# Blaizzy/mlx-audio-swift

Hardware: NVIDIA H100
Metric: orpheus3b_tts_rtfx_batch8 (higher is better)
Workload: dtype bf16

## Files before the change

### include/b200audio_internal.h

```cpp
#ifndef B200AUDIO_INTERNAL_H
#define B200AUDIO_INTERNAL_H

#include "b200audio.h"

#ifdef __cplusplus
extern "C" {
#endif

int32_t b2a_tts_create_random(int32_t device, const b2a_llama_config* cfg, float std, uint64_t seed,
                              b2a_snac* snac, b2a_tts** out);
int32_t b2a_stt_create_random(int32_t device, const b2a_whisper_config* cfg, float std, uint64_t seed, b2a_stt** out);
int32_t b2a_tts_set_bench_flags(b2a_tts* h, int32_t mask_eos, int32_t wrap_codes);
int32_t b2a_stt_set_bench_flags(b2a_stt* h, int32_t mask_eot);
int32_t b2a_tts_time_steps(b2a_tts* h, int32_t batch, int32_t ctx, int32_t iters, float* ms_per_step);
int32_t b2a_qwen3_talker_create_random(int32_t device, const b2a_qwen3_talker_config* cfg, float std, uint64_t seed, b2a_qwen3_talker** out);
int32_t b2a_qwen3_talker_set_bench_flags(b2a_qwen3_talker* h, int32_t mask_eos);

int32_t b2a_tts_debug_trace(b2a_tts* h, int32_t enable, int32_t batch, float* out);
int32_t b2a_debug_step_smem(int32_t gqa, int32_t* out);

int32_t b2a_speech_tokenizer_debug_layout(const float* w, int32_t out, int32_t k, int32_t in, int32_t stride, float* layout_out,
                                          int64_t capacity, int32_t* rows, int32_t* taps, int32_t* kpad);
int32_t b2a_speech_tokenizer_debug_stage(b2a_speech_tokenizer* h, int32_t stage, float* out, int64_t capacity, int64_t* n);
int32_t b2a_qwen3_sample_test(const float* logits, int32_t batch, int32_t vocab, float temperature, float top_p, int32_t top_k,
                              float min_p, float repetition_penalty, int32_t eos, int32_t suppress_lo, int32_t suppress_hi,
                              uint32_t* seen, int32_t track, uint64_t seed, int32_t step, int32_t* tokens_out, float* filtered_out);
int32_t b2a_implicit_conv_test(const float* w, int32_t M, int32_t taps, int32_t Cin, const float* x, int32_t B, int32_t Ttot, int32_t T,
                               int32_t dil, int32_t shift0, int32_t up, const float* bias, const float* gamma, int32_t gelu, int32_t add,
                               int32_t bias_twice_t0, const float* sa, const float* sb, int32_t Hout, int32_t fp16, float* xo, float* hl_out);
int32_t b2a_tc_gemm_epilogue_test(const void* W, const void* X, void* out, int32_t M, int32_t N, int32_t K, int32_t bn, int32_t epi,
                                  int32_t split, int32_t hilo, int32_t ctas, const float* bias, int32_t act, int32_t tile_rows,
                                  int32_t lo_rows, const float* rstd_ss, int32_t rstd_parts, float rstd_eps, int32_t stages, void* stream);
int32_t b2a_tc_gemm_test(const void* W, const void* X, void* out, int32_t M, int32_t N, int32_t K, int32_t bn, int32_t epi,
                         int32_t split, int32_t hilo, int32_t ctas, void* stream);
int32_t b2a_tc_gemm_splitk_test(const void* W, const void* X, float* h, const float* gain, void* xn, float* ss, int32_t M, int32_t N,
                                int32_t K, int32_t cluster, int32_t stages, void* stream);
int32_t b2a_mha_tc_test(const float* qkv, void* out, int32_t B, int32_t T, int32_t nh, void* stream);
int32_t b2a_wh_decode_attn_test(int32_t self_attn, const float* q, const float* kv, const int32_t* pos, void* kcache, void* vcache,
                                void* out, float* part_o, float* part_ml, int32_t* counters, int32_t B, int32_t nh, int32_t max_t,
                                void* stream);
int32_t b2a_conv_gemm_test(const float* w, int32_t M, int32_t K, const void* X, int32_t N, int32_t epi, const float* bias,
                           const float* alpha, const float* gamma, int32_t gelu, float* x, int32_t ldx, void* hl, int32_t ldh,
                           int32_t dual, int32_t T, int32_t Cout, int32_t stride, int32_t pad, int32_t Tin, const float* noise,
                           uint64_t seed, int32_t ctas, void* stream);
int32_t b2a_snac_unit_test(int32_t mode, int32_t C, int32_t dil, const float* x, float* y, int32_t B, int32_t T, const float* dw_w,
                           const float* dw_b, const float* a_in, const float* a_mid, const float* pw_w, const float* pw_bias,
                           const float* noise, uint64_t seed, void* hl, const float* a_next, int32_t ctas, void* stream);
int32_t b2a_snac_convt_test(const float* x, float* y, const float* alpha, const float* bias, const float* w, int32_t B, int32_t Tin,
                            int32_t stride, int32_t cout, int32_t ctas, void* stream);
int32_t b2a_snac_encode_latent_test(b2a_snac* h, const float* wave, int32_t batch, int64_t n_samples, float* z);

#ifdef __cplusplus
}
#endif
#endif
```

### mlx-audio-swift_b200/_ffi.py

```python
from __future__ import annotations

import ctypes as C
from pathlib import Path

import numpy as np

LIB_PATH = Path(__file__).resolve().parent / "lib" / "libb200audio.so"

(OK, ERR_MODEL_NOT_INITIALIZED, ERR_GENERATION_FAILED, ERR_INVALID_INPUT, ERR_AUDIO_DECODING_FAILED,
 ERR_AUDIO_ENCODING_FAILED, ERR_CANCELLED, ERR_CUDA) = range(8)
DTYPE_F32, DTYPE_BF16, DTYPE_I32 = 0, 1, 2


class AudioGenerationError(RuntimeError):
    CASES = {1: "modelNotInitialized", 2: "generationFailed", 3: "invalidInput", 4: "audioDecodingFailed",
             5: "audioEncodingFailed", 6: "cancelled", 7: "cudaError"}

    def __init__(self, code: int, message: str):
        super().__init__(f"{self.CASES.get(code, code)}: {message}")
        self.code, self.case, self.message = code, self.CASES.get(code, str(code)), message


class Tensor(C.Structure):
    _fields_ = [("name", C.c_char_p), ("dtype", C.c_int32), ("ndim", C.c_int32), ("shape", C.c_int64 * 4),
                ("data", C.c_void_p)]


class SnacConfig(C.Structure):
    _fields_ = [("sampling_rate", C.c_int32), ("encoder_dim", C.c_int32), ("n_encoder_rates", C.c_int32),
                ("encoder_rates", C.c_int32 * 8), ("latent_dim", C.c_int32), ("decoder_dim", C.c_int32),
                ("n_decoder_rates", C.c_int32), ("decoder_rates", C.c_int32 * 8), ("attn_window_size", C.c_int32),
                ("codebook_size", C.c_int32), ("codebook_dim", C.c_int32), ("n_vq_strides", C.c_int32),
                ("vq_strides", C.c_int32 * 8), ("noise", C.c_int32), ("depthwise", C.c_int32)]


class LlamaConfig(C.Structure):
    _fields_ = [("hidden_size", C.c_int32), ("num_hidden_layers", C.c_int32), ("intermediate_size", C.c_int32),
                ("num_attention_heads", C.c_int32), ("num_key_value_heads", C.c_int32), ("head_dim", C.c_int32),
                ("vocab_size", C.c_int32), ("rms_norm_eps", C.c_float), ("rope_theta", C.c_float),
                ("rope_factor", C.c_float), ("rope_low_freq_factor", C.c_float), ("rope_high_freq_factor", C.c_float),
                ("rope_old_context_len", C.c_float), ("tie_word_embeddings", C.c_int32), ("max_batch", C.c_int32),
                ("max_context", C.c_int32)]


class GenParams(C.Structure):
    _fields_ = [("max_tokens", C.c_int32), ("temperature", C.c_float), ("top_p", C.c_float),
                ("repetition_penalty", C.c_float), ("repetition_context_size", C.c_int32), ("seed", C.c_uint64)]


class GenInfo(C.Structure):
    _fields_ = [("prompt_token_count", C.c_int32), ("generation_token_count", C.c_int32), ("prefill_time", C.c_double),
                ("generate_time", C.c_double), ("tokens_per_second", C.c_double), ("codec_time", C.c_double),
                ("peak_memory_gb", C.c_double)]


class VocosConfig(C.Structure):
    _fields_ = [(n, C.c_int32) for n in ("input_channels", "dim", "intermediate_dim", "num_layers", "n_fft", "hop_length",
                                          "input_kernel_size", "dw_kernel_size", "adanorm_num_embeddings")]


class EncodecConfig(C.Structure):
    _fields_ = ([(n, C.c_int32) for n in ("audio_channels", "num_filters", "kernel_size", "num_residual_layers",
                                           "dilation_growth_rate", "codebook_size", "codebook_dim", "hidden_size",
                                           "num_lstm_layers", "residual_kernel_size", "use_causal_conv", "pad_mode_reflect",
                                           "norm_type", "last_kernel_size", "compress", "n_upsampling_ratios")]
                + [("upsampling_ratios", C.c_int32 * 8), ("sampling_rate", C.c_int32), ("use_conv_shortcut", C.c_int32),
                   ("trim_right_ratio", C.c_float), ("chunk_length_s", C.c_float), ("overlap", C.c_float)])


class SpeechTokenizerConfig(C.Structure):
    _fields_ = ([(n, C.c_int32) for n in ("codebook_size", "codebook_dim", "latent_dim", "decoder_dim", "hidden_size",
                                           "intermediate_size", "head_dim", "num_attention_heads", "num_key_value_heads",
                                           "num_hidden_layers", "num_quantizers", "num_semantic_quantizers")]
                + [("rms_norm_eps", C.c_float), ("rope_theta", C.c_float), ("attention_bias", C.c_int32),
                   ("num_upsample_rates", C.c_int32), ("upsample_rates", C.c_int32 * 8),
                   ("num_upsampling_ratios", C.c_int32), ("upsampling_ratios", C.c_int32 * 8),
                   ("max_batch", C.c_int32), ("max_cache_frames", C.c_int32)])


class Qwen3TalkerConfig(C.Structure):
    _fields_ = ([(n, C.c_int32) for n in ("vocab_size", "hidden_size", "intermediate_size", "num_hidden_layers", "num_attention_heads",
                                           "num_key_value_heads", "head_dim")]
                + [("rms_norm_eps", C.c_float), ("rope_theta", C.c_float)]
                + [(n, C.c_int32) for n in ("num_code_groups", "text_hidden_size", "text_vocab_size", "codec_eos_token_id", "cp_vocab_size",
                                             "cp_hidden_size", "cp_intermediate_size", "cp_num_hidden_layers", "cp_num_attention_heads",
                                             "cp_num_key_value_heads", "cp_head_dim")]
                + [("cp_rms_norm_eps", C.c_float), ("cp_rope_theta", C.c_float), ("max_batch", C.c_int32), ("max_context", C.c_int32)])


class Qwen3GenParams(C.Structure):
    _fields_ = [("max_tokens", C.c_int32), ("temperature", C.c_float), ("top_p", C.c_float), ("top_k", C.c_int32), ("min_p", C.c_float),
                ("repetition_penalty", C.c_float), ("seed", C.c_uint64)]


class WhisperConfig(C.Structure):
    _fields_ = [(n, C.c_int32) for n in ("vocab_size", "num_mel_bins", "d_model", "encoder_layers", "encoder_attention_heads",
                                          "encoder_ffn_dim", "max_source_positions", "decoder_layers", "decoder_attention_heads",
                                          "decoder_ffn_dim", "max_target_positions", "max_batch")]


class SttParams(C.Structure):
    _fields_ = [("max_tokens", C.c_int32), ("temperature", C.c_float), ("prompt_ids", C.c_void_p), ("n_prompt", C.c_int32),
                ("begin_suppress", C.c_void_p), ("n_begin_suppress", C.c_int32), ("suppress", C.c_void_p),
                ("n_suppress", C.c_int32), ("timestamp_begin", C.c_int32), ("eot", C.c_int32), ("seed", C.c_uint64)]


class SttInfo(C.Structure):
    _fields_ = [("prompt_tokens", C.c_int32), ("generation_tokens", C.c_int32), ("decode_steps", C.c_int32),
                ("encode_time", C.c_double), ("decode_time", C.c_double), ("total_time", C.c_double)]


TOKEN_CB = C.CFUNCTYPE(None, C.c_void_p, C.c_int32, C.c_int32, C.c_int32)
AUDIO_CB = C.CFUNCTYPE(None, C.c_void_p, C.c_int32, C.POINTER(C.c_float), C.c_int64, C.c_int32)
STT_DECODE_CB = C.CFUNCTYPE(C.c_int32, C.c_void_p, C.POINTER(C.c_float), C.c_int64, C.POINTER(C.c_int32), C.c_int32, C.POINTER(C.c_int32),
                            C.c_int32, C.POINTER(C.c_int32))


class SttStreamConfig(C.Structure):
    _fields_ = [("decode_interval_s", C.c_double), ("window_s", C.c_double), ("window_overlap_s", C.c_double), ("delay_ms", C.c_int32),
                ("min_agreement_passes", C.c_int32), ("max_tokens_per_pass", C.c_int32), ("sample_rate", C.c_int32)]


class SttStreamUpdate(C.Structure):
    _fields_ = [("kind", C.c_int32), ("promoted", C.c_int32), ("completed_windows", C.c_int32), ("n_confirmed", C.c_int32),
                ("n_provisional", C.c_int32), ("total_audio_s", C.c_double), ("pass_encode_time", C.c_double), ("pass_decode_time", C.c_double)]


_P = C.c_void_p
SIGNATURES = {
    "b2a_last_error": (C.c_char_p, []),
    "b2a_version": (C.c_char_p, []),
    "b2a_device_count": (C.c_int32, []),
    "b2a_launch_count": (C.c_int64, []),
    "b2a_hanning_window": (C.c_int32, [C.c_int32, C.c_int32, _P]),
    "b2a_hamming_window": (C.c_int32, [C.c_int32, C.c_int32, _P]),
    "b2a_power_to_db": (C.c_int32, [_P, C.c_int64, C.c_float, C.c_float, _P]),
    "b2a_mel_filters": (C.c_int32, [C.c_int32, C.c_int32, C.c_int32, C.c_float, C.c_float, C.c_int32, C.c_int32, _P]),
    "b2a_mel_create": (C.c_int32, [C.c_int32, C.c_int32, C.c_int32, C.c_int32, C.c_int32, C.POINTER(_P)]),
    "b2a_mel_max_frames": (C.c_int64, [_P, C.c_int64]),
    "b2a_mel_process": (C.c_int32, [_P, _P, C.c_int64, _P, C.c_int64, C.POINTER(C.c_int64)]),
    "b2a_mel_flush": (C.c_int32, [_P, _P, C.c_int64, C.POINTER(C.c_int64)]),
    "b2a_mel_reset": (C.c_int32, [_P]),
    "b2a_mel_total_frames": (C.c_int64, [_P]),
    "b2a_mel_destroy": (None, [_P]),
    "b2a_logmel_create": (C.c_int32, [C.c_int32, C.c_int32, C.c_int32, C.c_int32, C.c_int32, C.c_int32, C.POINTER(_P)]),
    "b2a_logmel_frames": (C.c_int64, [_P, C.c_int64]),
    "b2a_logmel_compute": (C.c_int32, [_P, _P, C.c_int32, C.c_int64, _P]),
    "b2a_logmel_compute_dev": (C.c_int32, [_P, _P, C.c_int32, C.c_int64, _P, _P]),
    "b2a_logmel_destroy": (None, [_P]),
    "b2a_snac_create": (C.c_int32, [C.c_int32, C.POINTER(SnacConfig), C.POINTER(Tensor), C.c_int32, C.POINTER(_P)]),
    "b2a_snac_hop_length": (C.c_int64, [_P]),
    "b2a_snac_decode": (C.c_int32, [_P, C.POINTER(_P), C.c_int32, C.c_int64, C.POINTER(_P), C.c_int32, C.c_uint64, _P]),
    "b2a_snac_decode_dev": (C.c_int32, [_P, C.POINTER(_P), C.c_int32, C.c_int64, C.POINTER(_P), C.c_int32, C.c_uint64, _P, _P]),
    "b2a_snac_quantize": (C.c_int32, [_P, _P, C.c_int32, C.c_int64, C.POINTER(_P), _P]),
    "b2a_snac_encoded_length": (C.c_int64, [_P, C.c_int64]),
    "b2a_snac_encode": (C.c_int32, [_P, _P, C.c_int32, C.c_int64, C.POINTER(_P)]),
    "b2a_snac_encode_dev": (C.c_int32, [_P, _P, C.c_int32, C.c_int64, C.POINTER(_P), _P]),
    "b2a_snac_encode_latent_test": (C.c_int32, [_P, _P, C.c_int32, C.c_int64, _P]),
    "b2a_snac_destroy": (None, [_P]),
    "b2a_tts_create": (C.c_int32, [C.c_int32, C.POINTER(LlamaConfig), C.POINTER(Tensor), C.c_int32, _P, C.POINTER(_P)]),
    "b2a_tts_debug_trace": (C.c_int32, [_P, C.c_int32, C.c_int32, _P]),
    "b2a_debug_step_smem": (C.c_int32, [C.c_int32, C.POINTER(C.c_int32)]),
    "b2a_tts_create_random": (C.c_int32, [C.c_int32, C.POINTER(LlamaConfig), C.c_float, C.c_uint64, _P, C.POINTER(_P)]),
    "b2a_tts_stream": (C.c_void_p, [_P]),
    "b2a_tts_set_bench_flags": (C.c_int32, [_P, C.c_int32, C.c_int32]),
    "b2a_stt_set_bench_flags": (C.c_int32, [_P, C.c_int32]),
    "b2a_tts_time_steps": (C.c_int32, [_P, C.c_int32, C.c_int32, C.c_int32, C.POINTER(C.c_float)]),
    "b2a_snac_stream": (C.c_void_p, [_P]),
    "b2a_tts_prepare_input_ids": (C.c_int32, [C.POINTER(_P), _P, C.c_int32, _P, C.POINTER(C.c_int32)]),
    "b2a_tts_prepare_input_ids_ref": (C.c_int32, [C.POINTER(_P), _P, C.c_int32, _P, C.c_int32, _P, C.c_int32, _P, C.POINTER(C.c_int32)]),
    "b2a_tts_forward_logits": (C.c_int32, [_P, _P, C.c_int32, C.c_int32, C.c_int32, _P]),
    "b2a_tts_generate": (C.c_int32, [_P, _P, C.c_int32, C.c_int32, C.POINTER(GenParams), _P, _P, _P, C.c_int64, _P,
                                     C.POINTER(GenInfo), TOKEN_CB, _P]),
    "b2a_tts_generate_stream": (C.c_int32, [_P, _P, C.c_int32, C.c_int32, C.POINTER(GenParams), C.c_int32, C.c_int32, _P, _P,
                                            C.POINTER(GenInfo), TOKEN_CB, AUDIO_CB, _P]),
    "b2a_tts_generate_dev": (C.c_int32, [_P, _P, C.c_int32, C.c_int32, C.POINTER(GenParams), _P, C.c_int64, _P,
                                         C.POINTER(GenInfo)]),
    "b2a_tts_cancel": (C.c_int32, [_P]),
    "b2a_tts_parse_output": (C.c_int32, [_P, C.c_int32, C.c_int32, _P, _P]),
    "b2a_tts_deinterleave": (C.c_int32, [_P, C.c_int32, _P, _P, _P, C.POINTER(C.c_int32)]),
    "b2a_tts_interleave": (C.c_int32, [_P, _P, _P, C.c_int32, _P]),
    "b2a_tts_destroy": (None, [_P]),
    "b2a_vocos_create": (C.c_int32, [C.c_int32, C.POINTER(VocosConfig), C.POINTER(Tensor), C.c_int32, C.POINTER(_P)]),
    "b2a_vocos_output_length": (C.c_int64, [_P, C.c_int32]),
    "b2a_vocos_stream": (C.c_void_p, [_P]),
    "b2a_vocos_decode": (C.c_int32, [_P, _P, C.c_int32, C.c_int32, _P]),
    "b2a_vocos_decode_dev": (C.c_int32, [_P, _P, C.c_int32, C.c_int32, _P, _P]),
    "b2a_vocos_decode_cond": (C.c_int32, [_P, _P, _P, C.c_int32, C.c_int32, _P]),
    "b2a_vocos_destroy": (None, [_P]),
    "b2a_speech_tokenizer_create": (C.c_int32, [C.c_int32, C.POINTER(SpeechTokenizerConfig), C.POINTER(Tensor), C.c_int32, C.POINTER(_P)]),
    "b2a_speech_tokenizer_total_upsample": (C.c_int32, [_P]),
    "b2a_speech_tokenizer_stream": (C.c_void_p, [_P]),
    "b2a_speech_tokenizer_reset": (C.c_int32, [_P]),
    "b2a_speech_tokenizer_streaming_step": (C.c_int32, [_P, _P, C.c_int32, C.c_int32, C.c_int32, _P]),
    "b2a_speech_tokenizer_streaming_step_dev": (C.c_int32, [_P, _P, C.c_int32, C.c_int32, C.c_int32, _P, _P]),
    "b2a_speech_tokenizer_streaming_decode": (C.c_int32, [_P, _P, C.c_int32, C.c_int32, C.c_int32, C.c_int32, _P]),
    "b2a_speech_tokenizer_chunked_decode": (C.c_int32, [_P, _P, C.c_int32, C.c_int32, C.c_int32, C.c_int32, C.c_int32, _P]),
    "b2a_speech_tokenizer_destroy": (None, [_P]),
    "b2a_weights_sanitize_speech_tokenizer": (C.c_int32, [_P]),
    "b2a_speech_tokenizer_config_from_json": (C.c_int32, [C.c_char_p, C.c_int32, C.c_int32, C.POINTER(SpeechTokenizerConfig), C.POINTER(C.c_int32)]),
    "b2a_speech_tokenizer_create_from_directory": (C.c_int32, [C.c_char_p, C.c_int32, C.c_int32, C.c_int32, C.POINTER(_P), C.POINTER(C.c_int32)]),
    "b2a_qwen3_sample_test": (C.c_int32, [_P, C.c_int32, C.c_int32, C.c_float, C.c_float, C.c_int32, C.c_float, C.c_float, C.c_int32, C.c_int32,
                                         C.c_int32, _P, C.c_int32, C.c_uint64, C.c_int32, _P, _P]),
    "b2a_implicit_conv_test": (C.c_int32, [_P, C.c_int32, C.c_int32, C.c_int32, _P, C.c_int32, C.c_int32, C.c_int32, C.c_int32, C.c_int32, C.c_int32,
                                          _P, _P, C.c_int32, C.c_int32, C.c_int32, _P, _P, C.c_int32, C.c_int32, _P, _P]),
    "b2a_tc_gemm_test": (C.c_int32, [_P, _P, _P] + [C.c_int32] * 8 + [_P]),
    "b2a_tc_gemm_epilogue_test": (C.c_int32, [_P, _P, _P] + [C.c_int32] * 8 + [_P, C.c_int32, C.c_int32, C.c_int32, _P, C.c_int32,
                                                                             C.c_float, C.c_int32, _P]),
    "b2a_tc_gemm_splitk_test": (C.c_int32, [_P, _P, _P, _P, _P, _P] + [C.c_int32] * 5 + [_P]),
    "b2a_mha_tc_test": (C.c_int32, [_P, _P, C.c_int32, C.c_int32, C.c_int32, _P]),
    "b2a_wh_decode_attn_test": (C.c_int32, [C.c_int32, _P, _P, _P, _P, _P, _P, _P, _P, _P, C.c_int32, C.c_int32, C.c_int32, _P]),
    "b2a_conv_gemm_test": (C.c_int32, [_P, C.c_int32, C.c_int32, _P, C.c_int32, C.c_int32, _P, _P, _P, C.c_int32, _P, C.c_int32, _P,
                                       C.c_int32] + [C.c_int32] * 6 + [_P, C.c_uint64, C.c_int32, _P]),
    "b2a_snac_unit_test": (C.c_int32, [C.c_int32] * 3 + [_P, _P, C.c_int32, C.c_int32] + [_P] * 6 + [_P, C.c_uint64, _P, _P, C.c_int32, _P]),
    "b2a_snac_convt_test": (C.c_int32, [_P] * 5 + [C.c_int32] * 5 + [_P]),
    "b2a_speech_tokenizer_debug_stage": (C.c_int32, [_P, C.c_int32, _P, C.c_int64, _P]),
    "b2a_speech_tokenizer_debug_layout": (C.c_int32, [_P, C.c_int32, C.c_int32, C.c_int32, C.c_int32, _P, C.c_int64, _P, _P, _P]),
    "b2a_encodec_create": (C.c_int32, [C.c_int32, C.POINTER(EncodecConfig), C.POINTER(Tensor), C.c_int32, C.POINTER(_P)]),
    "b2a_encodec_output_length": (C.c_int64, [_P, C.c_int32, C.c_int32]),
    "b2a_encodec_num_codebooks": (C.c_int32, [_P]),
    "b2a_encodec_stream": (C.c_void_p, [_P]),
    "b2a_encodec_decode": (C.c_int32, [_P, _P, C.c_int32, C.c_int32, C.c_int32, C.c_int32, _P, _P]),
    "b2a_encodec_decode_dev": (C.c_int32, [_P, _P, C.c_int32, C.c_int32, C.c_int32, C.c_int32, _P, _P, _P]),
    "b2a_encodec_destroy": (None, [_P]),
    "b2a_weights_load": (C.c_int32, [C.c_char_p, C.POINTER(_P)]),
    "b2a_weights_count": (C.c_int32, [_P]),
    "b2a_weights_get": (C.c_int32, [_P, C.c_int32, C.POINTER(Tensor)]),
    "b2a_weights_sanitize_whisper": (C.c_int32, [_P, C.POINTER(C.c_int32)]),
    "b2a_weights_sanitize_llama": (C.c_int32, [_P, C.c_int32, C.c_int32, C.c_int32]),
    "b2a_weights_sanitize_llama_config": (C.c_int32, [_P, C.c_char_p]),
    "b2a_weights_dequantize": (C.c_int32, [_P, C.c_int32, C.c_int32]),
    "b2a_weights_free": (None, [_P]),
    "b2a_tts_config_from_json": (C.c_int32, [C.c_char_p, C.c_int32, C.c_int32, C.POINTER(LlamaConfig), C.POINTER(C.c_int32), C.POINTER(C.c_int32)]),
    "b2a_tts_create_from_directory": (C.c_int32, [C.c_char_p, C.c_int32, C.c_int32, C.c_int32, _P, C.POINTER(_P)]),
    "b2a_stt_create": (C.c_int32, [C.c_int32, C.POINTER(WhisperConfig), C.POINTER(Tensor), C.c_int32, C.POINTER(_P)]),
    "b2a_stt_create_random": (C.c_int32, [C.c_int32, C.POINTER(WhisperConfig), C.c_float, C.c_uint64, C.POINTER(_P)]),
    "b2a_stt_stream": (C.c_void_p, [_P]),
    "b2a_stt_encode": (C.c_int32, [_P, _P, C.c_int32, C.c_int64, _P]),
    "b2a_stt_decoder_logits": (C.c_int32, [_P, _P, C.c_int32, C.c_int32, _P]),
    "b2a_stt_transcribe": (C.c_int32, [_P, _P, C.c_int32, C.c_int64, C.POINTER(SttParams), _P, _P, C.POINTER(SttInfo)]),
    "b2a_stt_transcribe_dev": (C.c_int32, [_P, _P, C.c_int32, C.c_int64, C.POINTER(SttParams), _P, _P, C.POINTER(SttInfo)]),
    "b2a_stt_transcribe_long": (C.c_int32, [_P, _P, C.c_int64, C.POINTER(SttParams), C.c_int32, _P, _P, _P, C.POINTER(C.c_int32), C.POINTER(SttInfo)]),
    "b2a_qwen3_talker_create": (C.c_int32, [C.c_int32, C.POINTER(Qwen3TalkerConfig), C.POINTER(Tensor), C.c_int32, C.POINTER(_P)]),
    "b2a_qwen3_talker_create_random": (C.c_int32, [C.c_int32, C.POINTER(Qwen3TalkerConfig), C.c_float, C.c_uint64, C.POINTER(_P)]),
    "b2a_qwen3_talker_set_bench_flags": (C.c_int32, [_P, C.c_int32]),
    "b2a_qwen3_talker_stream": (C.c_void_p, [_P]),
    "b2a_qwen3_talker_embed_text": (C.c_int32, [_P, _P, C.c_int32, _P]),
    "b2a_qwen3_talker_embed_codec": (C.c_int32, [_P, _P, C.c_int32, _P]),
    "b2a_qwen3_talker_forward": (C.c_int32, [_P, _P, C.c_int32, C.c_int32, _P, _P]),
    "b2a_qwen3_talker_generate": (C.c_int32, [_P, _P, C.c_int32, C.c_int32, _P, _P, C.c_int32, _P, C.POINTER(Qwen3GenParams), _P, _P,
                                              C.POINTER(GenInfo), _P, _P]),
    "b2a_qwen3_talker_config_from_json": (C.c_int32, [C.c_char_p, C.c_int32, C.c_int32, C.POINTER(Qwen3TalkerConfig)]),
    "b2a_weights_sanitize_qwen3_talker": (C.c_int32, [_P, C.c_char_p]),
    "b2a_qwen3_talker_create_from_directory": (C.c_int32, [C.c_char_p, C.c_int32, C.c_int32, C.c_int32, C.POINTER(_P)]),
    "b2a_qwen3_talker_cancel": (C.c_int32, [_P]),
    "b2a_qwen3_talker_destroy": (None, [_P]),
    "b2a_stt_session_create": (C.c_int32, [_P, C.POINTER(SttParams), C.POINTER(SttStreamConfig), C.POINTER(_P)]),
    "b2a_stt_session_create_with_decoder": (C.c_int32, [STT_DECODE_CB, _P, C.POINTER(SttStreamConfig), C.POINTER(_P)]),
    "b2a_stt_session_feed": (C.c_int32, [_P, _P, C.c_int64, C.c_double, C.POINTER(SttStreamUpdate)]),
    "b2a_stt_session_stop": (C.c_int32, [_P, C.c_double, C.POINTER(SttStreamUpdate)]),
    "b2a_stt_session_tokens": (C.c_int32, [_P, C.c_int32, C.c_int32, _P, C.c_int32, C.POINTER(C.c_int32)]),
    "b2a_stt_session_destroy": (None, [_P]),
    "b2a_stt_cancel": (C.c_int32, [_P]),
    "b2a_stt_destroy": (None, [_P]),
}

_lib = None


def lib() -> C.CDLL:
    global _lib
    if _lib is None:
        if not LIB_PATH.exists():
            raise ImportError(f"{LIB_PATH} is missing: build it with `python -c 'import __graft_entry__ as g; g.build()'`"
                              " -- there is no CPU fallback")
        _lib = C.CDLL(str(LIB_PATH))
        for name, (res, args) in SIGNATURES.items():
            fn = getattr(_lib, name)
            fn.restype, fn.argtypes = res, args
    return _lib


def check(status: int) -> None:
    if status != OK:
        raise AudioGenerationError(status, lib().b2a_last_error().decode("utf-8", "replace"))


def ptr(a) -> C.c_void_p:
    if a is None:
        return C.c_void_p(None)
    if isinstance(a, np.ndarray):
        assert a.flags["C_CONTIGUOUS"]
        return C.c_void_p(a.ctypes.data)
    return C.c_void_p(a.data_ptr())


def make_tensor_table(weights: dict):
    import torch
    arr = (Tensor * len(weights))()
    keep = []
    for i, (name, w) in enumerate(weights.items()):
        if isinstance(w, torch.Tensor):
            w = w.detach().contiguous().cpu()
            if w.dtype == torch.bfloat16:
                dt = DTYPE_BF16
            elif w.dtype == torch.float32:
                dt = DTYPE_F32
            else:
                w = w.to(torch.float32); dt = DTYPE_F32
            data, shape = w.data_ptr(), tuple(w.shape)
        else:
            w = np.ascontiguousarray(w)
            if w.dtype == np.int32:
                dt = DTYPE_I32
            else:
                if w.dtype != np.float32:
                    w = w.astype(np.float32)
                dt = DTYPE_F32
            data, shape = w.ctypes.data, w.shape
        assert len(shape) <= 4, name
        nm = name.encode()
        keep += [w, nm]
        arr[i].name, arr[i].dtype, arr[i].ndim, arr[i].data = nm, dt, len(shape), data
        for j, s in enumerate(shape):
            arr[i].shape[j] = s
    return arr, keep
```

### mlx-audio-swift_b200/csrc/llama.cu

```cuda
#include "common.cuh"
#include <cooperative_groups.h>
#include "tc_gemm.cuh"
#include "qwen3_sampler.cuh"

#include <algorithm>
#include <cstdlib>
#include <cstring>
#include <chrono>
#include <cmath>

namespace b2a {

typedef __nv_bfloat16 bf16;

constexpr int TOK_START_OF_HUMAN = 128259, TOK_END_OF_HUMAN = 128260, TOK_END_OF_TEXT = 128009;
constexpr int TOK_START_OF_SPEECH = 128257, TOK_END_OF_SPEECH = 128258, TOK_PAD = 128263;
constexpr int TOK_AUDIO_OFFSET = 128266;
constexpr int TOK_AUDIO_START = 128261, TOK_AUDIO_END = 128262;

__device__ __forceinline__ float bf16_round(float x) { return __bfloat162float(__float2bfloat16_rn(x)); }
__device__ __forceinline__ float bf_lo(unsigned u) { return __uint_as_float(u << 16); }
__device__ __forceinline__ float bf_hi(unsigned u) { return __uint_as_float(u & 0xffff0000u); }

__device__ __forceinline__ uint4 ldg_stream(const uint4* p) {
    uint4 r;
    asm volatile("ld.global.nc.L1::no_allocate.v4.u32 {%0,%1,%2,%3}, [%4];"
                 : "=r"(r.x), "=r"(r.y), "=r"(r.z), "=r"(r.w) : "l"(p));
    return r;
}

__global__ void embed_kernel(const int* __restrict__ tokens, const bf16* __restrict__ embed, float* __restrict__ x,
                             float* __restrict__ y, int H, int V) {
    const int b = blockIdx.x;
    pdl_trigger();
    pdl_wait();
    int tok = tokens[b];
    tok = min(max(tok, 0), V - 1);
    for (int i = threadIdx.x; i < H; i += blockDim.x) {
        x[(long long)b * H + i] = __bfloat162float(embed[(long long)tok * H + i]);
        y[(long long)b * H + i] = 0.f;
    }
}

__global__ void ext_embed_kernel(const float* __restrict__ src, float* __restrict__ x, float* __restrict__ y, int H) {
    const int b = blockIdx.x;
    pdl_trigger();
    pdl_wait();
    for (int i = threadIdx.x; i < H; i += blockDim.x) {
        x[(long long)b * H + i] = src[(long long)b * H + i];
        y[(long long)b * H + i] = 0.f;
    }
}

__global__ void finalize_norm_kernel(const float* __restrict__ x, const float* __restrict__ w, const float* __restrict__ ss, int parts,
                                     float* __restrict__ out, int H, float eps) {
    const int b = blockIdx.x;
    pdl_trigger();
    pdl_wait();
    float t = 0.f;
    for (int p = 0; p < parts; ++p) t += ss[p * 8 + b];
    const float r = rsqrtf(t / (float)H + eps);
    for (int i = threadIdx.x; i < H; i += blockDim.x) out[(long long)b * H + i] = x[(long long)b * H + i] * r * w[i];
}

constexpr int LO_ROW = 8;

constexpr int RN_THREADS = 1024, RN_MAXV = 8;
__global__ void __launch_bounds__(RN_THREADS)
add_rmsnorm_kernel(float* __restrict__ x, float* __restrict__ delta, const float* __restrict__ w,
                   bf16* __restrict__ xn, int H, float eps, float* __restrict__ trace, float* __restrict__ zero_ptr,
                   int zero_n, int half, float* __restrict__ normed = nullptr, float* __restrict__ ss_out = nullptr,
                   int ss_parts = 0) {
    __shared__ float red[RN_THREADS / 32];
    const int b = blockIdx.x, tid = threadIdx.x;
    pdl_trigger();
    pdl_wait();
    float* xr = x + (long long)b * H;
    float v[RN_MAXV];
    float ss = 0.f;
#pragma unroll
    for (int j = 0; j < RN_MAXV; ++j) {
        const int i = tid + j * RN_THREADS;
        float val = 0.f;
        if (i < H) {
            val = xr[i];
            if (delta) { val += delta[(long long)b * H + i]; xr[i] = val; delta[(long long)b * H + i] = 0.f; }
            if (trace) trace[(long long)b * H + i] = val;
        }
        v[j] = val;
        ss += val * val;
    }
    ss = warp_sum(ss);
    if ((tid & 31) == 0) red[tid >> 5] = ss;
    __syncthreads();
    float tot = 0.f;
#pragma unroll
    for (int i = 0; i < RN_THREADS / 32; ++i) tot += red[i];
    const float r = ss_out ? 1.0f : rsqrtf(tot / (float)H + eps);
    if (ss_out && tid < ss_parts) ss_out[tid * 8 + b] = tid == 0 ? tot : 0.f;
#pragma unroll
    for (int j = 0; j < RN_MAXV; ++j) {
        const int i = tid + j * RN_THREADS;
        if (i < H) {
            const float o = v[j] * r * w[i];
            tc::store_hilo(xn, H, b, i, o, half);
            if (normed) normed[(long long)b * H + i] = o;
        }
    }
    if (zero_ptr)
        for (int i = tid; i < zero_n; i += RN_THREADS) zero_ptr[(long long)b * zero_n + i] = 0.f;
}

constexpr int GV_MAX_THREADS = 256;
enum : int { GV_F32 = 0, GV_SWIGLU = 1, GV_F32_ATOMIC = 2 };

template <int NB, int ROWS, int EPI>
__global__ void __launch_bounds__(GV_MAX_THREADS)
gemv_bf16_kernel(const bf16* __restrict__ W, const bf16* __restrict__ xin, float* __restrict__ y,
                 bf16* __restrict__ act, int N, int K) {
    extern __shared__ uint4 sx[];
    pdl_trigger();
    pdl_wait();
    const int K8 = K >> 3;
    const int Kc8 = K8 / gridDim.y, kbase = blockIdx.y * Kc8;
    for (int i = threadIdx.x; i < 2 * NB * Kc8; i += blockDim.x) {
        const int r = i / Kc8, k = i - r * Kc8;
        const int grow = r < NB ? r : LO_ROW + (r - NB);
        sx[i] = reinterpret_cast<const uint4*>(xin)[(long long)grow * K8 + kbase + k];
    }
    __syncthreads();
    const int warp = threadIdx.x >> 5, lane = threadIdx.x & 31;
    const int row0 = (blockIdx.x * (blockDim.x >> 5) + warp) * ROWS;
    if (row0 >= N) return;
    const uint4* Wr[ROWS];
#pragma unroll
    for (int r = 0; r < ROWS; ++r)
        Wr[r] = reinterpret_cast<const uint4*>(W) + (long long)min(row0 + r, N - 1) * K8 + kbase;

    float acc[ROWS][2 * NB];
#pragma unroll
    for (int r = 0; r < ROWS; ++r)
#pragma unroll
        for (int b = 0; b < 2 * NB; ++b) acc[r][b] = 0.f;

    for (int k8 = lane; k8 < Kc8; k8 += 32) {
        float wf[ROWS][8];
#pragma unroll
        for (int r = 0; r < ROWS; ++r) {
            const uint4 wv = ldg_stream(Wr[r] + k8);
            wf[r][0] = bf_lo(wv.x); wf[r][1] = bf_hi(wv.x); wf[r][2] = bf_lo(wv.y); wf[r][3] = bf_hi(wv.y);
            wf[r][4] = bf_lo(wv.z); wf[r][5] = bf_hi(wv.z); wf[r][6] = bf_lo(wv.w); wf[r][7] = bf_hi(wv.w);
        }
#pragma unroll
        for (int b = 0; b < 2 * NB; ++b) {
            const uint4 xv = sx[b * Kc8 + k8];
            const float xf[8] = {bf_lo(xv.x), bf_hi(xv.x), bf_lo(xv.y), bf_hi(xv.y),
                                 bf_lo(xv.z), bf_hi(xv.z), bf_lo(xv.w), bf_hi(xv.w)};
#pragma unroll
            for (int r = 0; r < ROWS; ++r)
#pragma unroll
                for (int j = 0; j < 8; ++j) acc[r][b] = fmaf(wf[r][j], xf[j], acc[r][b]);
        }
    }
#pragma unroll
    for (int r = 0; r < ROWS; ++r)
#pragma unroll
        for (int b = 0; b < NB; ++b) acc[r][b] = warp_sum(acc[r][b] + acc[r][NB + b]);
    if (lane == 0) {
        if (EPI == GV_F32 || EPI == GV_F32_ATOMIC) {
#pragma unroll
            for (int r = 0; r < ROWS; ++r)
                if (row0 + r < N)
#pragma unroll
                    for (int b = 0; b < NB; ++b) {
                        if (EPI == GV_F32) y[(long long)b * N + row0 + r] = acc[r][b];
                        else atomicAdd(&y[(long long)b * N + row0 + r], acc[r][b]);
                    }
        } else {
#pragma unroll
            for (int r = 0; r < ROWS; r += 2)
                if (row0 + r + 1 < N)
#pragma unroll
                    for (int b = 0; b < NB; ++b) {
                        const float g = acc[r][b], u = acc[r + 1][b];
                        tc::store_hilo(act, N / 2, b, (row0 + r) / 2, g / (1.0f + __expf(-g)) * u, LO_ROW);
                    }
        }
    }
}

constexpr int HD = 128, AT_THREADS = 256, MAXG = 8, AT_CAP = 64;
constexpr int AT_SLOTS = 3;
constexpr size_t attn_smem_bytes(int G) {
    return ((size_t)AT_SLOTS * AT_CAP * HD + (size_t)G * HD + 2 * HD + (size_t)G * HD + 2 * MAXG) * sizeof(float) + 64;
}
static_assert((AT_THREADS / 32) * MAXG * HD <= AT_CAP * HD, "the warp-partial outputs must fit in one ring slot");

struct AttnArgs {
    const float* qkv;
    const int* pos;
    const float* freqs;
    float* kcache;
    float* vcache;
    bf16* out;
    int nq, nkv, max_ctx;
    float scale;
    const float* qnorm;
    const float* knorm;
    float qk_eps;
    int zero_qkv;
};

template <int G>
__global__ void __cluster_dims__(1, 1, 2) __launch_bounds__(AT_THREADS)
attn_decode_cluster_kernel(const __grid_constant__ AttnArgs a) {
    namespace cgr = cooperative_groups;
    cgr::cluster_group cluster = cgr::this_cluster();
    const int rank = (int)cluster.block_rank();
    extern __shared__ __align__(16) uint8_t at_smem[];
    float* sKV = reinterpret_cast<float*>(at_smem);
    float* wpo = sKV;
    float* sq = sKV + (size_t)AT_SLOTS * AT_CAP * HD;
    float* snew = sq + G * HD;
    float* xo = snew + 2 * HD;
    float* xml = xo + G * HD;
    uint64_t* bars = reinterpret_cast<uint64_t*>(xml + 2 * MAXG);
    __shared__ float red_m[AT_THREADS / 32][MAXG], red_l[AT_THREADS / 32][MAXG];

    const int h = blockIdx.x, b = blockIdx.y, tid = threadIdx.x;
    pdl_trigger();
    const int p = a.pos[b];
    if (!(p >= 0 && p < a.max_ctx)) { pdl_wait(); return; }
    const int nch = p / AT_CAP + 1;
    const int n_my = nch > rank ? (nch - rank + 1) / 2 : 0;
    const bool owner = ((nch - 1) & 1) == rank;
    const int qkv_ld = (a.nq + 2 * a.nkv) * HD;
    const float* row = a.qkv + (long long)b * qkv_ld;
    float* kc = a.kcache + (((long long)b * a.nkv + h) * a.max_ctx) * HD;
    float* vc = a.vcache + (((long long)b * a.nkv + h) * a.max_ctx) * HD;
    const int n_mat = 2 * n_my;
    auto issue = [&](int j) {
        const int slot = j % AT_SLOTS, c = rank + 2 * (j >> 1);
        const int n_load = (c < nch - 1) ? AT_CAP : p - c * AT_CAP;
        if (n_load > 0) {
            const uint32_t bytes = (uint32_t)n_load * HD * 4;
            tc::mbar_arrive_expect_tx(&bars[slot], bytes);
            asm volatile("cp.async.bulk.shared::cluster.global.mbarrier::complete_tx::bytes [%0], [%1], %2, [%3];"
                         ::"r"(tc::smem_u32(sKV + (size_t)slot * AT_CAP * HD)), "l"(((j & 1) ? vc : kc) + (long long)c * AT_CAP * HD), "r"(bytes),
                           "r"(tc::smem_u32(&bars[slot])) : "memory");
        } else {
            tc::mbar_arrive(&bars[slot]);
        }
    };
    if (tid == 0) {
        for (int i = 0; i < AT_SLOTS; ++i) tc::mbar_init(&bars[i], 1);
        tc::fence_barrier_init();
        asm volatile("fence.proxy.async.shared::cta;" ::: "memory");
        for (int j = 0; j < min(n_mat, AT_SLOTS); ++j) issue(j);
    }
    float sn = 0.f, cs = 1.f;
    if (tid < HD / 2) sincosf((float)p / a.freqs[tid], &sn, &cs);
    pdl_wait();
    const float* qsrc = row + (long long)h * G * HD;
    const float* ksrc = row + (a.nq + h) * HD;
    if (a.qnorm) {
        for (int vec = tid >> 5; vec < G + 1; vec += AT_THREADS / 32) {
            const float* src = vec < G ? qsrc + vec * HD : ksrc;
            const float* w = vec < G ? a.qnorm : a.knorm;
            const float4 x = reinterpret_cast<const float4*>(src)[tid & 31];
            const float ss = warp_sum(x.x * x.x + x.y * x.y + x.z * x.z + x.w * x.w);
            const float r = rsqrtf(ss * (1.0f / HD) + a.qk_eps);
            const float4 g4 = reinterpret_cast<const float4*>(w)[tid & 31];
            reinterpret_cast<float4*>(vec < G ? sq + vec * HD : snew)[tid & 31] =
                make_float4(x.x * r * g4.x, x.y * r * g4.y, x.z * r * g4.z, x.w * r * g4.w);
        }
        __syncthreads();
        qsrc = sq;
        ksrc = snew;
    }
    if (tid < HD / 2) {
        const int d = tid;
        _Pragma("unroll") for (int g = 0; g < G; ++g) {
            const float* q = qsrc + g * HD;
            const float x1 = q[d], x2 = q[d + HD / 2];
            sq[g * HD + d] = x1 * cs - x2 * sn;
            sq[g * HD + d + HD / 2] = x2 * cs + x1 * sn;
        }
        const float* k = ksrc;
        const float x1 = k[d], x2 = k[d + HD / 2];
        const float k1 = x1 * cs - x2 * sn, k2 = x2 * cs + x1 * sn;
        if (owner) { kc[(long long)p * HD + d] = k1; kc[(long long)p * HD + d + HD / 2] = k2; }
        snew[d] = k1;
        snew[d + HD / 2] = k2;
    } else if (tid >= 128) {
        const int d = tid - 128;
        const float v = row[(a.nq + a.nkv + h) * HD + d];
        if (owner) vc[(long long)p * HD + d] = v;
        snew[HD + d] = v;
    }
    __syncthreads();

    const int lane = tid & 31, warp = tid >> 5;
    const int kslot = warp * 8 + (lane >> 2), part = lane & 3;
    float m_run[G], l_run[G];
    float4 o4[G];
    _Pragma("unroll") for (int g = 0; g < G; ++g) { m_run[g] = -INFINITY; l_run[g] = 0.f; o4[g] = make_float4(0.f, 0.f, 0.f, 0.f); }

    for (int i = 0; i < n_my; ++i) {
        const int jk = 2 * i, jv = 2 * i + 1, c = rank + 2 * i;
        float* sK = sKV + (size_t)(jk % AT_SLOTS) * AT_CAP * HD;
        float* sV = sKV + (size_t)(jv % AT_SLOTS) * AT_CAP * HD;
        const int t0 = c * AT_CAP, nk = min(AT_CAP, p + 1 - t0);
        tc::mbar_wait(&bars[jk % AT_SLOTS], (uint32_t)((jk / AT_SLOTS) & 1));
        if (c == nch - 1) {
            if (tid < HD) sK[(p - t0) * HD + tid] = snew[tid];
            __syncthreads();
        }
        float sacc[G];
        _Pragma("unroll") for (int g = 0; g < G; ++g) sacc[g] = 0.f;
        if (kslot < nk) {
            const float4* kr = reinterpret_cast<const float4*>(sK + kslot * HD);
#pragma unroll
            for (int j = 0; j < 8; ++j) {
                const int d4 = part + 4 * ((j + kslot) & 7);
                const float4 kf = kr[d4];
                _Pragma("unroll") for (int g = 0; g < G; ++g) {
                    const float4 qf = reinterpret_cast<const float4*>(sq + g * HD)[d4];
                    sacc[g] = fmaf(qf.x, kf.x, sacc[g]); sacc[g] = fmaf(qf.y, kf.y, sacc[g]);
                    sacc[g] = fmaf(qf.z, kf.z, sacc[g]); sacc[g] = fmaf(qf.w, kf.w, sacc[g]);
                }
            }
        }
        if (jk + AT_SLOTS < n_mat) {
            __syncthreads();
            if (tid == 0) issue(jk + AT_SLOTS);
        }
        float pw[G];
        _Pragma("unroll") for (int g = 0; g < G; ++g) {
            float v = sacc[g];
            v += __shfl_xor_sync(0xffffffffu, v, 1);
            v += __shfl_xor_sync(0xffffffffu, v, 2);
            const float sv = kslot < nk ? v * a.scale : -INFINITY;
            float m = sv;
            m = fmaxf(m, __shfl_xor_sync(0xffffffffu, m, 4));
            m = fmaxf(m, __shfl_xor_sync(0xffffffffu, m, 8));
            m = fmaxf(m, __shfl_xor_sync(0xffffffffu, m, 16));
            const float m_new = fmaxf(m_run[g], m);
            const float rescale = (m_run[g] == -INFINITY) ? 0.f : __expf(m_run[g] - m_new);
            const float e = (sv == -INFINITY) ? 0.f : __expf(sv - m_new);
            float l = part == 0 ? e : 0.f;
            l = warp_sum(l);
            l_run[g] = l_run[g] * rescale + l;
            m_run[g] = m_new;
            o4[g].x *= rescale; o4[g].y *= rescale; o4[g].z *= rescale; o4[g].w *= rescale;
            pw[g] = e;
        }
        tc::mbar_wait(&bars[jv % AT_SLOTS], (uint32_t)((jv / AT_SLOTS) & 1));
        if (c == nch - 1) {
            if (tid >= HD) sV[(p - t0) * HD + tid - HD] = snew[tid];
            __syncthreads();
        }
#pragma unroll
        for (int kk = 0; kk < 8; ++kk) {
            const int t = warp * 8 + kk;
            if (t < nk) {
                const float4 v = reinterpret_cast<const float4*>(sV + t * HD)[lane];
                _Pragma("unroll") for (int g = 0; g < G; ++g) {
                    const float pk = __shfl_sync(0xffffffffu, pw[g], kk * 4);
                    o4[g].x = fmaf(pk, v.x, o4[g].x); o4[g].y = fmaf(pk, v.y, o4[g].y);
                    o4[g].z = fmaf(pk, v.z, o4[g].z); o4[g].w = fmaf(pk, v.w, o4[g].w);
                }
            }
        }
        if (jv + AT_SLOTS < n_mat) {
            __syncthreads();
            if (tid == 0) issue(jv + AT_SLOTS);
        }
    }
    __syncthreads();
    _Pragma("unroll") for (int g = 0; g < G; ++g) {
        reinterpret_cast<float4*>(wpo + (warp * G + g) * HD)[lane] = o4[g];
        if (lane == 0) { red_m[warp][g] = m_run[g]; red_l[warp][g] = l_run[g]; }
    }
    __syncthreads();
    float Ms[G], Ls[G], Os[G];
    if (tid < HD) {
        _Pragma("unroll") for (int g = 0; g < G; ++g) {
            float M = red_m[0][g];
#pragma unroll
            for (int w = 1; w < AT_THREADS / 32; ++w) M = fmaxf(M, red_m[w][g]);
            float L = 0.f, O = 0.f;
#pragma unroll
            for (int w = 0; w < AT_THREADS / 32; ++w) {
                const float sc_w = red_m[w][g] == -INFINITY ? 0.f : __expf(red_m[w][g] - M);
                L = fmaf(red_l[w][g], sc_w, L);
                O = fmaf(wpo[(w * G + g) * HD + tid], sc_w, O);
            }
            Ms[g] = M; Ls[g] = L; Os[g] = O;
        }
        if (rank == 1) {
            float* rxo = cluster.map_shared_rank(xo, 0);
            float* rxml = cluster.map_shared_rank(xml, 0);
            _Pragma("unroll") for (int g = 0; g < G; ++g) {
                rxo[g * HD + tid] = Os[g];
                if (tid == 0) { rxml[g] = Ms[g]; rxml[MAXG + g] = Ls[g]; }
            }
        }
    }
    cluster.sync();
    if (a.zero_qkv && rank == 0) {
        float* wrow = const_cast<float*>(row);
        for (int i = tid; i < G * HD; i += AT_THREADS) wrow[(long long)h * G * HD + i] = 0.f;
        if (tid < HD) { wrow[(a.nq + h) * HD + tid] = 0.f; wrow[(a.nq + a.nkv + h) * HD + tid] = 0.f; }
    }
    if (rank == 0 && tid < HD) {
        _Pragma("unroll") for (int g = 0; g < G; ++g) {
            const float M1 = xml[g], L1 = xml[MAXG + g], O1 = xo[g * HD + tid];
            const float M = fmaxf(Ms[g], M1);
            const float w0 = Ms[g] == -INFINITY ? 0.f : __expf(Ms[g] - M), w1 = M1 == -INFINITY ? 0.f : __expf(M1 - M);
            const float L = Ls[g] * w0 + L1 * w1, O = Os[g] * w0 + O1 * w1;
            tc::store_hilo(a.out, (long long)a.nq * HD, b, (h * G + g) * HD + tid, O / L, LO_ROW);
        }
    }
}

constexpr int PF_HALF = 64;
constexpr int PA_QT = 32, PA_THREADS = 256, PA_MAXL = 128;

__global__ void embed_rows_kernel(const int* __restrict__ ids, const bf16* __restrict__ embed, float* __restrict__ x,
                                  int H, int V) {
    const int t = blockIdx.x;
    int tok = ids[t];
    tok = min(max(tok, 0), V - 1);
    for (int i = threadIdx.x; i < H; i += blockDim.x) x[(long long)t * H + i] = __bfloat162float(embed[(long long)tok * H + i]);
}

__global__ void rope_table_kernel(const float* __restrict__ freqs, float2* __restrict__ tab, int L) {
    const int i = blockIdx.x * blockDim.x + threadIdx.x;
    if (i >= L * (HD / 2)) return;
    const int p = i / (HD / 2), d = i - p * (HD / 2);
    float s, c;
    sincosf((float)p / freqs[d], &s, &c);
    tab[i] = make_float2(c, s);
}

struct PrefillAttnArgs {
    const float* qkv;
    const float2* rope;
    float* kcache;
    float* vcache;
    bf16* out;
    int nq, nkv, max_ctx, L;
    float scale;
};

template <int G>
__global__ void __launch_bounds__(PA_THREADS)
prefill_attn_kernel(PrefillAttnArgs a) {
    extern __shared__ __align__(16) uint8_t pa_smem[];
    const int h = blockIdx.x, b = blockIdx.y, q0 = blockIdx.z * PA_QT;
    const int nqt = min(PA_QT, a.L - q0), kmax = q0 + nqt;
    float* sK = reinterpret_cast<float*>(pa_smem);
    float* sV = sK + (size_t)a.L * HD;
    float* sQ = sV + (size_t)a.L * HD;
    const int tid = threadIdx.x, lane = tid & 31, warp = tid >> 5;
    const int ld = (a.nq + 2 * a.nkv) * HD;
    const float* base = a.qkv + (long long)b * a.L * ld;
    float* kc = a.kcache + (((long long)b * a.nkv + h) * a.max_ctx) * HD;
    float* vc = a.vcache + (((long long)b * a.nkv + h) * a.max_ctx) * HD;

    for (int i = tid; i < kmax * (HD / 2); i += PA_THREADS) {
        const int t = i / (HD / 2), d = i - t * (HD / 2);
        const float2 cs = a.rope[t * (HD / 2) + d];
        const float* k = base + (long long)t * ld + (a.nq + h) * HD;
        const float x1 = k[d], x2 = k[d + HD / 2];
        const float k1 = x1 * cs.x - x2 * cs.y, k2 = x2 * cs.x + x1 * cs.y;
        sK[t * HD + d] = k1; sK[t * HD + d + HD / 2] = k2;
        if (t >= q0) { kc[(long long)t * HD + d] = k1; kc[(long long)t * HD + d + HD / 2] = k2; }
    }
    for (int i = tid; i < kmax * HD; i += PA_THREADS) {
        const int t = i / HD, d = i - t * HD;
        const float v = base[(long long)t * ld + (a.nq + a.nkv + h) * HD + d];
        sV[i] = v;
        if (t >= q0) vc[(long long)t * HD + d] = v;
    }
    for (int i = tid; i < G * nqt * (HD / 2); i += PA_THREADS) {
        const int g = i / (nqt * (HD / 2)), r = i - g * nqt * (HD / 2), qi = r / (HD / 2), d = r - qi * (HD / 2);
        const float2 cs = a.rope[(q0 + qi) * (HD / 2) + d];
        const float* q = base + (long long)(q0 + qi) * ld + (h * G + g) * HD;
        const float x1 = q[d], x2 = q[d + HD / 2];
        sQ[(g * PA_QT + qi) * HD + d] = x1 * cs.x - x2 * cs.y;
        sQ[(g * PA_QT + qi) * HD + d + HD / 2] = x2 * cs.x + x1 * cs.y;
    }
    __syncthreads();

    constexpr int KJ = PA_MAXL / 32;
    for (int r = warp; r < G * nqt; r += PA_THREADS / 32) {
        const int g = r / nqt, qi = r - g * nqt, qpos = q0 + qi;
        const float4* q4 = reinterpret_cast<const float4*>(sQ + (g * PA_QT + qi) * HD);
        float sc[KJ];
        float mx = -INFINITY;
#pragma unroll
        for (int j = 0; j < KJ; ++j) {
            const int t = j * 32 + lane;
            float acc = -INFINITY;
            if (t <= qpos) {
                const float4* k4 = reinterpret_cast<const float4*>(sK + t * HD);
                acc = 0.f;
#pragma unroll 8
                for (int i = 0; i < HD / 4; ++i) {
                    const int d4 = (i + lane) & (HD / 4 - 1);
                    const float4 kf = k4[d4], qf = q4[d4];
                    acc = fmaf(qf.x, kf.x, acc); acc = fmaf(qf.y, kf.y, acc);
                    acc = fmaf(qf.z, kf.z, acc); acc = fmaf(qf.w, kf.w, acc);
                }
                acc *= a.scale;
            }
            sc[j] = acc;
            mx = fmaxf(mx, acc);
        }
        for (int o = 16; o; o >>= 1) mx = fmaxf(mx, __shfl_xor_sync(0xffffffffu, mx, o));
        float sum = 0.f;
#pragma unroll
        for (int j = 0; j < KJ; ++j) { sc[j] = sc[j] == -INFINITY ? 0.f : __expf(sc[j] - mx); sum += sc[j]; }
        sum = warp_sum(sum);
        float4 o = make_float4(0.f, 0.f, 0.f, 0.f);
#pragma unroll
        for (int j = 0; j < KJ; ++j) {
            if (j * 32 > qpos) break;
            for (int l = 0; l < 32; ++l) {
                const int t = j * 32 + l;
                if (t > qpos) break;
                const float p = __shfl_sync(0xffffffffu, sc[j], l);
                const float4 v = reinterpret_cast<const float4*>(sV + t * HD)[lane];
                o.x = fmaf(p, v.x, o.x); o.y = fmaf(p, v.y, o.y); o.z = fmaf(p, v.z, o.z); o.w = fmaf(p, v.w, o.w);
            }
        }
        const float inv = 1.0f / sum;
        const int tok = b * a.L + qpos;
        const long long col = (long long)(h * G + g) * HD + lane * 4;
        const long long ldo = (long long)a.nq * HD;
        tc::store_hilo(a.out, ldo, tok, col + 0, o.x * inv, PF_HALF);
        tc::store_hilo(a.out, ldo, tok, col + 1, o.y * inv, PF_HALF);
        tc::store_hilo(a.out, ldo, tok, col + 2, o.z * inv, PF_HALF);
        tc::store_hilo(a.out, ldo, tok, col + 3, o.w * inv, PF_HALF);
    }
}

__global__ void gather_last_kernel(const float* __restrict__ xp, const float* __restrict__ yp, float* __restrict__ x,
                                   float* __restrict__ y, int* __restrict__ pos, int L, int H) {
    const int b = blockIdx.x;
    const long long src = ((long long)b * L + L - 1) * H;
    for (int i = threadIdx.x; i < H; i += blockDim.x) {
        x[(long long)b * H + i] = xp[src + i];
        y[(long long)b * H + i] = yp[src + i];
    }
    if (threadIdx.x == 0) pos[b] = L - 1;
}

constexpr int SM_THREADS = 1024, SM_WARPS = SM_THREADS / 32, SM_MAX_ATTEMPTS = 12;

struct SampleArgs {
    float* logits;
    float* probs;
    int* tokens;
    int* pos;
    int* recent;
    int* recent_n;
    int* out_tokens;
    int* n_gen;
    int* done;
    int* n_active;
    const int* forced;
    int V, R, max_tokens;
    float temperature, top_p, rep_penalty;
    unsigned long long seed;
    int mask_eos;
};

constexpr int SM_CLUSTER = 8;
struct SampleExchange { float v[2][SM_CLUSTER]; int i[2][SM_CLUSTER]; float s[2][SM_CLUSTER]; };

__global__ void __cluster_dims__(SM_CLUSTER, 1, 1) __launch_bounds__(SM_THREADS)
sample_kernel(SampleArgs a) {
    namespace cgr = cooperative_groups;
    cgr::cluster_group cluster = cgr::this_cluster();
    const int rank = (int)cluster.block_rank();
    __shared__ float sred[SM_WARPS];
    __shared__ float s_val[SM_WARPS];
    __shared__ int s_idx[SM_WARPS];
    __shared__ SampleExchange ex;
    const int b = blockIdx.x / SM_CLUSTER, t = threadIdx.x, lane = t & 31, warp = t >> 5;
    pdl_wait();
    float* lg = a.logits + (long long)b * a.V;
    const int chunk = (a.V + SM_CLUSTER - 1) / SM_CLUSTER, i0 = rank * chunk, i1 = min(a.V, i0 + chunk);
    const int nrec = min(a.recent_n[b], a.R);
    int parity = 0;
    int tok_final = 0;

    auto exchange = [&](float& v, int& i, float& sum) {
        for (int o = 16; o; o >>= 1) {
            const float ov = __shfl_xor_sync(0xffffffffu, v, o);
            const int oi = __shfl_xor_sync(0xffffffffu, i, o);
            if (ov > v || (ov == v && oi < i)) { v = ov; i = oi; }
        }
        sum = warp_sum(sum);
        __syncthreads();
        if (lane == 0) { s_val[warp] = v; s_idx[warp] = i; sred[warp] = sum; }
        __syncthreads();
        if (warp == 0) {
            float bv = s_val[lane], bs = sred[lane];
            int bi = s_idx[lane];
            for (int o = 16; o; o >>= 1) {
                const float ov = __shfl_xor_sync(0xffffffffu, bv, o);
                const int oi = __shfl_xor_sync(0xffffffffu, bi, o);
                if (ov > bv || (ov == bv && oi < bi)) { bv = ov; bi = oi; }
            }
            bs = warp_sum(bs);
            if (lane < SM_CLUSTER) {
                SampleExchange* peer = cluster.map_shared_rank(&ex, lane);
                peer->v[parity][rank] = bv; peer->i[parity][rank] = bi; peer->s[parity][rank] = bs;
            }
        }
        cluster.sync();
        v = ex.v[parity][0]; i = ex.i[parity][0]; sum = ex.s[parity][0];
#pragma unroll
        for (int r = 1; r < SM_CLUSTER; ++r) {
            const float ov = ex.v[parity][r];
            const int oi = ex.i[parity][r];
            if (ov > v || (ov == v && oi < i)) { v = ov; i = oi; }
            sum += ex.s[parity][r];
        }
        parity ^= 1;
    };

    if (a.forced == nullptr) {
        if (a.rep_penalty != 1.0f && t < nrec) {
            const int tok = a.recent[b * a.R + t];
            bool dup = false;
            for (int j = 0; j < t; ++j) dup |= (a.recent[b * a.R + j] == tok);
            if (!dup && tok >= i0 && tok < i1) {
                const float l = lg[tok];
                lg[tok] = l < 0.f ? l * a.rep_penalty : l / a.rep_penalty;
            }
        }
        if (a.mask_eos && t == 0 && TOK_END_OF_SPEECH >= i0 && TOK_END_OF_SPEECH < i1) lg[TOK_END_OF_SPEECH] = -INFINITY;
        __syncthreads();

        float best = -INFINITY, dummy = 0.f;
        int bi = 0x7fffffff;
        for (int i = i0 + t; i < i1; i += SM_THREADS) {
            const float v = lg[i];
            if (v > best) { best = v; bi = i; }
        }
        exchange(best, bi, dummy);
        const float mx = best;
        tok_final = bi;

        if (a.temperature > 0.f) {
            const float inv_t = 1.0f / a.temperature;
            const int step = a.n_gen[b];
            auto gumbel_key = [&](int i, float l, int att) {
                unsigned long long z = a.seed + 0x9E3779B97F4A7C15ull * ((unsigned long long)b * 1000003ull + (unsigned long long)step * 131ull + (unsigned long long)att + 1ull);
                z ^= (unsigned long long)(unsigned)i * 0xD6E8FEB86659FD93ull;
                z = (z ^ (z >> 30)) * 0xBF58476D1CE4E5B9ull;
                z = (z ^ (z >> 27)) * 0x94D049BB133111EBull;
                z ^= z >> 31;
                const float u = ((float)(z >> 40) + 0.5f) * (1.0f / 16777216.0f);
                return l * inv_t - __logf(-__logf(u));
            };
            float z = 0.f, gv = -INFINITY;
            int gi = 0x7fffffff;
            for (int i = i0 + t; i < i1; i += SM_THREADS) {
                const float l = lg[i];
                z += __expf((l - mx) * inv_t);
                const float k = l == -INFINITY ? -INFINITY : gumbel_key(i, l, 0);
                if (k > gv) { gv = k; gi = i; }
            }
            exchange(gv, gi, z);
            const float Z = z;
            int cand = gi;
            bool accepted = a.top_p >= 1.0f;
            for (int att = 0; !accepted; ++att) {
                const float lc = lg[cand];
                float gm = 0.f, dv = -INFINITY;
                int di = 0x7fffffff;
                for (int i = i0 + t; i < i1; i += SM_THREADS) { const float l = lg[i]; if (l > lc) gm += __expf((l - mx) * inv_t); }
                exchange(dv, di, gm);
                if (gm < a.top_p * Z) { accepted = true; break; }
                if (att + 1 >= SM_MAX_ATTEMPTS) { cand = tok_final; break; }
                gv = -INFINITY; gi = 0x7fffffff;
                float ds = 0.f;
                for (int i = i0 + t; i < i1; i += SM_THREADS) {
                    const float l = lg[i];
                    const float k = l == -INFINITY ? -INFINITY : gumbel_key(i, l, att + 1);
                    if (k > gv) { gv = k; gi = i; }
                }
                exchange(gv, gi, ds);
                cand = gi;
            }
            if (cand >= 0 && cand < a.V) tok_final = cand;
        }
    } else {
        tok_final = a.forced[b];
    }

    if (rank == 0 && t == 0) {
        const int tok = tok_final;
        a.tokens[b] = tok;
        a.pos[b] += 1;
        const int rn = a.recent_n[b];
        if (a.R > 0) {
            if (rn < a.R) a.recent[b * a.R + rn] = tok;
            else {
                for (int j = 1; j < a.R; ++j) a.recent[b * a.R + j - 1] = a.recent[b * a.R + j];
                a.recent[b * a.R + a.R - 1] = tok;
            }
            a.recent_n[b] = rn + 1;
        }
        if (a.forced == nullptr && !a.done[b]) {
            if (tok == TOK_END_OF_SPEECH) {
                a.done[b] = 1;
                atomicSub(a.n_active, 1);
            } else {
                const int n = a.n_gen[b];
                if (n < a.max_tokens) a.out_tokens[b * a.max_tokens + n] = tok;
                a.n_gen[b] = n + 1;
                if (n + 1 >= a.max_tokens) { a.done[b] = 1; atomicSub(a.n_active, 1); }
            }
        }
    }
}

__global__ void prefill_advance_kernel(const int* __restrict__ ids, int L, int* tokens, int* pos, int B) {
    const int b = threadIdx.x;
    pdl_wait();
    if (b >= B) return;
    const int p = pos[b] + 1;
    pos[b] = p;
    if (p < L) tokens[b] = ids[b * L + p];
}

__global__ void init_rows_kernel(const int* __restrict__ ids, int L, int B, int R, int* tokens, int* pos, int* recent,
                                 int* recent_n, int* n_gen, int* done, int* n_active, int start_pos) {
    const int b = threadIdx.x;
    if (b == 0) *n_active = B;
    if (b >= B) return;
    tokens[b] = ids[b * L];
    pos[b] = start_pos;
    n_gen[b] = 0;
    done[b] = 0;
    const int n = min(R, L);
    for (int j = 0; j < n; ++j) recent[b * R + j] = ids[b * L + L - n + j];
    recent_n[b] = n;
}

__global__ void random_bf16_kernel(bf16* __restrict__ w, long long n, float std, unsigned long long seed) {
    for (long long i = (long long)blockIdx.x * blockDim.x + threadIdx.x; i < n; i += (long long)gridDim.x * blockDim.x) {
        unsigned long long z = seed + 0x9E3779B97F4A7C15ull * (unsigned long long)(i + 1);
        z = (z ^ (z >> 30)) * 0xBF58476D1CE4E5B9ull;
        z = (z ^ (z >> 27)) * 0x94D049BB133111EBull;
        z ^= z >> 31;
        const float u1 = ((unsigned)(z >> 40) + 1.0f) * (1.0f / 16777217.0f);
        const float u2 = (unsigned)((z >> 8) & 0xFFFFFF) * (1.0f / 16777216.0f);
        w[i] = __float2bfloat16_rn(std * sqrtf(-2.0f * __logf(u1)) * cospif(2.0f * u2));
    }
}
__global__ void fill_f32_kernel(float* p, int n, float v) {
    const int i = blockIdx.x * blockDim.x + threadIdx.x;
    if (i < n) p[i] = v;
}

static std::vector<float> llama3_freqs(const b2a_llama_config& c) {
    const int d = c.head_dim;
    std::vector<float> f(d / 2);
    const float low_wl = c.rope_old_context_len / c.rope_low_freq_factor;
    const float high_wl = c.rope_old_context_len / c.rope_high_freq_factor;
    for (int i = 0; i < d / 2; ++i) {
        float fr = powf(c.rope_theta, (float)(2 * i) / (float)d);
        const float wl = 2.0f * (float)M_PI * fr;
        const float base = fr;
        if (wl > low_wl) fr = fr * c.rope_factor;
        const bool med = wl > high_wl && wl < low_wl;
        if (med) {
            const float smooth = (c.rope_old_context_len / wl - c.rope_low_freq_factor) /
                                 (c.rope_high_freq_factor - c.rope_low_freq_factor);
            fr = base / ((1.0f - smooth) / c.rope_factor + smooth);
        }
        f[i] = fr;
    }
    return f;
}

struct LayerW {
    DBuf<bf16> wqkv, wo, wgu, wdown;
    DBuf<float> ln1, ln2;
    DBuf<float> qnorm, knorm;
};

struct StackSpec {
    std::string prefix = "model.";
    bool qk_norm = false;
    bool has_embed = true;
    std::string head;
    bool has_head = true;
};

}

using namespace b2a;

struct b2a_tts {
    int device;
    b2a_llama_config cfg;
    b2a_snac* snac;
    cudaStream_t stream = nullptr;
    std::vector<LayerW> layers;
    DBuf<bf16> embed, lm_head_w;
    const bf16* lm_head = nullptr;
    DBuf<float> final_ln, freqs;
    DBuf<float> kcache, vcache;
    DBuf<float> x, y, qkv, logits, probs;
    DBuf<bf16> xn, attn, act;
    DBuf<float> sk_ws;
    DBuf<unsigned> sk_cnt;
    int sk_slots = 0;
    bool use_tc = true;
    int num_sms = 132;
    std::vector<CUtensorMap> tm_qkv, tm_o, tm_gu, tm_down;
    static int pick_tile_rows(int M, int sms) {
        if (cdiv(M, tc::BM) * 4 >= sms * 3) return tc::BM;
        return std::max(8, std::min(tc::BM, cdiv(cdiv(M, sms), 8) * 8));
    }
    int lm_tile_rows = 128, head_rows_now = 0;
    std::vector<CUtensorMap> tm_gu_dec;
    int gu_tile_rows = 0;
    CUtensorMap tm_lm{}, tmx_xn{}, tmx_attn{}, tmx_act{};
    DBuf<float> xp, yp, qkvp;
    DBuf<bf16> xnp, attnp, actp;
    DBuf<float2> rope_tab;
    CUtensorMap tmp_xn{}, tmp_attn{}, tmp_act{};
    int pf_tokens_cap = 0;
    bool use_batched_prefill = true;
    DBuf<int> tokens, pos, recent, recent_n, out_tokens, n_gen, done, n_active, ids, forced;
    HBuf<int> h_flag;
    cudaEvent_t ev_poll[2] = {nullptr, nullptr};
    bool fused = false;
    static constexpr int fused_cluster = 5;
    static constexpr int gemm_stages = 6, splitk_stages = 5;
    int fused_parts = 0;
    DBuf<float> ss_a, ss_b;
    StackSpec spec;
    const float* x_ext = nullptr;
    float* normed_out = nullptr;
    std::atomic<int> cancel{0};
    int bench_mask_eos = 0, bench_wrap_codes = 0;
    int nb_pad = 0;
    bool trace_on = false;
    DBuf<float> trace;
    cudaGraphExec_t g_step = nullptr, g_prefill = nullptr;
    SampleArgs g_args{};
    int g_nb = 0;
    DBuf<int> d_codes[3];
    DBuf<float> d_wave;

    ~b2a_tts() {
        if (g_step) cudaGraphExecDestroy(g_step);
        if (g_prefill) cudaGraphExecDestroy(g_prefill);
        for (auto& e : ev_poll) if (e) cudaEventDestroy(e);
        if (stream) cudaStreamDestroy(stream);
    }

    static void upload_bf16(const TensorTable& tt, const std::string& name, int64_t expect, DBuf<bf16>& dst, size_t offset_elems,
                            size_t total_elems) {
        const b2a_tensor& t = tt.get(name);
        B2A_CHECK(t.dtype == B2A_DTYPE_BF16 || t.dtype == B2A_DTYPE_F32, B2A_ERR_MODEL_NOT_INITIALIZED, "tensor must be bf16 or f32: " + name);
        B2A_CHECK(TensorTable::numel(t) == expect, B2A_ERR_MODEL_NOT_INITIALIZED, "bad shape for tensor: " + name);
        dst.alloc(total_elems);
        if (t.dtype == B2A_DTYPE_BF16) {
            B2A_CUDA(cudaMemcpy(dst.p + offset_elems, t.data, expect * sizeof(bf16), cudaMemcpyHostToDevice));
        } else {
            std::vector<bf16> tmp((size_t)expect);
            const float* src = (const float*)t.data;
            for (int64_t i = 0; i < expect; ++i) tmp[i] = __float2bfloat16_rn(src[i]);
            B2A_CUDA(cudaMemcpy(dst.p + offset_elems, tmp.data(), expect * sizeof(bf16), cudaMemcpyHostToDevice));
        }
    }

    template <int G>
    static void attn_cluster_attr() {
        B2A_CUDA(cudaFuncSetAttribute(attn_decode_cluster_kernel<G>, cudaFuncAttributeMaxDynamicSharedMemorySize, (int)attn_smem_bytes(G)));
        B2A_CUDA(cudaFuncSetAttribute(attn_decode_cluster_kernel<G>, cudaFuncAttributePreferredSharedMemoryCarveout, cudaSharedmemCarveoutMaxShared));
    }
    void attn_launch(const AttnArgs& aa, int B, cudaStream_t s) {
        const int G = aa.nq / aa.nkv;
        const size_t sm = attn_smem_bytes(G);
        const dim3 g3(aa.nkv, B, 2);
        switch (G) {
            case 1: launch_pdl(attn_decode_cluster_kernel<1>, g3, dim3(AT_THREADS), sm, s, aa); break;
            case 2: launch_pdl(attn_decode_cluster_kernel<2>, g3, dim3(AT_THREADS), sm, s, aa); break;
            case 3: launch_pdl(attn_decode_cluster_kernel<3>, g3, dim3(AT_THREADS), sm, s, aa); break;
            case 4: launch_pdl(attn_decode_cluster_kernel<4>, g3, dim3(AT_THREADS), sm, s, aa); break;
            case 6: launch_pdl(attn_decode_cluster_kernel<6>, g3, dim3(AT_THREADS), sm, s, aa); break;
            default: launch_pdl(attn_decode_cluster_kernel<8>, g3, dim3(AT_THREADS), sm, s, aa); break;
        }
    }

    void check_config() {
        const b2a_llama_config& c = cfg;
        B2A_CHECK(c.head_dim == HD, B2A_ERR_INVALID_INPUT, "llama: head_dim must be 128");
        B2A_CHECK(c.hidden_size % 8 == 0 && c.intermediate_size % 8 == 0, B2A_ERR_INVALID_INPUT, "llama: sizes must be multiples of 8");
        {
            const int g = c.num_key_value_heads > 0 && c.num_attention_heads % c.num_key_value_heads == 0
                              ? c.num_attention_heads / c.num_key_value_heads : 0;
            B2A_CHECK(g == 1 || g == 2 || g == 3 || g == 4 || g == 6 || g == 8, B2A_ERR_INVALID_INPUT,
                      "llama: unsupported GQA ratio (q heads per kv head must be 1, 2, 3, 4, 6 or 8)");
        }
        B2A_CHECK(c.max_batch >= 1 && c.max_batch <= 8, B2A_ERR_INVALID_INPUT, "llama: max_batch must be in 1..8");
        B2A_CHECK(c.max_context >= 8, B2A_ERR_INVALID_INPUT, "llama: max_context too small");
        require_device(device);
        B2A_CUDA(cudaStreamCreateWithFlags(&stream, cudaStreamNonBlocking));
    }

    void alloc_state() {
        const b2a_llama_config& c = cfg;
        const int H = c.hidden_size, I = c.intermediate_size, nq = c.num_attention_heads, nkv = c.num_key_value_heads;
        const int NQ = nq * HD, NKV = nkv * HD;
        B2A_CHECK(H <= RN_THREADS * RN_MAXV, B2A_ERR_INVALID_INPUT, "llama: hidden_size above 8192 is not supported");
        std::vector<float> fr = llama3_freqs(c);
        freqs.upload(fr.data(), fr.size());
        const size_t kv = (size_t)c.num_hidden_layers * c.max_batch * nkv * c.max_context * HD;
        kcache.alloc(kv);
        vcache.alloc(kv);
        B2A_CUDA(cudaMemset(kcache.p, 0, kv * sizeof(float)));
        B2A_CUDA(cudaMemset(vcache.p, 0, kv * sizeof(float)));
        const int B = 8, R16 = 16;
        x.alloc((size_t)B * H); y.alloc((size_t)B * H); qkv.alloc((size_t)B * (NQ + 2 * NKV));
        logits.alloc((size_t)B * c.vocab_size); probs.alloc((size_t)B * c.vocab_size);
        xn.alloc((size_t)R16 * H); attn.alloc((size_t)R16 * NQ); act.alloc((size_t)R16 * I);
        B2A_CUDA(cudaMemset(xn.p, 0, (size_t)R16 * H * sizeof(bf16)));
        B2A_CUDA(cudaMemset(attn.p, 0, (size_t)R16 * NQ * sizeof(bf16)));
        B2A_CUDA(cudaMemset(act.p, 0, (size_t)R16 * I * sizeof(bf16)));
        B2A_CUDA(cudaMemset(x.p, 0, (size_t)B * H * sizeof(float)));
        B2A_CUDA(cudaMemset(y.p, 0, (size_t)B * H * sizeof(float)));
        B2A_CUDA(cudaMemset(qkv.p, 0, (size_t)B * (NQ + 2 * NKV) * sizeof(float)));
        tokens.alloc(B); pos.alloc(B); recent.alloc(B * 64); recent_n.alloc(B); n_gen.alloc(B); done.alloc(B);
        n_active.alloc(1); forced.alloc(B);
        B2A_CUDA(cudaMemset(tokens.p, 0, B * sizeof(int)));
        B2A_CUDA(cudaMemset(pos.p, 0, B * sizeof(int)));
        h_flag.alloc(16);
        gemv_attrs<1>(); gemv_attrs<2>(); gemv_attrs<4>(); gemv_attrs<8>();
        attn_cluster_attr<1>(); attn_cluster_attr<2>(); attn_cluster_attr<3>(); attn_cluster_attr<4>(); attn_cluster_attr<6>(); attn_cluster_attr<8>();
        const char* env = getenv("B2A_GEMM");
        use_tc = !(env && std::string(env) == "simt") && H % tc::BK == 0 && NQ % tc::BK == 0 && I % tc::BK == 0;
        fused_parts = H / tc::BM;
        fused = use_tc && H % tc::BM == 0 && fused_parts <= 64;
        ss_a.alloc((size_t)64 * 8); ss_b.alloc((size_t)64 * 8);
        B2A_CUDA(cudaMemset(ss_a.p, 0, 64 * 8 * sizeof(float)));
        B2A_CUDA(cudaMemset(ss_b.p, 0, 64 * 8 * sizeof(float)));
        B2A_CUDA(cudaDeviceGetAttribute(&num_sms, cudaDevAttrMultiProcessorCount, device));
        {
            const int ops[3][2] = {{NQ + 2 * NKV, H}, {H, NQ}, {H, I}};
            int mt_max = 0;
            for (const auto& op : ops) {
                const int mt = cdiv(op[0], tc::BM), kb = op[1] / tc::BK;
                if (kb == 0) continue;
                const int ctas = (int)std::min<long long>(num_sms, (long long)mt * kb);
                sk_slots = std::max(sk_slots, tc::stream_k_slots(mt, kb, ctas));
                mt_max = std::max(mt_max, mt);
            }
            sk_ws.alloc((size_t)std::max(1, mt_max) * std::max(1, sk_slots) * 16 * tc::BM);
            sk_cnt.alloc((size_t)std::max(1, mt_max));
            B2A_CUDA(cudaMemset(sk_cnt.p, 0, (size_t)std::max(1, mt_max) * sizeof(unsigned)));
        }
        const char* envp = getenv("B2A_PREFILL");
        use_batched_prefill = !(envp && std::string(envp) == "step");
        if (use_tc) {
            tc::set_attributes();
            for (auto& L : layers) {
                tm_qkv.push_back(tc::make_tmap_bf16(L.wqkv.p, NQ + 2 * NKV, H, tc::BM));
                tm_o.push_back(tc::make_tmap_bf16(L.wo.p, H, NQ, tc::BM));
                tm_gu.push_back(tc::make_tmap_bf16(L.wgu.p, 2 * I, H, tc::BM));
                {
                    gu_tile_rows = pick_tile_rows(2 * I, num_sms);
                    tm_gu_dec.push_back(tc::make_tmap_bf16(L.wgu.p, 2 * I, H, gu_tile_rows));
                }
                tm_down.push_back(tc::make_tmap_bf16(L.wdown.p, H, I, tc::BM));
            }
            lm_tile_rows = pick_tile_rows(c.vocab_size, num_sms);
            if (lm_head) tm_lm = tc::make_tmap_bf16(lm_head, c.vocab_size, H, lm_tile_rows);
            tmx_xn = tc::make_tmap_bf16(xn.p, R16, H, 16);
            tmx_attn = tc::make_tmap_bf16(attn.p, R16, NQ, 16);
            tmx_act = tc::make_tmap_bf16(act.p, R16, I, 16);
        }
        B2A_CUDA(cudaDeviceSynchronize());
    }

    b2a_tts(int dev, const b2a_llama_config& c, const TensorTable& tt, b2a_snac* sn, const StackSpec& sp = StackSpec())
        : device(dev), cfg(c), snac(sn), spec(sp) {
        check_config();
        const int H = c.hidden_size, I = c.intermediate_size, nq = c.num_attention_heads, nkv = c.num_key_value_heads;
        const int NQ = nq * HD, NKV = nkv * HD;
        if (sp.has_embed) upload_bf16(tt, sp.prefix + "embed_tokens.weight", (int64_t)c.vocab_size * H, embed, 0, (size_t)c.vocab_size * H);
        if (sp.has_head) {
            if (sp.head.empty() && c.tie_word_embeddings) {
                B2A_CHECK(sp.has_embed, B2A_ERR_MODEL_NOT_INITIALIZED, "a tied head needs the embedding");
                lm_head = embed.p;
            } else {
                upload_bf16(tt, sp.head.empty() ? std::string("lm_head.weight") : sp.head, (int64_t)c.vocab_size * H, lm_head_w, 0, (size_t)c.vocab_size * H);
                lm_head = lm_head_w.p;
            }
        }
        layers.resize(c.num_hidden_layers);
        std::vector<bf16> tmp;
        for (int l = 0; l < c.num_hidden_layers; ++l) {
            const std::string p = sp.prefix + "layers." + std::to_string(l) + ".";
            if (sp.qk_norm) {
                std::vector<float> qn = tt.f32(p + "self_attn.q_norm.weight", HD), kn = tt.f32(p + "self_attn.k_norm.weight", HD);
                layers[l].qnorm.upload(qn.data(), HD);
                layers[l].knorm.upload(kn.data(), HD);
            }
            LayerW& L = layers[l];
            const size_t qkv_n = (size_t)(NQ + 2 * NKV) * H;
            upload_bf16(tt, p + "self_attn.q_proj.weight", (int64_t)NQ * H, L.wqkv, 0, qkv_n);
            upload_bf16(tt, p + "self_attn.k_proj.weight", (int64_t)NKV * H, L.wqkv, (size_t)NQ * H, qkv_n);
            upload_bf16(tt, p + "self_attn.v_proj.weight", (int64_t)NKV * H, L.wqkv, (size_t)(NQ + NKV) * H, qkv_n);
            upload_bf16(tt, p + "self_attn.o_proj.weight", (int64_t)H * NQ, L.wo, 0, (size_t)H * NQ);
            upload_bf16(tt, p + "mlp.down_proj.weight", (int64_t)H * I, L.wdown, 0, (size_t)H * I);
            const b2a_tensor& tg = tt.get(p + "mlp.gate_proj.weight");
            const b2a_tensor& tu = tt.get(p + "mlp.up_proj.weight");
            B2A_CHECK(tg.dtype == tu.dtype && (tg.dtype == B2A_DTYPE_BF16 || tg.dtype == B2A_DTYPE_F32) &&
                          TensorTable::numel(tg) == (int64_t)I * H && TensorTable::numel(tu) == (int64_t)I * H,
                      B2A_ERR_MODEL_NOT_INITIALIZED, "bad gate/up projection: " + p);
            tmp.resize((size_t)2 * I * H);
            for (int n = 0; n < I; ++n) {
                if (tg.dtype == B2A_DTYPE_BF16) {
                    memcpy(&tmp[(size_t)(2 * n) * H], (const bf16*)tg.data + (size_t)n * H, H * sizeof(bf16));
                    memcpy(&tmp[(size_t)(2 * n + 1) * H], (const bf16*)tu.data + (size_t)n * H, H * sizeof(bf16));
                } else {
                    for (int k = 0; k < H; ++k) {
                        tmp[(size_t)(2 * n) * H + k] = __float2bfloat16_rn(((const float*)tg.data)[(size_t)n * H + k]);
                        tmp[(size_t)(2 * n + 1) * H + k] = __float2bfloat16_rn(((const float*)tu.data)[(size_t)n * H + k]);
                    }
                }
            }
            L.wgu.alloc(tmp.size());
            B2A_CUDA(cudaMemcpy(L.wgu.p, tmp.data(), tmp.size() * sizeof(bf16), cudaMemcpyHostToDevice));
            std::vector<float> g1 = tt.f32(p + "input_layernorm.weight", H), g2 = tt.f32(p + "post_attention_layernorm.weight", H);
            L.ln1.upload(g1.data(), H);
            L.ln2.upload(g2.data(), H);
        }
        std::vector<float> gf = tt.f32(sp.prefix + "norm.weight", H);
        final_ln.upload(gf.data(), H);
        alloc_state();
    }

    b2a_tts(int dev, const b2a_llama_config& c, float std, unsigned long long seed, b2a_snac* sn, const StackSpec& sp = StackSpec())
        : device(dev), cfg(c), snac(sn), spec(sp) {
        check_config();
        const int H = c.hidden_size, I = c.intermediate_size, nq = c.num_attention_heads, nkv = c.num_key_value_heads;
        const int NQ = nq * HD, NKV = nkv * HD;
        unsigned long long sd = seed * 1000003ull + 17;
        auto rnd = [&](DBuf<bf16>& d, size_t n) {
            d.alloc(n);
            random_bf16_kernel<<<132 * 8, 256, 0, stream>>>(d.p, (long long)n, std, sd++);
            count_launch();
        };
        auto ones = [&](DBuf<float>& d, int n) {
            d.alloc(n);
            fill_f32_kernel<<<cdiv(n, 256), 256, 0, stream>>>(d.p, n, 1.0f);
            count_launch();
        };
        if (sp.has_embed) rnd(embed, (size_t)c.vocab_size * H);
        if (sp.has_head) {
            if (sp.head.empty() && c.tie_word_embeddings && sp.has_embed) lm_head = embed.p;
            else { rnd(lm_head_w, (size_t)c.vocab_size * H); lm_head = lm_head_w.p; }
        }
        layers.resize(c.num_hidden_layers);
        for (auto& L : layers) {
            if (sp.qk_norm) { ones(L.qnorm, HD); ones(L.knorm, HD); }
            rnd(L.wqkv, (size_t)(NQ + 2 * NKV) * H);
            rnd(L.wo, (size_t)H * NQ);
            rnd(L.wgu, (size_t)2 * I * H);
            rnd(L.wdown, (size_t)H * I);
            ones(L.ln1, H);
            ones(L.ln2, H);
        }
        ones(final_ln, H);
        B2A_CUDA(cudaStreamSynchronize(stream));
        B2A_CUDA(cudaGetLastError());
        alloc_state();
    }

    template <int NB, int ROWS, int EPI>
    void gemv_launch(const bf16* W, const bf16* xin, float* yout, bf16* actout, int N, int K, int warps, int ksplit,
                     cudaStream_t s) {
        const size_t sm = (size_t)2 * NB * (K / ksplit) * sizeof(bf16);
        dim3 grid(cdiv(N, warps * ROWS), ksplit);
        launch_pdl(gemv_bf16_kernel<NB, ROWS, EPI>, grid, dim3(warps * 32), sm, s, W, xin, yout, actout, N, K);
    }
    template <int NB, int ROWS, int EPI>
    static void gemv_attr() {
        B2A_CUDA(cudaFuncSetAttribute(gemv_bf16_kernel<NB, ROWS, EPI>, cudaFuncAttributeMaxDynamicSharedMemorySize, 200 * 1024));
    }
    template <int NB>
    static void gemv_attrs() {
        gemv_attr<NB, 2, GV_F32>(); gemv_attr<NB, 2, GV_SWIGLU>(); gemv_attr<NB, 2, GV_F32_ATOMIC>();
    }
    enum { OP_QKV, OP_O, OP_GU, OP_DOWN, OP_LM };
    template <int NB>
    void gemv_op(int op, const bf16* W, const bf16* xin, float* yout, bf16* actout, int N, int K, cudaStream_t s) {
        const bool split = (K / 8) % 2 == 0 && (size_t)2 * NB * K * sizeof(bf16) > 96 * 1024;
        switch (op) {
            case OP_GU: gemv_launch<NB, 2, GV_SWIGLU>(W, xin, yout, actout, N, K, 8, 1, s); break;
            case OP_DOWN:
            case OP_O:
                if (split) gemv_launch<NB, 2, GV_F32_ATOMIC>(W, xin, yout, actout, N, K, 4, 2, s);
                else gemv_launch<NB, 2, GV_F32>(W, xin, yout, actout, N, K, 4, 1, s);
                break;
            default: gemv_launch<NB, 2, GV_F32>(W, xin, yout, actout, N, K, 8, 1, s); break;
        }
    }
    void gemv_nb(int op, const bf16* W, const bf16* xin, float* yout, bf16* actout, int N, int K, cudaStream_t s) {
        B2A_CHECK((size_t)2 * nb_pad * K * sizeof(bf16) <= 200 * 1024 * ((op == OP_DOWN || op == OP_O) ? 2 : 1),
                  B2A_ERR_INVALID_INPUT, "llama: layer too wide for the shared-memory activation tile");
        switch (nb_pad) {
            case 1: gemv_op<1>(op, W, xin, yout, actout, N, K, s); break;
            case 2: gemv_op<2>(op, W, xin, yout, actout, N, K, s); break;
            case 4: gemv_op<4>(op, W, xin, yout, actout, N, K, s); break;
            default: gemv_op<8>(op, W, xin, yout, actout, N, K, s); break;
        }
    }

    void tc_gemm(const CUtensorMap& tmW, const CUtensorMap& tmX, int op, float* yout, bf16* actout, int B, int M, int K,
                 cudaStream_t s, const float* rstd_ss = nullptr) {
        tc::Args a{};
        a.rstd_ss = rstd_ss; a.rstd_parts = fused_parts; a.rstd_inv_h = 1.0f / (float)cfg.hidden_size; a.rstd_eps = cfg.rms_norm_eps;
        a.out_f32 = yout; a.out_bf16 = actout; a.M = M; a.N = B; a.K = K;
        a.m_tiles = cdiv(M, tc::BM); a.k_blocks = K / tc::BK;
        a.stages = gemm_stages;
        a.hilo = 1;
        int ctas = num_sms;
        if (op == OP_GU) {
            a.ldo = M / 2; a.epi_full = tc::EPI_SWIGLU; a.epi_partial = -1; a.lo_rows = LO_ROW;
            a.tile_rows = gu_tile_rows; a.m_tiles = cdiv(M, gu_tile_rows);
            ctas = std::min(num_sms, a.m_tiles);
        } else if (op == OP_LM) {
            a.ldo = M; a.epi_full = tc::EPI_STORE; a.epi_partial = -1; a.lo_rows = 0;
            a.tile_rows = head_rows_now > 0 ? head_rows_now : lm_tile_rows; a.m_tiles = cdiv(M, a.tile_rows);
            ctas = std::min(num_sms, a.m_tiles);
        } else {
            a.ldo = M; a.epi_full = tc::EPI_STORE; a.epi_partial = tc::EPI_PARTIAL; a.lo_rows = 0;
            ctas = (int)std::min<long long>(num_sms, (long long)a.m_tiles * a.k_blocks);
            a.part_ws = sk_ws.p; a.part_cnt = sk_cnt.p; a.part_slots = sk_slots;
        }
        tc::launch<16>(tmW, tmX, a, ctas, 1, s);
    }

    void gemm(int op, int layer, int B, cudaStream_t s) {
        const int H = cfg.hidden_size, I = cfg.intermediate_size, NQ = cfg.num_attention_heads * HD,
                  NKV = cfg.num_key_value_heads * HD;
        LayerW* L = layer >= 0 ? &layers[layer] : nullptr;
        switch (op) {
            case OP_QKV:
                if (use_tc) tc_gemm(tm_qkv[layer], tmx_xn, op, qkv.p, nullptr, B, NQ + 2 * NKV, H, s);
                else gemv_nb(op, L->wqkv.p, xn.p, qkv.p, nullptr, NQ + 2 * NKV, H, s);
                break;
            case OP_O:
                if (use_tc) tc_gemm(tm_o[layer], tmx_attn, op, y.p, nullptr, B, H, NQ, s);
                else gemv_nb(op, L->wo.p, attn.p, y.p, nullptr, H, NQ, s);
                break;
            case OP_GU:
                if (use_tc) tc_gemm(tm_gu_dec[layer], tmx_xn, op, nullptr, act.p, B, 2 * I, H, s);
                else gemv_nb(op, L->wgu.p, xn.p, nullptr, act.p, 2 * I, H, s);
                break;
            case OP_DOWN:
                if (use_tc) tc_gemm(tm_down[layer], tmx_act, op, y.p, nullptr, B, H, I, s);
                else gemv_nb(op, L->wdown.p, act.p, y.p, nullptr, H, I, s);
                break;
            default:
                if (use_tc) tc_gemm(tm_lm, tmx_xn, op, logits.p, nullptr, B, cfg.vocab_size, H, s);
                else gemv_nb(op, lm_head, xn.p, logits.p, nullptr, cfg.vocab_size, H, s);
                break;
        }
    }

    void splitk_gemm(const CUtensorMap& tmW, const CUtensorMap& tmX, int M, int K, const float* gain, float* ss, int B, cudaStream_t s) {
        tc::SplitArgs a{};
        a.M = M; a.N = B; a.K = K; a.k_blocks = K / tc::BK; a.stages = splitk_stages;
        a.h = x.p; a.gain = gain; a.xn = xn.p; a.ss = ss;
        a.rstd_ss = nullptr; a.rstd_parts = 0; a.rstd_inv_h = 0.f; a.rstd_eps = 0.f;
        tc::launch_splitk(tmW, tmX, a, cdiv(M, tc::BM), std::max(1, std::min(fused_cluster, a.k_blocks)), s);
    }
    void run_layers_fused(int B, cudaStream_t s) {
        const int H = cfg.hidden_size, I = cfg.intermediate_size, nq = cfg.num_attention_heads, nkv = cfg.num_key_value_heads;
        const int NQ = nq * HD, NKV = nkv * HD, L = cfg.num_hidden_layers;
        if (x_ext) launch_pdl(ext_embed_kernel, dim3(B), dim3(256), 0, s, x_ext, x.p, y.p, H);
        else launch_pdl(embed_kernel, dim3(B), dim3(256), 0, s, tokens.p, embed.p, x.p, y.p, H, cfg.vocab_size);
        launch_pdl(add_rmsnorm_kernel, dim3(B), dim3(RN_THREADS), 0, s, x.p, (float*)nullptr, layers[0].ln1.p, xn.p, H, cfg.rms_norm_eps,
                   (float*)nullptr, (float*)nullptr, 0, LO_ROW, (float*)nullptr, ss_b.p, fused_parts);
        const size_t kv_layer = (size_t)cfg.max_batch * nkv * cfg.max_context * HD;
        for (int l = 0; l < L; ++l) {
            LayerW& Lw = layers[l];
            tc_gemm(tm_qkv[l], tmx_xn, OP_QKV, qkv.p, nullptr, B, NQ + 2 * NKV, H, s, ss_b.p);
            AttnArgs aa{qkv.p, pos.p, freqs.p, kcache.p + l * kv_layer, vcache.p + l * kv_layer, attn.p, nq, nkv, cfg.max_context,
                        1.0f / sqrtf((float)HD), spec.qk_norm ? Lw.qnorm.p : nullptr, spec.qk_norm ? Lw.knorm.p : nullptr, cfg.rms_norm_eps, 1};
            attn_launch(aa, B, s);
            splitk_gemm(tm_o[l], tmx_attn, H, NQ, Lw.ln2.p, ss_a.p, B, s);
            tc_gemm(tm_gu_dec[l], tmx_xn, OP_GU, nullptr, act.p, B, 2 * I, H, s, ss_a.p);
            splitk_gemm(tm_down[l], tmx_act, H, I, l + 1 < L ? layers[l + 1].ln1.p : final_ln.p, ss_b.p, B, s);
        }
    }
    int launches_layers_fused() const { return 2 + cfg.num_hidden_layers * 5; }

    void run_layers(int B, cudaStream_t s) {
        if (fused && !trace_on) { run_layers_fused(B, s); return; }
        const int H = cfg.hidden_size, nq = cfg.num_attention_heads, nkv = cfg.num_key_value_heads;
        const int QKV_N = (nq + 2 * nkv) * HD, G = nq / nkv;
        if (x_ext) launch_pdl(ext_embed_kernel, dim3(B), dim3(256), 0, s, x_ext, x.p, y.p, H);
        else launch_pdl(embed_kernel, dim3(B), dim3(256), 0, s, tokens.p, embed.p, x.p, y.p, H, cfg.vocab_size);
        const size_t kv_layer = (size_t)cfg.max_batch * nkv * cfg.max_context * HD;
        for (int l = 0; l < cfg.num_hidden_layers; ++l) {
            LayerW& L = layers[l];
            launch_pdl(add_rmsnorm_kernel, dim3(B), dim3(RN_THREADS), 0, s, x.p, l == 0 ? (float*)nullptr : y.p, L.ln1.p, xn.p, H,
                       cfg.rms_norm_eps, trace_on ? trace.p + (size_t)(2 * l) * 8 * H : (float*)nullptr, (float*)nullptr, 0, LO_ROW,
                       (float*)nullptr, (float*)nullptr, 0);
            gemm(OP_QKV, l, B, s);
            AttnArgs aa{qkv.p, pos.p, freqs.p, kcache.p + l * kv_layer, vcache.p + l * kv_layer, attn.p, nq, nkv, cfg.max_context,
                        1.0f / sqrtf((float)HD), spec.qk_norm ? L.qnorm.p : nullptr, spec.qk_norm ? L.knorm.p : nullptr, cfg.rms_norm_eps, 0};
            attn_launch(aa, B, s);
            gemm(OP_O, l, B, s);
            launch_pdl(add_rmsnorm_kernel, dim3(B), dim3(RN_THREADS), 0, s, x.p, y.p, L.ln2.p, xn.p, H, cfg.rms_norm_eps,
                       trace_on ? trace.p + (size_t)(2 * l + 1) * 8 * H : (float*)nullptr, qkv.p, QKV_N, LO_ROW, (float*)nullptr, (float*)nullptr, 0);
            gemm(OP_GU, l, B, s);
            gemm(OP_DOWN, l, B, s);
        }
        (void)G;
    }

    void run_final_norm(int B, cudaStream_t s) {
        if (fused && !trace_on) {
            if (normed_out)
                launch_pdl(finalize_norm_kernel, dim3(B), dim3(256), 0, s, (const float*)x.p, (const float*)final_ln.p, (const float*)ss_b.p, fused_parts,
                           normed_out, cfg.hidden_size, cfg.rms_norm_eps);
            return;
        }
        launch_pdl(add_rmsnorm_kernel, dim3(B), dim3(RN_THREADS), 0, s, x.p, y.p, final_ln.p, xn.p, cfg.hidden_size, cfg.rms_norm_eps,
                   trace_on ? trace.p + (size_t)(2 * cfg.num_hidden_layers) * 8 * cfg.hidden_size : (float*)nullptr, (float*)nullptr, 0, LO_ROW,
                   normed_out, (float*)nullptr, 0);
    }
    void run_lm_head(int B, cudaStream_t s) {
        run_final_norm(B, s);
        if (fused && !trace_on) tc_gemm(tm_lm, tmx_xn, OP_LM, logits.p, nullptr, B, cfg.vocab_size, cfg.hidden_size, s, ss_b.p);
        else gemm(OP_LM, -1, B, s);
    }
    void run_lm_head_after_prefill(int B, cudaStream_t s) {
        launch_pdl(add_rmsnorm_kernel, dim3(B), dim3(RN_THREADS), 0, s, x.p, y.p, final_ln.p, xn.p, cfg.hidden_size, cfg.rms_norm_eps,
                   (float*)nullptr, (float*)nullptr, 0, LO_ROW, (float*)nullptr, (float*)nullptr, 0);
        gemm(OP_LM, -1, B, s);
    }
    void run_head(const CUtensorMap& tmW, const bf16* W, int M, float* logits_out, int B, cudaStream_t s, int tile_rows = 0) {
        head_rows_now = tile_rows;
        if (use_tc) tc_gemm(tmW, tmx_xn, OP_LM, logits_out, nullptr, B, M, cfg.hidden_size, s, (fused && !trace_on) ? ss_b.p : nullptr);
        else gemv_nb(OP_LM, W, xn.p, logits_out, nullptr, M, cfg.hidden_size, s);
        head_rows_now = 0;
    }

    template <int G>
    static void pattn_attr() {
        B2A_CUDA(cudaFuncSetAttribute(prefill_attn_kernel<G>, cudaFuncAttributeMaxDynamicSharedMemorySize, 220 * 1024));
    }
    size_t pattn_smem(int L) const {
        const int G = cfg.num_attention_heads / cfg.num_key_value_heads;
        return ((size_t)2 * L * HD + (size_t)G * PA_QT * HD) * sizeof(float);
    }
    bool can_batch_prefill(int L) const {
        return use_tc && use_batched_prefill && spec.has_embed && !spec.qk_norm && L >= 2 && L <= PA_MAXL && pattn_smem(L) <= 220 * 1024;
    }

    void pf_gemm(const CUtensorMap& tmW, const CUtensorMap& tmX, int epi, float* yout, bf16* actout, int T, int M, int K,
                 cudaStream_t s) {
        tc::Args a{};
        a.out_f32 = yout; a.out_bf16 = actout; a.M = M; a.N = T; a.K = K;
        a.m_tiles = cdiv(M, tc::BM); a.k_blocks = K / tc::BK;
        a.stages = tc::Smem<128>::max_stages(); a.hilo = 1; a.epi_full = epi; a.epi_partial = -1;
        a.ldo = epi == tc::EPI_SWIGLU ? M / 2 : M;
        a.lo_rows = epi == tc::EPI_SWIGLU ? PF_HALF : 0;
        const int n_tiles = cdiv(T, PF_HALF);
        const int ctas = std::max(1, std::min(a.m_tiles, num_sms / n_tiles));
        tc::launch<128>(tmW, tmX, a, ctas, n_tiles, s);
    }

    void prefill_batched(int B, int L, cudaStream_t s) {
        const int H = cfg.hidden_size, I = cfg.intermediate_size, nq = cfg.num_attention_heads, nkv = cfg.num_key_value_heads;
        const int NQ = nq * HD, QKV_N = (nq + 2 * nkv) * HD, T = B * L, G = nq / nkv;
        const int n_tiles = cdiv(T, PF_HALF), Tp = n_tiles * PF_HALF;
        if (Tp > pf_tokens_cap) {
            xp.alloc((size_t)Tp * H); yp.alloc((size_t)Tp * H); qkvp.alloc((size_t)Tp * QKV_N);
            xnp.alloc((size_t)2 * Tp * H); attnp.alloc((size_t)2 * Tp * NQ); actp.alloc((size_t)2 * Tp * I);
            pf_tokens_cap = Tp;
            tmp_xn = tc::make_tmap_bf16(xnp.p, 2 * Tp, H, 128);
            tmp_attn = tc::make_tmap_bf16(attnp.p, 2 * Tp, NQ, 128);
            tmp_act = tc::make_tmap_bf16(actp.p, 2 * Tp, I, 128);
            pattn_attr<1>(); pattn_attr<2>(); pattn_attr<3>(); pattn_attr<4>(); pattn_attr<6>(); pattn_attr<8>();
        }
        rope_tab.alloc((size_t)PA_MAXL * (HD / 2));
        B2A_CUDA(cudaMemsetAsync(xnp.p, 0, (size_t)2 * pf_tokens_cap * H * sizeof(bf16), s));
        B2A_CUDA(cudaMemsetAsync(attnp.p, 0, (size_t)2 * pf_tokens_cap * NQ * sizeof(bf16), s));
        B2A_CUDA(cudaMemsetAsync(actp.p, 0, (size_t)2 * pf_tokens_cap * I * sizeof(bf16), s));
        embed_rows_kernel<<<T, 256, 0, s>>>(ids.p, embed.p, xp.p, H, cfg.vocab_size);
        rope_table_kernel<<<cdiv(L * (HD / 2), 256), 256, 0, s>>>(freqs.p, rope_tab.p, L);
        count_launch(2);
        const size_t kv_layer = (size_t)cfg.max_batch * nkv * cfg.max_context * HD;
        for (int l = 0; l < cfg.num_hidden_layers; ++l) {
            LayerW& Lw = layers[l];
            launch_pdl(add_rmsnorm_kernel, dim3(T), dim3(RN_THREADS), 0, s, xp.p, l == 0 ? (float*)nullptr : yp.p, Lw.ln1.p, xnp.p, H,
                       cfg.rms_norm_eps, (float*)nullptr, (float*)nullptr, 0, PF_HALF, (float*)nullptr, (float*)nullptr, 0);
            pf_gemm(tm_qkv[l], tmp_xn, tc::EPI_STORE, qkvp.p, nullptr, T, QKV_N, H, s);
            PrefillAttnArgs pa{qkvp.p, rope_tab.p, kcache.p + l * kv_layer, vcache.p + l * kv_layer, attnp.p, nq, nkv,
                               cfg.max_context, L, 1.0f / sqrtf((float)HD)};
            const dim3 grid(nkv, B, cdiv(L, PA_QT));
            const size_t sm = pattn_smem(L);
            switch (G) {
                case 1: prefill_attn_kernel<1><<<grid, PA_THREADS, sm, s>>>(pa); break;
                case 2: prefill_attn_kernel<2><<<grid, PA_THREADS, sm, s>>>(pa); break;
                case 3: prefill_attn_kernel<3><<<grid, PA_THREADS, sm, s>>>(pa); break;
                case 4: prefill_attn_kernel<4><<<grid, PA_THREADS, sm, s>>>(pa); break;
                case 6: prefill_attn_kernel<6><<<grid, PA_THREADS, sm, s>>>(pa); break;
                default: prefill_attn_kernel<8><<<grid, PA_THREADS, sm, s>>>(pa); break;
            }
            count_launch();
            pf_gemm(tm_o[l], tmp_attn, tc::EPI_STORE, yp.p, nullptr, T, H, NQ, s);
            launch_pdl(add_rmsnorm_kernel, dim3(T), dim3(RN_THREADS), 0, s, xp.p, yp.p, Lw.ln2.p, xnp.p, H, cfg.rms_norm_eps,
                       (float*)nullptr, (float*)nullptr, 0, PF_HALF, (float*)nullptr, (float*)nullptr, 0);
            pf_gemm(tm_gu[l], tmp_xn, tc::EPI_SWIGLU, nullptr, actp.p, T, 2 * I, H, s);
            pf_gemm(tm_down[l], tmp_act, tc::EPI_STORE, yp.p, nullptr, T, H, I, s);
        }
        gather_last_kernel<<<B, 256, 0, s>>>(xp.p, yp.p, x.p, y.p, pos.p, L, H);
        count_launch();
        B2A_CUDA(cudaGetLastError());
    }

    void set_batch(int B) {
        nb_pad = B <= 1 ? 1 : B <= 2 ? 2 : B <= 4 ? 4 : 8;
    }

    void drop_graphs() {
        if (g_step) { cudaGraphExecDestroy(g_step); g_step = nullptr; }
        if (g_prefill) { cudaGraphExecDestroy(g_prefill); g_prefill = nullptr; }
    }

    static bool same_args(const SampleArgs& a, const SampleArgs& b) {
        return a.V == b.V && a.R == b.R && a.max_tokens == b.max_tokens && a.temperature == b.temperature &&
               a.top_p == b.top_p && a.rep_penalty == b.rep_penalty && a.seed == b.seed && a.mask_eos == b.mask_eos &&
               a.out_tokens == b.out_tokens;
    }

    void capture(int B, const SampleArgs& sa, int L) {
        if (g_step && g_nb == B && same_args(sa, g_args) && g_L == L) return;
        drop_graphs();
        cudaGraph_t g;
        B2A_CUDA(cudaStreamBeginCapture(stream, cudaStreamCaptureModeThreadLocal));
        run_layers(B, stream);
        run_lm_head(B, stream);
        launch_pdl(sample_kernel, dim3(B * SM_CLUSTER), dim3(SM_THREADS), 0, stream, sa);
        B2A_CUDA(cudaStreamEndCapture(stream, &g));
        B2A_CUDA(cudaGraphInstantiate(&g_step, g, 0));
        cudaGraphDestroy(g);
        B2A_CUDA(cudaStreamBeginCapture(stream, cudaStreamCaptureModeThreadLocal));
        run_layers(B, stream);
        launch_pdl(prefill_advance_kernel, dim3(1), dim3(32), 0, stream, ids.p, L, tokens.p, pos.p, B);
        B2A_CUDA(cudaStreamEndCapture(stream, &g));
        B2A_CUDA(cudaGraphInstantiate(&g_prefill, g, 0));
        cudaGraphDestroy(g);
        g_nb = B; g_args = sa; g_L = L;
        launches_step = fused ? launches_layers_fused() + 1 + 1 : 1 + cfg.num_hidden_layers * 7 + 2 + 1;
        launches_prefill = fused ? launches_layers_fused() + 1 : 1 + cfg.num_hidden_layers * 7 + 1;
    }
    int g_L = 0, launches_step = 0, launches_prefill = 0;
};

static std::vector<int> parse_row(const int* row, int n, int crop_after) {
    std::vector<int> r;
    for (int j = crop_after + 1; j < n; ++j)
        if (row[j] != TOK_END_OF_SPEECH) r.push_back(row[j]);
    r.resize((r.size() / 7) * 7);
    for (auto& t : r) t -= TOK_AUDIO_OFFSET;
    return r;
}

static void deinterleave(const int* cl, int n, std::vector<int>& l1, std::vector<int>& l2, std::vector<int>& l3) {
    const int groups = (n + 1) / 7;
    for (int i = 0; i < groups; ++i) {
        const int b = 7 * i;
        l1.push_back(cl[b]);
        l2.push_back(cl[b + 1] - 4096);
        l3.push_back(cl[b + 2] - 2 * 4096);
        l3.push_back(cl[b + 3] - 3 * 4096);
        l2.push_back(cl[b + 4] - 4 * 4096);
        l3.push_back(cl[b + 5] - 5 * 4096);
        l3.push_back(cl[b + 6] - 6 * 4096);
    }
}

static double now_s() {
    return std::chrono::duration<double>(std::chrono::steady_clock::now().time_since_epoch()).count();
}

struct StreamSpec {
    int frames_per_chunk = 0;
    int left_context = 0;
    b2a_audio_cb on_audio = nullptr;
};

static void tts_generate_impl(b2a_tts* h, const int32_t* input_ids, bool ids_on_device, int32_t B, int32_t L,
                              const b2a_gen_params* gp, int32_t* tokens_out, int32_t* n_tokens_out, float* wave_out,
                              bool wave_on_device, int64_t wave_cap, int64_t* wave_len, b2a_gen_info* info,
                              b2a_token_cb on_token, void* user, const StreamSpec& ss = StreamSpec()) {
    B2A_CHECK(h && input_ids && gp, B2A_ERR_INVALID_INPUT, "tts generate: null argument");
    B2A_CHECK(B >= 1 && B <= h->cfg.max_batch, B2A_ERR_INVALID_INPUT, "tts generate: batch exceeds max_batch");
    B2A_CHECK(L >= 1, B2A_ERR_INVALID_INPUT, "tts generate: empty prompt");
    B2A_CHECK(gp->max_tokens >= 1, B2A_ERR_INVALID_INPUT, "tts generate: max_tokens must be positive");
    B2A_CHECK(L + gp->max_tokens <= h->cfg.max_context, B2A_ERR_INVALID_INPUT, "tts generate: prompt + max_tokens exceeds max_context");
    B2A_CHECK(gp->repetition_context_size >= 0 && gp->repetition_context_size <= 64, B2A_ERR_INVALID_INPUT,
              "tts generate: repetition_context_size must be in 0..64");
    B2A_CHECK(gp->temperature >= 0.f && gp->top_p > 0.f, B2A_ERR_INVALID_INPUT, "tts generate: bad sampling parameters");
    if (wave_out) B2A_CHECK(h->snac, B2A_ERR_MODEL_NOT_INITIALIZED, "SNAC model not loaded");
    B2A_CUDA(cudaSetDevice(h->device));
    cudaStream_t s = h->stream;
    h->cancel.store(0);
    h->set_batch(B);
    if (h->trace_on) { h->trace_on = false; h->drop_graphs(); }
    const int MT = gp->max_tokens, R = std::max(1, gp->repetition_context_size);
    h->ids.alloc((size_t)B * L);
    h->out_tokens.alloc((size_t)B * MT);
    h->recent.alloc((size_t)8 * R);
    B2A_CUDA(cudaMemcpyAsync(h->ids.p, input_ids, (size_t)B * L * sizeof(int),
                             ids_on_device ? cudaMemcpyDeviceToDevice : cudaMemcpyHostToDevice, s));
    SampleArgs sa{};
    sa.logits = h->logits.p; sa.probs = h->probs.p; sa.tokens = h->tokens.p; sa.pos = h->pos.p; sa.recent = h->recent.p;
    sa.recent_n = h->recent_n.p; sa.out_tokens = h->out_tokens.p; sa.n_gen = h->n_gen.p; sa.done = h->done.p;
    sa.n_active = h->n_active.p; sa.forced = nullptr; sa.V = h->cfg.vocab_size; sa.R = gp->repetition_context_size > 0 ? R : 0;
    sa.max_tokens = MT; sa.temperature = gp->temperature; sa.top_p = gp->top_p;
    sa.rep_penalty = gp->repetition_context_size > 0 ? gp->repetition_penalty : 1.0f;
    sa.seed = gp->seed; sa.mask_eos = h->bench_mask_eos;
    if (sa.R == 0) { sa.R = 1; }
    h->capture(B, sa, L);

    const double t0 = now_s();
    init_rows_kernel<<<1, 32, 0, s>>>(h->ids.p, L, B, gp->repetition_context_size > 0 ? R : 0, h->tokens.p, h->pos.p, h->recent.p,
                                      h->recent_n.p, h->n_gen.p, h->done.p, h->n_active.p, 0);
    count_launch();
    int steps = 0;
    if (h->can_batch_prefill(L)) {
        h->prefill_batched(B, L, s);
        h->run_lm_head_after_prefill(B, s);
        launch_pdl(sample_kernel, dim3(B * SM_CLUSTER), dim3(SM_THREADS), 0, s, sa);
        steps = 1;
    } else {
        for (int p = 0; p < L - 1; ++p) {
            B2A_CUDA(cudaGraphLaunch(h->g_prefill, s));
            count_launch(h->launches_prefill);
        }
    }
    B2A_CUDA(cudaStreamSynchronize(s));
    const double t1 = now_s();
    bool cancelled = false;
    int streamed = 0;
    std::vector<int> h_tok;
    const bool streaming = ss.frames_per_chunk > 0 && ss.on_audio;
    if (streaming) B2A_CHECK(h->snac && !ids_on_device, B2A_ERR_MODEL_NOT_INITIALIZED, "SNAC model not loaded");
    std::vector<int> emitted(B, 0), s_prompt, s_tok, s_ng(B);
    std::vector<float> s_wave;
    double codec_stream_t = 0;
    if (streaming) { s_prompt.assign(input_ids, input_ids + (size_t)B * L); s_tok.resize((size_t)B * MT); }
    auto emit_audio = [&](bool final_call) {
        const double c0 = now_s();
        B2A_CUDA(cudaMemcpy(s_ng.data(), h->n_gen.p, B * sizeof(int), cudaMemcpyDeviceToHost));
        B2A_CUDA(cudaMemcpy(s_tok.data(), h->out_tokens.p, (size_t)B * MT * sizeof(int), cudaMemcpyDeviceToHost));
        const int64_t hop = b2a_snac_hop_length(h->snac);
        for (int b = 0; b < B; ++b) {
            const int ng = std::min(s_ng[b], MT);
            std::vector<int> all(s_prompt.begin() + (size_t)b * L, s_prompt.begin() + (size_t)(b + 1) * L);
            all.insert(all.end(), s_tok.begin() + (size_t)b * MT, s_tok.begin() + (size_t)b * MT + ng);
            int last = -1;
            for (int j = 0; j < (int)all.size(); ++j) if (all[j] == TOK_START_OF_SPEECH) last = j;
            std::vector<int> cl = parse_row(all.data(), (int)all.size(), last);
            if (h->bench_wrap_codes)
                for (size_t i = 0; i < cl.size(); ++i) cl[i] = ((cl[i] % 4096) + 4096) % 4096 + 4096 * (int)(i % 7);
            const int total = (int)cl.size() / 7;
            while (total - emitted[b] >= ss.frames_per_chunk || (final_call && total > emitted[b])) {
                const int f1 = final_call ? total : emitted[b] + ss.frames_per_chunk;
                const int f0 = std::max(0, emitted[b] - ss.left_context);
                std::vector<int> l1, l2, l3;
                deinterleave(cl.data() + (size_t)f0 * 7, (f1 - f0) * 7, l1, l2, l3);
                const int F = f1 - f0;
                h->d_codes[0].upload(l1.data(), l1.size(), s);
                h->d_codes[1].upload(l2.data(), l2.size(), s);
                h->d_codes[2].upload(l3.data(), l3.size(), s);
                const int64_t T = 4ll * F, wl = T * hop;
                h->d_wave.alloc((size_t)wl);
                const int* dc[3] = {h->d_codes[0].p, h->d_codes[1].p, h->d_codes[2].p};
                B2A_CUDA(cudaStreamSynchronize(s));
                const int32_t st = b2a_snac_decode_dev(h->snac, dc, 1, T, nullptr, 0, gp->seed + (uint64_t)b, h->d_wave.p, s);
                B2A_CHECK(st == B2A_OK, B2A_ERR_AUDIO_DECODING_FAILED, std::string("SNAC decode failed: ") + b2a_last_error());
                const int64_t skip = (int64_t)(emitted[b] - f0) * 4 * hop, n_new = wl - skip;
                s_wave.resize((size_t)n_new);
                B2A_CUDA(cudaMemcpyAsync(s_wave.data(), h->d_wave.p + skip, (size_t)n_new * sizeof(float), cudaMemcpyDeviceToHost, s));
                B2A_CUDA(cudaStreamSynchronize(s));
                emitted[b] = f1;
                ss.on_audio(user, b, s_wave.data(), n_new, (final_call && f1 == total) ? 1 : 0);
            }
        }
        codec_stream_t += now_s() - c0;
    };
    auto stream_tokens = [&]() {
        h_tok.resize((size_t)B * MT);
        std::vector<int> ng(B);
        B2A_CUDA(cudaMemcpy(ng.data(), h->n_gen.p, B * sizeof(int), cudaMemcpyDeviceToHost));
        B2A_CUDA(cudaMemcpy(h_tok.data(), h->out_tokens.p, (size_t)B * MT * sizeof(int), cudaMemcpyDeviceToHost));
        for (int b = 0; b < B; ++b)
            if (ng[b] > streamed) on_token(user, b, streamed, h_tok[(size_t)b * MT + streamed]);
        ++streamed;
    };
    if (steps == 1) {
        if (on_token) stream_tokens();
        B2A_CUDA(cudaMemcpyAsync(h->h_flag.p, h->n_active.p, sizeof(int), cudaMemcpyDeviceToHost, s));
        B2A_CUDA(cudaStreamSynchronize(s));
    }
    const bool pipelined = !on_token && !streaming;
    if (pipelined && !h->ev_poll[0]) { B2A_CUDA(cudaEventCreateWithFlags(&h->ev_poll[0], cudaEventDisableTiming)); B2A_CUDA(cudaEventCreateWithFlags(&h->ev_poll[1], cudaEventDisableTiming)); }
    int slot = 0, pending = -1;
    while (steps < MT && !(steps == 1 && h->h_flag.p[0] <= 0)) {
        const int burst = on_token ? 1 : std::min(streaming ? 7 : 16, MT - steps);
        for (int i = 0; i < burst; ++i) {
            B2A_CUDA(cudaGraphLaunch(h->g_step, s));
            count_launch(h->launches_step);
        }
        steps += burst;
        if (pipelined) {
            B2A_CUDA(cudaMemcpyAsync(h->h_flag.p + 1 + slot, h->n_active.p, sizeof(int), cudaMemcpyDeviceToHost, s));
            B2A_CUDA(cudaEventRecord(h->ev_poll[slot], s));
            if (pending >= 0) {
                B2A_CUDA(cudaEventSynchronize(h->ev_poll[pending]));
                if (h->cancel.load()) { cancelled = true; break; }
                if (h->h_flag.p[1 + pending] <= 0) break;
            }
            pending = slot; slot ^= 1;
            continue;
        }
        B2A_CUDA(cudaMemcpyAsync(h->h_flag.p, h->n_active.p, sizeof(int), cudaMemcpyDeviceToHost, s));
        B2A_CUDA(cudaStreamSynchronize(s));
        if (on_token) stream_tokens();
        if (streaming) emit_audio(false);
        if (h->cancel.load()) { cancelled = true; break; }
        if (h->h_flag.p[0] <= 0) break;
    }
    if (pipelined) { B2A_CUDA(cudaStreamSynchronize(s)); if (h->cancel.load()) cancelled = true; }
    if (streaming && !cancelled) emit_audio(true);
    const double t2 = now_s();
    B2A_CHECK(!cancelled, B2A_ERR_CANCELLED, "generation cancelled");

    std::vector<int> ng(B), toks((size_t)B * MT), prompt((size_t)B * L);
    B2A_CUDA(cudaMemcpyAsync(ng.data(), h->n_gen.p, B * sizeof(int), cudaMemcpyDeviceToHost, s));
    B2A_CUDA(cudaMemcpyAsync(toks.data(), h->out_tokens.p, (size_t)B * MT * sizeof(int), cudaMemcpyDeviceToHost, s));
    B2A_CUDA(cudaMemcpyAsync(prompt.data(), h->ids.p, (size_t)B * L * sizeof(int), cudaMemcpyDeviceToHost, s));
    B2A_CUDA(cudaStreamSynchronize(s));
    int total_gen = 0;
    for (int b = 0; b < B; ++b) {
        ng[b] = std::min(ng[b], MT);
        total_gen += ng[b];
        if (n_tokens_out) n_tokens_out[b] = ng[b];
        if (tokens_out) memcpy(tokens_out + (size_t)b * MT, toks.data() + (size_t)b * MT, ng[b] * sizeof(int));
    }

    double codec_t = 0;
    if (wave_out) {
        const double c0 = now_s();
        std::vector<std::vector<int>> l1(B), l2(B), l3(B);
        std::vector<int> frames(B, 0);
        bool any = false;
        for (int b = 0; b < B; ++b) {
            std::vector<int> all(prompt.begin() + (size_t)b * L, prompt.begin() + (size_t)(b + 1) * L);
            all.insert(all.end(), toks.begin() + (size_t)b * MT, toks.begin() + (size_t)b * MT + ng[b]);
            int last = -1;
            for (int j = 0; j < (int)all.size(); ++j) if (all[j] == TOK_START_OF_SPEECH) last = j;
            std::vector<int> cl = parse_row(all.data(), (int)all.size(), last);
            if (h->bench_wrap_codes)
                for (size_t i = 0; i < cl.size(); ++i) cl[i] = ((cl[i] % 4096) + 4096) % 4096 + 4096 * (int)(i % 7);
            deinterleave(cl.data(), (int)cl.size(), l1[b], l2[b], l3[b]);
            frames[b] = (int)l1[b].size();
            any |= frames[b] > 0;
            if (wave_len) wave_len[b] = 0;
        }
        B2A_CHECK(any, B2A_ERR_GENERATION_FAILED, "No audio codes generated");
        const int64_t hop = b2a_snac_hop_length(h->snac);
        std::vector<bool> used(B, false);
        for (int b = 0; b < B; ++b) {
            if (used[b] || frames[b] == 0) continue;
            std::vector<int> grp;
            for (int c = b; c < B; ++c) if (!used[c] && frames[c] == frames[b]) { grp.push_back(c); used[c] = true; }
            const int F = frames[b], nb = (int)grp.size();
            const int64_t T = 4ll * F, wl = T * hop;
            B2A_CHECK(wl <= wave_cap, B2A_ERR_INVALID_INPUT, "tts generate: wave buffer too small");
            std::vector<int> c0v, c1v, c2v;
            for (int r : grp) { c0v.insert(c0v.end(), l1[r].begin(), l1[r].end()); c1v.insert(c1v.end(), l2[r].begin(), l2[r].end());
                                c2v.insert(c2v.end(), l3[r].begin(), l3[r].end()); }
            h->d_codes[0].upload(c0v.data(), c0v.size(), s);
            h->d_codes[1].upload(c1v.data(), c1v.size(), s);
            h->d_codes[2].upload(c2v.data(), c2v.size(), s);
            h->d_wave.alloc((size_t)nb * wl);
            const int* dc[3] = {h->d_codes[0].p, h->d_codes[1].p, h->d_codes[2].p};
            B2A_CUDA(cudaStreamSynchronize(s));
            const int32_t st = b2a_snac_decode_dev(h->snac, dc, nb, T, nullptr, 0, gp->seed, h->d_wave.p, s);
            B2A_CHECK(st == B2A_OK, B2A_ERR_AUDIO_DECODING_FAILED, std::string("SNAC decode failed: ") + b2a_last_error());
            for (int i = 0; i < nb; ++i) {
                const int r = grp[i];
                B2A_CUDA(cudaMemcpyAsync(wave_out + (size_t)r * wave_cap, h->d_wave.p + (size_t)i * wl, wl * sizeof(float),
                                         wave_on_device ? cudaMemcpyDeviceToDevice : cudaMemcpyDeviceToHost, s));
                if (wave_len) wave_len[r] = wl;
            }
            B2A_CUDA(cudaStreamSynchronize(s));
        }
        codec_t = now_s() - c0;
    }
    if (info) {
        info->prompt_token_count = L;
        info->generation_token_count = total_gen;
        info->prefill_time = t1 - t0;
        info->generate_time = t2 - t1;
        info->tokens_per_second = total_gen / std::max(1e-9, t2 - t1);
        info->codec_time = codec_t + codec_stream_t;
        size_t fr = 0, tot = 0;
        cudaMemGetInfo(&fr, &tot);
        info->peak_memory_gb = (double)(tot - fr) / 1e9;
    }
}

extern "C" {

int32_t b2a_tts_generate_stream(b2a_tts* h, const int32_t* input_ids, int32_t B, int32_t L, const b2a_gen_params* gp,
                                int32_t frames_per_chunk, int32_t left_context_frames, int32_t* tokens_out, int32_t* n_tokens_out,
                                b2a_gen_info* info, b2a_token_cb on_token, b2a_audio_cb on_audio, void* user) {
    return guarded([&] {
        B2A_CHECK(on_audio && frames_per_chunk >= 1 && left_context_frames >= 0, B2A_ERR_INVALID_INPUT,
                  "b2a_tts_generate_stream: needs on_audio, frames_per_chunk >= 1, left_context_frames >= 0");
        StreamSpec ss;
        ss.frames_per_chunk = frames_per_chunk; ss.left_context = left_context_frames; ss.on_audio = on_audio;
        tts_generate_impl(h, input_ids, false, B, L, gp, tokens_out, n_tokens_out, nullptr, false, 0, nullptr, info, on_token, user, ss);
    });
}

int32_t b2a_tts_create(int32_t device, const b2a_llama_config* cfg, const b2a_tensor* tensors, int32_t n, b2a_snac* snac,
                       b2a_tts** out) {
    return guarded([&] {
        B2A_CHECK(out, B2A_ERR_INVALID_INPUT, "b2a_tts_create: null out");
        *out = nullptr;
        B2A_CHECK(cfg && tensors && n > 0, B2A_ERR_MODEL_NOT_INITIALIZED, "b2a_tts_create: missing config or weights");
        TensorTable tt(tensors, n);
        *out = new b2a_tts(device, *cfg, tt, snac);
    });
}

int32_t b2a_tts_create_random(int32_t device, const b2a_llama_config* cfg, float std, uint64_t seed, b2a_snac* snac,
                              b2a_tts** out) {
    return guarded([&] {
        B2A_CHECK(out, B2A_ERR_INVALID_INPUT, "b2a_tts_create_random: null out");
        *out = nullptr;
        B2A_CHECK(cfg && std > 0.f, B2A_ERR_MODEL_NOT_INITIALIZED, "b2a_tts_create_random: missing config");
        *out = new b2a_tts(device, *cfg, std, seed, snac);
    });
}

void* b2a_tts_stream(b2a_tts* h) { return h ? (void*)h->stream : nullptr; }

int32_t b2a_tts_time_steps(b2a_tts* h, int32_t B, int32_t ctx, int32_t iters, float* ms_per_step) {
    return guarded([&] {
        B2A_CHECK(h && ms_per_step && iters > 0, B2A_ERR_INVALID_INPUT, "b2a_tts_time_steps: bad argument");
        B2A_CHECK(B >= 1 && B <= h->cfg.max_batch && ctx >= 0 && ctx + iters < h->cfg.max_context, B2A_ERR_INVALID_INPUT,
                  "b2a_tts_time_steps: batch / context out of range");
        B2A_CUDA(cudaSetDevice(h->device));
        cudaStream_t s = h->stream;
        h->set_batch(B);
        const int MT = iters + 8;
        h->ids.alloc((size_t)B * 1);
        h->out_tokens.alloc((size_t)B * MT);
        h->recent.alloc(8);
        SampleArgs sa{};
        sa.logits = h->logits.p; sa.probs = h->probs.p; sa.tokens = h->tokens.p; sa.pos = h->pos.p; sa.recent = h->recent.p;
        sa.recent_n = h->recent_n.p; sa.out_tokens = h->out_tokens.p; sa.n_gen = h->n_gen.p; sa.done = h->done.p;
        sa.n_active = h->n_active.p; sa.forced = nullptr; sa.V = h->cfg.vocab_size; sa.R = 1; sa.max_tokens = MT;
        sa.temperature = 0.f; sa.top_p = 1.f; sa.rep_penalty = 1.f; sa.seed = 0; sa.mask_eos = 1;
        h->capture(B, sa, 1);
        B2A_CUDA(cudaMemsetAsync(h->ids.p, 0, (size_t)B * sizeof(int), s));
        init_rows_kernel<<<1, 32, 0, s>>>(h->ids.p, 1, B, 0, h->tokens.p, h->pos.p, h->recent.p, h->recent_n.p, h->n_gen.p,
                                          h->done.p, h->n_active.p, ctx);
        count_launch();
        cudaEvent_t e0, e1;
        B2A_CUDA(cudaEventCreate(&e0));
        B2A_CUDA(cudaEventCreate(&e1));
        B2A_CUDA(cudaGraphLaunch(h->g_step, s));
        B2A_CUDA(cudaEventRecord(e0, s));
        for (int i = 0; i < iters - 1; ++i) B2A_CUDA(cudaGraphLaunch(h->g_step, s));
        B2A_CUDA(cudaEventRecord(e1, s));
        B2A_CUDA(cudaStreamSynchronize(s));
        count_launch(h->launches_step * iters);
        float ms = 0.f;
        B2A_CUDA(cudaEventElapsedTime(&ms, e0, e1));
        cudaEventDestroy(e0);
        cudaEventDestroy(e1);
        *ms_per_step = ms / (float)std::max(1, iters - 1);
    });
}

int32_t b2a_tts_prepare_input_ids(const int32_t* const* prompt_ids, const int32_t* lens, int32_t batch, int32_t* out,
                                  int32_t* out_len) {
    return guarded([&] {
        B2A_CHECK(prompt_ids && lens && out_len && batch > 0, B2A_ERR_INVALID_INPUT, "b2a_tts_prepare_input_ids: null argument");
        int mx = 0;
        for (int b = 0; b < batch; ++b) mx = std::max(mx, lens[b]);
        *out_len = mx + 3;
        if (!out) return;
        for (int b = 0; b < batch; ++b) {
            int32_t* r = out + (size_t)b * (mx + 3);
            int j = 0;
            for (; j < mx - lens[b]; ++j) r[j] = TOK_PAD;
            r[j++] = TOK_START_OF_HUMAN;
            for (int i = 0; i < lens[b]; ++i) r[j++] = prompt_ids[b][i];
            r[j++] = TOK_END_OF_TEXT;
            r[j++] = TOK_END_OF_HUMAN;
        }
    });
}

int32_t b2a_tts_prepare_input_ids_ref(const int32_t* const* prompt_ids, const int32_t* lens, int32_t batch, const int32_t* ref_text_ids,
                                      int32_t ref_text_len, const int32_t* ref_code_list, int32_t ref_code_len, int32_t* out,
                                      int32_t* out_len) {
    return guarded([&] {
        B2A_CHECK(prompt_ids && lens && out_len && batch > 0 && ref_text_len >= 0 && ref_code_len >= 0 && (ref_text_ids || ref_text_len == 0) &&
                      (ref_code_list || ref_code_len == 0),
                  B2A_ERR_INVALID_INPUT, "b2a_tts_prepare_input_ids_ref: null argument");
        B2A_CHECK(ref_code_len % 7 == 0, B2A_ERR_INVALID_INPUT, "b2a_tts_prepare_input_ids_ref: ref_code_len must be a multiple of 7");
        for (int i = 0; i < ref_code_len; ++i)
            B2A_CHECK(ref_code_list[i] >= 0 && ref_code_list[i] < 7 * 4096, B2A_ERR_INVALID_INPUT,
                      "b2a_tts_prepare_input_ids_ref: reference code out of range [0, 7 * 4096)");
        int mx = 0;
        for (int b = 0; b < batch; ++b) {
            B2A_CHECK(lens[b] >= 0 && (prompt_ids[b] || lens[b] == 0), B2A_ERR_INVALID_INPUT, "b2a_tts_prepare_input_ids_ref: bad prompt");
            mx = std::max(mx, lens[b]);
        }
        const int ref = 1 + ref_text_len + 2 + 2 + ref_code_len + 2;
        *out_len = mx + ref + 3;
        if (!out) return;
        for (int b = 0; b < batch; ++b) {
            int32_t* r = out + (size_t)b * (mx + ref + 3);
            int j = 0;
            for (; j < mx - lens[b]; ++j) r[j] = TOK_PAD;
            r[j++] = TOK_START_OF_HUMAN;
            for (int i = 0; i < ref_text_len; ++i) r[j++] = ref_text_ids[i];
            r[j++] = TOK_END_OF_TEXT;
            r[j++] = TOK_END_OF_HUMAN;
            r[j++] = TOK_AUDIO_START;
            r[j++] = TOK_START_OF_SPEECH;
            for (int i = 0; i < ref_code_len; ++i) r[j++] = ref_code_list[i] + TOK_AUDIO_OFFSET;
            r[j++] = TOK_END_OF_SPEECH;
            r[j++] = TOK_AUDIO_END;
            r[j++] = TOK_START_OF_HUMAN;
            for (int i = 0; i < lens[b]; ++i) r[j++] = prompt_ids[b][i];
            r[j++] = TOK_END_OF_TEXT;
            r[j++] = TOK_END_OF_HUMAN;
        }
    });
}

int32_t b2a_debug_step_smem(int32_t gqa, int32_t* out) {
    return guarded([&] {
        B2A_CHECK(out && (gqa == 1 || gqa == 2 || gqa == 3 || gqa == 4 || gqa == 6 || gqa == 8), B2A_ERR_INVALID_INPUT,
                  "b2a_debug_step_smem: q heads per kv head must be 1, 2, 3, 4, 6 or 8");
        out[0] = (int32_t)tc::Smem<16>::bytes(b2a_tts::gemm_stages);
        out[1] = (int32_t)tc::SmemSplit::bytes(b2a_tts::splitk_stages, b2a_tts::fused_cluster);
        out[2] = (int32_t)attn_smem_bytes(gqa);
    });
}

int32_t b2a_tts_debug_trace(b2a_tts* h, int32_t enable, int32_t batch, float* out) {
    return guarded([&] {
        B2A_CHECK(h, B2A_ERR_INVALID_INPUT, "b2a_tts_debug_trace: null handle");
        B2A_CUDA(cudaSetDevice(h->device));
        const int H = h->cfg.hidden_size, n = 2 * h->cfg.num_hidden_layers + 1;
        if (out) {
            B2A_CHECK(h->trace.p && batch >= 1 && batch <= 8, B2A_ERR_INVALID_INPUT, "b2a_tts_debug_trace: nothing traced");
            B2A_CUDA(cudaStreamSynchronize(h->stream));
            for (int i = 0; i < n; ++i)
                B2A_CUDA(cudaMemcpy(out + (size_t)i * batch * H, h->trace.p + (size_t)i * 8 * H, (size_t)batch * H * sizeof(float),
                                    cudaMemcpyDeviceToHost));
        }
        h->trace_on = enable != 0;
        if (h->trace_on) { h->trace.alloc((size_t)n * 8 * H); h->drop_graphs(); }
    });
}

int32_t b2a_tts_forward_logits(b2a_tts* h, const int32_t* ids, int32_t B, int32_t L, int32_t reset_cache, float* logits_out) {
    return guarded([&] {
        B2A_CHECK(h && ids && logits_out, B2A_ERR_INVALID_INPUT, "b2a_tts_forward_logits: null argument");
        B2A_CHECK(B >= 1 && B <= h->cfg.max_batch && L >= 1, B2A_ERR_INVALID_INPUT, "b2a_tts_forward_logits: bad batch / length");
        B2A_CUDA(cudaSetDevice(h->device));
        cudaStream_t s = h->stream;
        h->set_batch(B);
        h->drop_graphs();
        std::vector<int> hp(8, 0);
        if (!reset_cache) B2A_CUDA(cudaMemcpy(hp.data(), h->pos.p, 8 * sizeof(int), cudaMemcpyDeviceToHost));
        const int start = reset_cache ? 0 : hp[0];
        B2A_CHECK(start + L <= h->cfg.max_context, B2A_ERR_INVALID_INPUT, "b2a_tts_forward_logits: context overflow");
        h->ids.alloc((size_t)B * L);
        B2A_CUDA(cudaMemcpyAsync(h->ids.p, ids, (size_t)B * L * sizeof(int), cudaMemcpyHostToDevice, s));
        const int V = h->cfg.vocab_size;
        std::vector<int> tk(8, 0), ps(8, -1);
        for (int p = 0; p < L; ++p) {
            for (int b = 0; b < B; ++b) { tk[b] = ids[(size_t)b * L + p]; ps[b] = start + p; }
            B2A_CUDA(cudaMemcpyAsync(h->tokens.p, tk.data(), 8 * sizeof(int), cudaMemcpyHostToDevice, s));
            B2A_CUDA(cudaMemcpyAsync(h->pos.p, ps.data(), 8 * sizeof(int), cudaMemcpyHostToDevice, s));
            h->run_layers(B, s);
            h->run_lm_head(B, s);
            for (int b = 0; b < B; ++b)
                B2A_CUDA(cudaMemcpyAsync(logits_out + ((size_t)b * L + p) * V, h->logits.p + (size_t)b * V, V * sizeof(float),
                                         cudaMemcpyDeviceToHost, s));
            B2A_CUDA(cudaStreamSynchronize(s));
        }
        for (int b = 0; b < B; ++b) ps[b] = start + L;
        B2A_CUDA(cudaMemcpy(h->pos.p, ps.data(), 8 * sizeof(int), cudaMemcpyHostToDevice));
        B2A_CUDA(cudaGetLastError());
    });
}

int32_t b2a_tts_generate(b2a_tts* h, const int32_t* input_ids, int32_t B, int32_t L, const b2a_gen_params* gp,
                         int32_t* tokens_out, int32_t* n_tokens_out, float* wave_out, int64_t wave_cap, int64_t* wave_len,
                         b2a_gen_info* info, b2a_token_cb on_token, void* user) {
    return guarded([&] {
        tts_generate_impl(h, input_ids, false, B, L, gp, tokens_out, n_tokens_out, wave_out, false, wave_cap, wave_len, info,
                          on_token, user);
    });
}

int32_t b2a_tts_generate_dev(b2a_tts* h, const int32_t* d_input_ids, int32_t B, int32_t L, const b2a_gen_params* gp,
                             float* d_wave_out, int64_t wave_cap, int64_t* wave_len, b2a_gen_info* info) {
    return guarded([&] {
        tts_generate_impl(h, d_input_ids, true, B, L, gp, nullptr, nullptr, d_wave_out, true, wave_cap, wave_len, info, nullptr,
                          nullptr);
    });
}

int32_t b2a_tts_set_bench_flags(b2a_tts* h, int32_t mask_eos, int32_t wrap_codes) {
    if (!h) return B2A_ERR_INVALID_INPUT;
    h->bench_mask_eos = mask_eos != 0;
    h->bench_wrap_codes = wrap_codes != 0;
    return B2A_OK;
}

int32_t b2a_tts_cancel(b2a_tts* h) {
    if (!h) return B2A_ERR_INVALID_INPUT;
    h->cancel.store(1);
    return B2A_OK;
}

int32_t b2a_tts_parse_output(const int32_t* tokens, int32_t batch, int32_t n, int32_t* code_lists_out, int32_t* code_lens) {
    return guarded([&] {
        B2A_CHECK(tokens && code_lists_out && code_lens && batch > 0 && n >= 0, B2A_ERR_INVALID_INPUT, "b2a_tts_parse_output: bad argument");
        int last = -1;
        for (int i = 0; i < batch; ++i)
            for (int j = 0; j < n; ++j)
                if (tokens[(size_t)i * n + j] == TOK_START_OF_SPEECH) last = j;
        for (int i = 0; i < batch; ++i) {
            std::vector<int> r = parse_row(tokens + (size_t)i * n, n, last);
            code_lens[i] = (int)r.size();
            memcpy(code_lists_out + (size_t)i * n, r.data(), r.size() * sizeof(int));
        }
    });
}

int32_t b2a_tts_deinterleave(const int32_t* code_list, int32_t n, int32_t* c0, int32_t* c1, int32_t* c2, int32_t* n_frames) {
    return guarded([&] {
        B2A_CHECK(code_list && c0 && c1 && c2 && n_frames && n >= 0, B2A_ERR_INVALID_INPUT, "b2a_tts_deinterleave: bad argument");
        const int groups = (n + 1) / 7;
        B2A_CHECK(groups * 7 <= n, B2A_ERR_INVALID_INPUT, "b2a_tts_deinterleave: code list must hold whole 7-token frames");
        std::vector<int> l1, l2, l3;
        deinterleave(code_list, n, l1, l2, l3);
        memcpy(c0, l1.data(), l1.size() * sizeof(int));
        memcpy(c1, l2.data(), l2.size() * sizeof(int));
        memcpy(c2, l3.data(), l3.size() * sizeof(int));
        *n_frames = groups;
    });
}

int32_t b2a_tts_interleave(const int32_t* c0, const int32_t* c1, const int32_t* c2, int32_t n_frames, int32_t* cl) {
    return guarded([&] {
        B2A_CHECK(c0 && c1 && c2 && cl && n_frames >= 0, B2A_ERR_INVALID_INPUT, "b2a_tts_interleave: bad argument");
        for (int i = 0; i < n_frames; ++i) {
            int32_t* o = cl + 7 * i;
            o[0] = c0[i];
            o[1] = c1[2 * i] + 4096;
            o[2] = c2[4 * i] + 2 * 4096;
            o[3] = c2[4 * i + 1] + 3 * 4096;
            o[4] = c1[2 * i + 1] + 4 * 4096;
            o[5] = c2[4 * i + 2] + 5 * 4096;
            o[6] = c2[4 * i + 3] + 6 * 4096;
        }
    });
}

void b2a_tts_destroy(b2a_tts* h) { delete h; }

}

namespace b2a {

__global__ void q3_gather_kernel(const bf16* __restrict__ table, int rows, const int* __restrict__ ids, int id_stride, int id_col,
                                 float* __restrict__ dst, int H, int* pos, int pos_value) {
    const int b = blockIdx.x;
    if (!pos) pdl_trigger();
    pdl_wait();
    int t = ids[b * id_stride + id_col];
    t = min(max(t, 0), rows - 1);
    for (int i = threadIdx.x; i < H; i += blockDim.x) dst[(long long)b * H + i] = __bfloat162float(table[(long long)t * H + i]);
    if (pos && threadIdx.x == 0) pos[b] = pos_value;
}
__global__ void q3_copy_rows_kernel(const float* __restrict__ src, long long src_stride, float* __restrict__ dst, int H, int* pos, int pos_value) {
    const int b = blockIdx.x;
    if (!(pos && pos_value >= 0)) pdl_trigger();
    pdl_wait();
    for (int i = threadIdx.x; i < H; i += blockDim.x) dst[(long long)b * H + i] = src[(long long)b * src_stride + i];
    if (pos && pos_value >= 0 && threadIdx.x == 0) pos[b] = pos_value;
}
__global__ void q3_linear_kernel(const bf16* __restrict__ W, const float* __restrict__ bias, const float* __restrict__ x, float* __restrict__ y,
                                 int O, int K, int silu) {
    const int o = blockIdx.x * (blockDim.x >> 5) + (threadIdx.x >> 5), t = blockIdx.y, lane = threadIdx.x & 31;
    if (o >= O) return;
    float acc = 0.f;
    for (int k = lane; k < K; k += 32) acc = fmaf(__bfloat162float(W[(long long)o * K + k]), x[(long long)t * K + k], acc);
    acc = warp_sum(acc);
    if (lane == 0) {
        acc += bias ? bias[o] : 0.f;
        y[(long long)t * O + o] = silu ? acc / (1.0f + __expf(-acc)) : acc;
    }
}

struct Q3Feedback {
    const bf16* codec_emb; int codec_rows;
    const bf16* const* cp_emb;
    int cp_rows;
    const int* codes;
    const float* trailing;
    const int* n_trailing;
    int n_max;
    const float* pad;
    float* x_in;
    int* talker_pos;
    int* row_frame;
    int* out_codes;
    int* n_frames; int* done; int* n_active;
    int G, H, max_tokens, eos, mask_eos;
};
__global__ void q3_feedback_kernel(Q3Feedback a) {
    const int b = blockIdx.x;
    pdl_wait();
    const int f = a.row_frame[b];
    const float* text = f < a.n_trailing[b] ? a.trailing + ((long long)b * a.n_max + f) * a.H : a.pad;
    const int* c = a.codes + b * a.G;
    for (int i = threadIdx.x; i < a.H; i += blockDim.x) {
        float e = __bfloat162float(a.codec_emb[(long long)min(max(c[0], 0), a.codec_rows - 1) * a.H + i]);
        for (int g = 1; g < a.G; ++g) e += __bfloat162float(a.cp_emb[g - 1][(long long)min(max(c[g], 0), a.cp_rows - 1) * a.H + i]);
        a.x_in[(long long)b * a.H + i] = text[i] + e;
    }
    __syncthreads();
    if (threadIdx.x == 0) {
        a.row_frame[b] = f + 1;
        a.talker_pos[b] += 1;
        if (!a.done[b]) {
            if (c[0] == a.eos && !a.mask_eos) { a.done[b] = 1; atomicSub(a.n_active, 1); }
            else {
                const int n = a.n_frames[b];
                if (n < a.max_tokens) for (int g = 0; g < a.G; ++g) a.out_codes[((long long)b * a.max_tokens + n) * a.G + g] = c[g];
                a.n_frames[b] = n + 1;
                if (n + 1 >= a.max_tokens) { a.done[b] = 1; atomicSub(a.n_active, 1); }
            }
        }
    }
}
__global__ void q3_init_rows_kernel(int B, int L, int* talker_pos, int* row_frame, int* n_frames, int* done, int* n_active, unsigned* seen, int words) {
    const int b = threadIdx.x;
    if (b == 0) *n_active = B;
    if (b < 8) { talker_pos[b] = L - 1; row_frame[b] = 0; n_frames[b] = 0; done[b] = b < B ? 0 : 1; }
    for (int i = threadIdx.x; i < 8 * words; i += blockDim.x) seen[i] = 0u;
}
__global__ void q3_mask_eos_kernel(float* logits, int V, int eos) {
    if (threadIdx.x == 0 && eos >= 0 && eos < V) logits[(long long)blockIdx.x * V + eos] = -INFINITY;
}

}

struct b2a_qwen3_talker {
    int device;
    b2a_qwen3_talker_config cfg;
    b2a_tts* talker = nullptr;
    b2a_tts* pred = nullptr;
    cudaStream_t stream = nullptr;
    DBuf<bf16> codec_emb, text_emb, fc1_w, fc2_w;
    DBuf<float> fc1_b, fc2_b;
    std::vector<DBuf<bf16>> cp_emb, cp_head;
    std::vector<CUtensorMap> tm_cp_head;
    int cp_head_rows = 128;
    DBuf<const bf16*> cp_emb_ptrs;
    DBuf<float> x_in, hid, px, trailing, pad, embeds, tmp_a, tmp_b;
    DBuf<int> codes, out_codes, n_frames, done, n_active, row_frame, n_trailing, ids;
    DBuf<unsigned> seen;
    HBuf<int> h_flag;
    cudaGraphExec_t g_frame = nullptr;
    b2a_qwen3_gen_params g_params{};
    int g_B = 0, g_max_tokens = 0, g_nmax = 0, g_mask = -1;
    const float* g_trailing = nullptr;
    int launches_frame = 0;
    int bench_mask_eos = 0;
    std::atomic<int> cancel{0};

    ~b2a_qwen3_talker() {
        if (g_frame) cudaGraphExecDestroy(g_frame);
        delete pred;
        delete talker;
    }
    int G() const { return cfg.num_code_groups; }
    int H() const { return cfg.hidden_size; }

    static b2a_llama_config stack_cfg(const b2a_qwen3_talker_config& c, bool predictor) {
        b2a_llama_config l{};
        l.hidden_size = predictor ? c.cp_hidden_size : c.hidden_size;
        l.num_hidden_layers = predictor ? c.cp_num_hidden_layers : c.num_hidden_layers;
        l.intermediate_size = predictor ? c.cp_intermediate_size : c.intermediate_size;
        l.num_attention_heads = predictor ? c.cp_num_attention_heads : c.num_attention_heads;
        l.num_key_value_heads = predictor ? c.cp_num_key_value_heads : c.num_key_value_heads;
        l.head_dim = predictor ? c.cp_head_dim : c.head_dim;
        l.vocab_size = predictor ? c.cp_vocab_size : c.vocab_size;
        l.rms_norm_eps = predictor ? c.cp_rms_norm_eps : c.rms_norm_eps;
        l.rope_theta = predictor ? c.cp_rope_theta : c.rope_theta;
        l.rope_factor = 1.0f; l.rope_low_freq_factor = 1.0f; l.rope_high_freq_factor = 4.0f; l.rope_old_context_len = 8192.0f;
        l.tie_word_embeddings = 0;
        l.max_batch = c.max_batch;
        l.max_context = predictor ? std::max(32, c.num_code_groups + 8) : c.max_context;
        return l;
    }
    static StackSpec talker_spec() { StackSpec s; s.prefix = "model."; s.qk_norm = true; s.has_embed = false; s.head = "codec_head.weight"; s.has_head = true; return s; }
    static StackSpec pred_spec() { StackSpec s; s.prefix = "code_predictor.model."; s.qk_norm = true; s.has_embed = false; s.has_head = false; return s; }

    void check() {
        const b2a_qwen3_talker_config& c = cfg;
        B2A_CHECK(c.head_dim == HD && c.cp_head_dim == HD, B2A_ERR_INVALID_INPUT, "qwen3 talker: head_dim must be 128");
        B2A_CHECK(c.cp_hidden_size == c.hidden_size, B2A_ERR_INVALID_INPUT,
                  "qwen3 talker: code predictor hidden size must equal the talker's (small_to_mtp_projection is not implemented)");
        B2A_CHECK(c.vocab_size >= 1 && c.vocab_size <= q3s::SLOTS && c.cp_vocab_size >= 1 && c.cp_vocab_size <= q3s::SLOTS, B2A_ERR_INVALID_INPUT,
                  "qwen3 talker: codec vocabularies must be <= 4096");
        B2A_CHECK(c.num_code_groups >= 2 && c.num_code_groups <= 32, B2A_ERR_INVALID_INPUT, "qwen3 talker: num_code_groups must be in 2..32");
        B2A_CHECK(c.max_batch >= 1 && c.max_batch <= 8, B2A_ERR_INVALID_INPUT, "qwen3 talker: max_batch must be in 1..8");
    }
    void alloc_state() {
        stream = talker->stream;
        const int Hh = H();
        x_in.alloc((size_t)8 * Hh); hid.alloc((size_t)8 * Hh); px.alloc((size_t)8 * Hh); pad.alloc(Hh);
        B2A_CUDA(cudaMemset(x_in.p, 0, (size_t)8 * Hh * sizeof(float)));
        B2A_CUDA(cudaMemset(hid.p, 0, (size_t)8 * Hh * sizeof(float)));
        B2A_CUDA(cudaMemset(px.p, 0, (size_t)8 * Hh * sizeof(float)));
        codes.alloc((size_t)8 * G()); n_frames.alloc(8); done.alloc(8); n_active.alloc(1); row_frame.alloc(8); n_trailing.alloc(8);
        B2A_CUDA(cudaMemset(codes.p, 0, (size_t)8 * G() * sizeof(int)));
        seen.alloc((size_t)8 * cdiv(cfg.vocab_size, 32));
        h_flag.alloc(16);
        std::vector<const bf16*> ptrs;
        for (auto& e : cp_emb) ptrs.push_back(e.p);
        cp_emb_ptrs.upload(ptrs.data(), ptrs.size());
        if (pred->use_tc) {
            tm_cp_head.clear();
            cp_head_rows = b2a_tts::pick_tile_rows(cfg.cp_vocab_size, pred->num_sms);
            for (auto& hd : cp_head) tm_cp_head.push_back(tc::make_tmap_bf16(hd.p, cfg.cp_vocab_size, Hh, cp_head_rows));
        } else tm_cp_head.resize(cp_head.size());
        talker->x_ext = x_in.p; talker->normed_out = hid.p;
        pred->x_ext = px.p;
        talker->set_batch(8); pred->set_batch(8);
        B2A_CUDA(cudaDeviceSynchronize());
    }

    b2a_qwen3_talker(int dev, const b2a_qwen3_talker_config& c, const TensorTable& tt) : device(dev), cfg(c) {
// ... 278 lines not shown
```

### mlx-audio-swift_b200/csrc/tc_gemm.cu

```cuda
#define B2A_TC_GEMM_IMPL
#include "common.cuh"
#include "tc_gemm.cuh"

namespace b2a {
namespace tc {

typedef CUresult (*EncodeTiledFn)(CUtensorMap*, CUtensorMapDataType, cuuint32_t, void*, const cuuint64_t*, const cuuint64_t*,
                                  const cuuint32_t*, const cuuint32_t*, CUtensorMapInterleave, CUtensorMapSwizzle,
                                  CUtensorMapL2promotion, CUtensorMapFloatOOBfill);

static EncodeTiledFn encode_fn() {
    static EncodeTiledFn fn = nullptr;
    if (!fn) {
        void* p = nullptr;
        cudaDriverEntryPointQueryResult q;
        B2A_CUDA(cudaGetDriverEntryPoint("cuTensorMapEncodeTiled", &p, cudaEnableDefault, &q));
        B2A_CHECK(p && q == cudaDriverEntryPointSuccess, B2A_ERR_CUDA, "cuTensorMapEncodeTiled is not available in this driver");
        fn = (EncodeTiledFn)p;
    }
    return fn;
}

static CUtensorMapDataType type16(int f16) { return f16 ? CU_TENSOR_MAP_DATA_TYPE_FLOAT16 : CU_TENSOR_MAP_DATA_TYPE_BFLOAT16; }

CUtensorMap make_tmap_bf16(const void* base, long long rows, long long cols, int box_rows, int f16) {
    B2A_CHECK(cols % 8 == 0 && ((uintptr_t)base & 15) == 0, B2A_ERR_INVALID_INPUT, "TMA: tensor must be 16-byte aligned with cols % 8 == 0");
    CUtensorMap m;
    const cuuint64_t dims[2] = {(cuuint64_t)cols, (cuuint64_t)rows};
    const cuuint64_t strides[1] = {(cuuint64_t)cols * 2};
    const cuuint32_t box[2] = {(cuuint32_t)BK, (cuuint32_t)box_rows};
    const cuuint32_t estr[2] = {1, 1};
    const CUresult r = encode_fn()(&m, type16(f16), 2, const_cast<void*>(base), dims, strides, box, estr,
                                   CU_TENSOR_MAP_INTERLEAVE_NONE, CU_TENSOR_MAP_SWIZZLE_128B, CU_TENSOR_MAP_L2_PROMOTION_L2_256B,
                                   CU_TENSOR_MAP_FLOAT_OOB_FILL_NONE);
    B2A_CHECK(r == CUDA_SUCCESS, B2A_ERR_CUDA, "cuTensorMapEncodeTiled failed (" + std::to_string((int)r) + ")");
    return m;
}

CUtensorMap make_tmap_f16_3d(const void* base, long long d0, long long d1, long long d2, int b0, int b1) {
    B2A_CHECK(b0 * 2 == 128 && d0 % 8 == 0 && ((uintptr_t)base & 15) == 0, B2A_ERR_INVALID_INPUT, "TMA: bad 3-D fp16 tensor");
    CUtensorMap m;
    const cuuint64_t dims[3] = {(cuuint64_t)d0, (cuuint64_t)d1, (cuuint64_t)d2};
    const cuuint64_t strides[2] = {(cuuint64_t)d0 * 2, (cuuint64_t)d0 * (cuuint64_t)d1 * 2};
    const cuuint32_t box[3] = {(cuuint32_t)b0, (cuuint32_t)b1, 1};
    const cuuint32_t estr[3] = {1, 1, 1};
    const CUresult r = encode_fn()(&m, CU_TENSOR_MAP_DATA_TYPE_FLOAT16, 3, const_cast<void*>(base), dims, strides, box, estr,
                                   CU_TENSOR_MAP_INTERLEAVE_NONE, CU_TENSOR_MAP_SWIZZLE_128B, CU_TENSOR_MAP_L2_PROMOTION_L2_256B,
                                   CU_TENSOR_MAP_FLOAT_OOB_FILL_NONE);
    B2A_CHECK(r == CUDA_SUCCESS, B2A_ERR_CUDA, "cuTensorMapEncodeTiled (3-D fp16) failed (" + std::to_string((int)r) + ")");
    return m;
}

CUtensorMap make_tmap_planes(const void* base, int C, long long Ttot, int B, int box_frames, int f16) {
    B2A_CHECK(C % 8 == 0 && ((uintptr_t)base & 15) == 0 && Ttot >= 1 && B >= 1, B2A_ERR_INVALID_INPUT,
              "TMA: activation planes must be 16-byte aligned with channels % 8 == 0");
    CUtensorMap m;
    const cuuint64_t dims[4] = {(cuuint64_t)C, (cuuint64_t)Ttot, (cuuint64_t)B, 2};
    const cuuint64_t strides[3] = {(cuuint64_t)C * 2, (cuuint64_t)Ttot * C * 2, (cuuint64_t)B * Ttot * C * 2};
    const cuuint32_t box[4] = {(cuuint32_t)BK, (cuuint32_t)box_frames, 1, 2};
    const cuuint32_t estr[4] = {1, 1, 1, 1};
    const CUresult r = encode_fn()(&m, type16(f16), 4, const_cast<void*>(base), dims, strides, box, estr,
                                   CU_TENSOR_MAP_INTERLEAVE_NONE, CU_TENSOR_MAP_SWIZZLE_128B, CU_TENSOR_MAP_L2_PROMOTION_L2_256B,
                                   CU_TENSOR_MAP_FLOAT_OOB_FILL_NONE);
    B2A_CHECK(r == CUDA_SUCCESS, B2A_ERR_CUDA, "cuTensorMapEncodeTiled (rank 4) failed (" + std::to_string((int)r) + ")");
    return m;
}

template <int BN>
void launch(const CUtensorMap& tmA, const CUtensorMap& tmB, const Args& a, int ctas, int n_tiles, cudaStream_t s) {
    B2A_CHECK(a.stages >= 1 && a.stages <= Smem<BN>::max_stages(), B2A_ERR_INVALID_INPUT, "tc_gemm: ring depth does not fit in shared memory");
    B2A_CHECK(a.epi_partial < 0 || (a.part_ws && a.part_cnt && a.part_slots >= stream_k_slots(a.m_tiles, a.k_blocks, ctas)),
              B2A_ERR_INVALID_INPUT, "tc_gemm: stream-K workspace missing or too small");
    launch_pdl(tc_gemm_kernel<BN>, dim3(ctas, n_tiles), dim3(Cfg<BN>::NTHREADS), Smem<BN>::bytes(a.stages), s, tmA, tmB, a);
}
template void launch<16>(const CUtensorMap&, const CUtensorMap&, const Args&, int, int, cudaStream_t);
template void launch<32>(const CUtensorMap&, const CUtensorMap&, const Args&, int, int, cudaStream_t);
template void launch<128>(const CUtensorMap&, const CUtensorMap&, const Args&, int, int, cudaStream_t);

void launch_splitk(const CUtensorMap& tmA, const CUtensorMap& tmB, const SplitArgs& a, int m_tiles, int cluster, cudaStream_t s) {
    B2A_CHECK(SmemSplit::bytes(a.stages, cluster) <= 227 * 1024, B2A_ERR_INVALID_INPUT, "tc_gemm: split-K ring does not fit in shared memory");
    cudaLaunchConfig_t cfg{};
    cfg.gridDim = dim3((unsigned)(m_tiles * cluster)); cfg.blockDim = dim3(THREADS);
    cfg.dynamicSmemBytes = SmemSplit::bytes(a.stages, cluster); cfg.stream = s;
    cudaLaunchAttribute at[2];
    at[0].id = cudaLaunchAttributeProgrammaticStreamSerialization;
    at[0].val.programmaticStreamSerializationAllowed = pdl_enabled() ? 1 : 0;
    at[1].id = cudaLaunchAttributeClusterDimension;
    at[1].val.clusterDim.x = (unsigned)cluster; at[1].val.clusterDim.y = 1; at[1].val.clusterDim.z = 1;
    cfg.attrs = at; cfg.numAttrs = 2;
    B2A_CUDA(cudaLaunchKernelEx(&cfg, tc_gemm_splitk_kernel, tmA, tmB, a));
    count_launch();
}

void set_attributes() {
    B2A_CUDA(cudaFuncSetAttribute(tc_gemm_splitk_kernel, cudaFuncAttributeMaxDynamicSharedMemorySize, 227 * 1024));
    B2A_CUDA(cudaFuncSetAttribute(tc_gemm_kernel<16>, cudaFuncAttributeMaxDynamicSharedMemorySize, 227 * 1024));
    B2A_CUDA(cudaFuncSetAttribute(tc_gemm_splitk_kernel, cudaFuncAttributePreferredSharedMemoryCarveout, cudaSharedmemCarveoutMaxShared));
    B2A_CUDA(cudaFuncSetAttribute(tc_gemm_kernel<16>, cudaFuncAttributePreferredSharedMemoryCarveout, cudaSharedmemCarveoutMaxShared));
    B2A_CUDA(cudaFuncSetAttribute(tc_gemm_kernel<32>, cudaFuncAttributeMaxDynamicSharedMemorySize, 227 * 1024));
    B2A_CUDA(cudaFuncSetAttribute(tc_gemm_kernel<128>, cudaFuncAttributeMaxDynamicSharedMemorySize, 227 * 1024));
}

}
}


extern "C" int32_t b2a_tc_gemm_epilogue_test(const void* W, const void* X, void* out, int32_t M, int32_t N, int32_t K, int32_t bn,
                                             int32_t epi, int32_t split, int32_t hilo, int32_t ctas, const float* bias, int32_t act,
                                             int32_t tile_rows, int32_t lo_rows, const float* rstd_ss, int32_t rstd_parts,
                                             float rstd_eps, int32_t stages, void* stream) {
    using namespace b2a;
    using namespace b2a::tc;
    return guarded([&] {
        B2A_CHECK(W && X && out && (bn == 16 || bn == 32 || bn == 128) && K % BK == 0 && M > 0 && N > 0 && ctas > 0, B2A_ERR_INVALID_INPUT,
                  "b2a_tc_gemm_epilogue_test: bad argument");
        B2A_CHECK(epi == EPI_STORE || epi == EPI_SWIGLU || epi == EPI_STORE_BF16 || epi == EPI_ADD, B2A_ERR_INVALID_INPUT,
                  "b2a_tc_gemm_epilogue_test: unknown epilogue");
        B2A_CHECK(act == ACT_NONE || act == ACT_GELU, B2A_ERR_INVALID_INPUT, "b2a_tc_gemm_epilogue_test: unknown activation");
        B2A_CHECK(!split || epi == EPI_STORE || epi == EPI_ADD, B2A_ERR_INVALID_INPUT,
                  "b2a_tc_gemm_epilogue_test: stream-K partial tiles are summed into fp32 outputs only");
        B2A_CHECK(!split || act == ACT_NONE, B2A_ERR_INVALID_INPUT, "b2a_tc_gemm_epilogue_test: GELU of a partial K range is not the GELU of the sum");
        B2A_CHECK(!split || tile_rows == 0, B2A_ERR_INVALID_INPUT, "b2a_tc_gemm_epilogue_test: tile_rows is a whole-tile option");
        B2A_CHECK(tile_rows == 0 || (tile_rows % 8 == 0 && tile_rows >= 8 && tile_rows <= BM), B2A_ERR_INVALID_INPUT,
                  "b2a_tc_gemm_epilogue_test: tile_rows must be a multiple of 8 in [8, 128]");
        B2A_CHECK(!lo_rows || (hilo && (epi == EPI_SWIGLU || epi == EPI_STORE_BF16)), B2A_ERR_INVALID_INPUT,
                  "b2a_tc_gemm_epilogue_test: hi/lo outputs need hi/lo inputs and a bf16 epilogue");
        B2A_CHECK(epi != EPI_SWIGLU || M % 2 == 0, B2A_ERR_INVALID_INPUT, "b2a_tc_gemm_epilogue_test: SwiGLU needs (gate, up) row pairs");
        B2A_CHECK(!rstd_ss || (bn == 16 && hilo && N <= 8 && rstd_parts >= 1), B2A_ERR_INVALID_INPUT,
                  "b2a_tc_gemm_epilogue_test: the fused RMSNorm scale is a BN = 16 hi/lo option");
        require_device(0);
        set_attributes();
        const int n_tiles = hilo ? cdiv(N, bn / 2) : cdiv(N, bn);
        B2A_CHECK(n_tiles <= 65535, B2A_ERR_INVALID_INPUT, "b2a_tc_gemm_epilogue_test: too many tokens");
        const int x_rows = hilo ? n_tiles * bn : N;
        const int TR = tile_rows > 0 ? tile_rows : BM;
        CUtensorMap ta = make_tmap_bf16(W, M, K, TR), tb = make_tmap_bf16(X, x_rows, K, bn);
        Args a{};
        a.out_f32 = (float*)out; a.out_bf16 = (__nv_bfloat16*)out; a.M = M; a.N = N; a.K = K;
        a.ldo = epi == EPI_SWIGLU ? M / 2 : M;
        a.tile_rows = tile_rows; a.m_tiles = cdiv(M, TR); a.k_blocks = K / BK;
        const int max_st = bn == 16 ? Smem<16>::max_stages() : bn == 32 ? Smem<32>::max_stages() : Smem<128>::max_stages();
        a.stages = stages > 0 ? stages : max_st;
        a.epi_full = epi; a.epi_partial = split ? EPI_PARTIAL : -1; a.hilo = hilo;
        a.bias = bias; a.act = act;
        a.lo_rows = lo_rows ? bn / 2 : 0;
        a.rstd_ss = rstd_ss; a.rstd_parts = rstd_parts; a.rstd_inv_h = 1.0f / (float)K; a.rstd_eps = rstd_eps;
        DBuf<float> ws;
        DBuf<unsigned> cnt;
        if (split) {
            a.part_slots = stream_k_slots(a.m_tiles, a.k_blocks, ctas);
            ws.alloc((size_t)n_tiles * a.m_tiles * a.part_slots * bn * BM);
            cnt.alloc((size_t)n_tiles * a.m_tiles);
            B2A_CUDA(cudaMemset(cnt.p, 0, (size_t)n_tiles * a.m_tiles * sizeof(unsigned)));
            a.part_ws = ws.p; a.part_cnt = cnt.p;
        }
        if (bn == 16) launch<16>(ta, tb, a, ctas, n_tiles, (cudaStream_t)stream);
        else if (bn == 32) launch<32>(ta, tb, a, ctas, n_tiles, (cudaStream_t)stream);
        else launch<128>(ta, tb, a, ctas, n_tiles, (cudaStream_t)stream);
        B2A_CUDA(cudaGetLastError());
        B2A_CUDA(cudaStreamSynchronize((cudaStream_t)stream));
    });
}

extern "C" int32_t b2a_tc_gemm_test(const void* W, const void* X, void* out, int32_t M, int32_t N, int32_t K, int32_t bn,
                                    int32_t epi, int32_t split, int32_t hilo, int32_t ctas, void* stream) {
    const int32_t lo_rows = hilo && (epi == b2a::tc::EPI_SWIGLU || epi == b2a::tc::EPI_STORE_BF16);
    return b2a_tc_gemm_epilogue_test(W, X, out, M, N, K, bn, epi, split, hilo, ctas, nullptr, b2a::tc::ACT_NONE, 0, lo_rows, nullptr, 0,
                                     0.f, 0, stream);
}

extern "C" int32_t b2a_tc_gemm_splitk_test(const void* W, const void* X, float* h, const float* gain, void* xn, float* ss, int32_t M,
                                           int32_t N, int32_t K, int32_t cluster, int32_t stages, void* stream) {
    using namespace b2a;
    using namespace b2a::tc;
    return guarded([&] {
        B2A_CHECK(W && X && h && gain && xn && ss && M > 0 && M % 8 == 0 && K > 0 && K % BK == 0 && N >= 1 && N <= 8 && stages >= 1,
                  B2A_ERR_INVALID_INPUT, "b2a_tc_gemm_splitk_test: bad argument");
        B2A_CHECK(cluster >= 1 && cluster <= SPLIT_MAX_CLUSTER && cluster <= K / BK, B2A_ERR_INVALID_INPUT,
                  "b2a_tc_gemm_splitk_test: cluster must be in [1, min(8, K / 64)]");
        require_device(0);
        set_attributes();
        CUtensorMap ta = make_tmap_bf16(W, M, K, BM), tb = make_tmap_bf16(X, 16, K, 16);
        SplitArgs a{};
        a.M = M; a.N = N; a.K = K; a.k_blocks = K / BK; a.stages = stages;
        a.h = h; a.gain = gain; a.xn = (__nv_bfloat16*)xn; a.ss = ss;
        launch_splitk(ta, tb, a, cdiv(M, BM), cluster, (cudaStream_t)stream);
        B2A_CUDA(cudaGetLastError());
        B2A_CUDA(cudaStreamSynchronize((cudaStream_t)stream));
    });
}
```

### mlx-audio-swift_b200/csrc/tc_gemm.cuh

```cuda
#pragma once
#include <cuda.h>
#include <cuda_bf16.h>
#include <cuda_runtime.h>
#include <stdint.h>

namespace b2a {
namespace tc {

constexpr int BM = 128, BK = 64, UMMA_K = 16;
constexpr int THREADS = 160;
enum : int { EPI_STORE = 0, EPI_PARTIAL = 1, EPI_SWIGLU = 2, EPI_STORE_BF16 = 3, EPI_ADD = 4 };
enum : int { ACT_NONE = 0, ACT_GELU = 1 };

struct Args {
    float* out_f32;
    __nv_bfloat16* out_bf16;
    int M, N, K;
    int ldo;
    int m_tiles, k_blocks;
    int stages;
    int epi_full;
    int epi_partial;
    int hilo;
    const float* bias;
// ... 125 lines not shown
}

__device__ __forceinline__ uint64_t make_smem_desc(uint32_t saddr) {
    return (uint64_t)((saddr & 0x3FFFF) >> 4) | ((uint64_t)1 << 16) | ((uint64_t)(1024 >> 4) << 32) | ((uint64_t)1 << 62);
}

template <int N>
__device__ __forceinline__ void store_frag(float* s, int ld, const float (&d)[N / 2], int r0, int c0) {
    const int t = threadIdx.x & 127, r = r0 + (t >> 5) * 16 + ((t & 31) >> 2), c = c0 + 2 * (t & 3);
#pragma unroll
    for (int i = 0; i < N / 8; ++i) {
        *reinterpret_cast<float2*>(s + (size_t)r * ld + c + 8 * i) = make_float2(d[4 * i], d[4 * i + 1]);
        *reinterpret_cast<float2*>(s + (size_t)(r + 8) * ld + c + 8 * i) = make_float2(d[4 * i + 2], d[4 * i + 3]);
    }
}
__device__ __forceinline__ void ld_acc16(const float* p, float* v) {
#pragma unroll
    for (int i = 0; i < 4; ++i) {
        const float4 f = reinterpret_cast<const float4*>(p)[i];
        v[4 * i] = f.x; v[4 * i + 1] = f.y; v[4 * i + 2] = f.z; v[4 * i + 3] = f.w;
    }
}
__device__ __forceinline__ void named_sync(int id, int threads) { asm volatile("bar.sync %0, %1;" ::"r"(id), "r"(threads) : "memory"); }

template <class I>
__device__ __forceinline__ void store_hilo(__nv_bfloat16* base, long long ld, I t, long long col, float v, int half) {
    const __nv_bfloat16 hi = __float2bfloat16_rn(v);
    const long long r = (long long)(t / half) * 2 * half + (t % half);
    base[r * ld + col] = hi;
    base[(r + half) * ld + col] = __float2bfloat16_rn(v - __bfloat162float(hi));
}

template <int BN>
struct Cfg {
    static constexpr int EPI_WARPS = BN >= 128 ? 16 : 4;
    static constexpr int WG = EPI_WARPS / 4;
    static constexpr int RB = WG == 1 ? 2 : 1;
    static constexpr int WN = WG == 1 ? BN : BN * 2 / WG;
    static constexpr int LD = BN + 4;
    static constexpr int NTHREADS = 32 * EPI_WARPS + 32;
};

template <int BN>
struct Smem {
    static constexpr int A_BYTES = BM * BK * 2, B_BYTES = BN * BK * 2, STAGE = A_BYTES + B_BYTES;
    static constexpr int ACC_BYTES = BM * Cfg<BN>::LD * 4;
    static int max_stages() { return (226 * 1024 - 256 - ACC_BYTES) / STAGE; }
    static size_t bytes(int stages) { return (size_t)stages * STAGE + ACC_BYTES + 256; }
};
__device__ __forceinline__ void check_smem_base(const void* base) {
    if (threadIdx.x == 0 && (smem_u32(base) & 1023u)) __trap();
}

template <int BN>
__global__ void __launch_bounds__(Cfg<BN>::NTHREADS, Cfg<BN>::EPI_WARPS > 4 ? 1 : 2)
tc_gemm_kernel(const __grid_constant__ CUtensorMap tmA, const __grid_constant__ CUtensorMap tmB, const __grid_constant__ Args a) {
    using S = Smem<BN>;
    using C = Cfg<BN>;
    extern __shared__ __align__(1024) uint8_t smem[];
    float* sacc = reinterpret_cast<float*>(smem + (size_t)a.stages * S::STAGE);
    uint64_t* full = reinterpret_cast<uint64_t*>(smem + (size_t)a.stages * S::STAGE + S::ACC_BYTES);
    uint64_t* empty = full + a.stages;
    int* s_reduce = reinterpret_cast<int*>(empty + a.stages);

    const int warp = threadIdx.x >> 5, lane = threadIdx.x & 31;
    const int n0 = blockIdx.y * BN;
    const int TR = a.tile_rows > 0 ? a.tile_rows : BM;
    const uint32_t stage_tx = (uint32_t)(TR * BK * 2 + S::B_BYTES);
    asm volatile("griddepcontrol.launch_dependents;" ::: "memory");

    check_smem_base(smem);
    if (threadIdx.x == 0) {
        tma_prefetch_desc(&tmA);
        tma_prefetch_desc(&tmB);
        for (int i = 0; i < a.stages; ++i) { mbar_init(&full[i], 1); mbar_init(&empty[i], C::EPI_WARPS); }
        fence_barrier_init();
    }
    __syncthreads();

    const long long units = (long long)a.m_tiles * a.k_blocks;
    long long u0, u1;
    if (a.epi_partial >= 0) {
        u0 = units * blockIdx.x / gridDim.x;
        u1 = units * (blockIdx.x + 1) / gridDim.x;
    } else {
        u0 = ((long long)a.m_tiles * blockIdx.x / gridDim.x) * a.k_blocks;
        u1 = ((long long)a.m_tiles * (blockIdx.x + 1) / gridDim.x) * a.k_blocks;
    }

    if (warp == C::EPI_WARPS) {
        if (lane == 0) {
            const int npre = (int)min((long long)a.stages, u1 - u0);
            for (int i = 0; i < npre; ++i) {
                const long long u = u0 + i;
                const int mt = (int)(u / a.k_blocks), kb = (int)(u - (long long)mt * a.k_blocks);
                mbar_arrive_expect_tx(&full[i], stage_tx);
                tma_load_2d(smem + (size_t)i * S::STAGE, &tmA, &full[i], kb * BK, mt * TR);
            }
            asm volatile("griddepcontrol.wait;" ::: "memory");
            for (int i = 0; i < npre; ++i) {
                const long long u = u0 + i;
                const int mt = (int)(u / a.k_blocks), kb = (int)(u - (long long)mt * a.k_blocks);
                tma_load_2d(smem + (size_t)i * S::STAGE + S::A_BYTES, &tmB, &full[i], kb * BK, n0);
            }
            int stage = npre == a.stages ? 0 : npre;
            uint32_t phase = npre == a.stages ? 1 : 0;
            for (long long u = u0 + npre; u < u1; ++u) {
                const int mt = (int)(u / a.k_blocks), kb = (int)(u - (long long)mt * a.k_blocks);
                mbar_wait(&empty[stage], phase ^ 1);
                uint8_t* sa = smem + (size_t)stage * S::STAGE;
                mbar_arrive_expect_tx(&full[stage], stage_tx);
                tma_load_2d(sa, &tmA, &full[stage], kb * BK, mt * TR);
                tma_load_2d(sa + S::A_BYTES, &tmB, &full[stage], kb * BK, n0);
                if (++stage == a.stages) { stage = 0; phase ^= 1; }
            }
        }
    } else {
        const int q = warp & 3;
        constexpr int NCG = C::EPI_WARPS / 4;
        const int cg = warp >> 2, wg = warp >> 2;
        const int row_blk = C::WG == 1 ? 0 : (wg & 1), col_blk = C::WG == 1 ? 0 : (wg >> 1);
        int stage = 0; uint32_t phase = 0;
        float acc[C::RB][C::WN / 2];
#pragma unroll
        for (int rb = 0; rb < C::RB; ++rb)
#pragma unroll
            for (int i = 0; i < C::WN / 2; ++i) acc[rb][i] = 0.f;
        long long u = u0;
        float rstd[8];
        bool have_rstd = false;
        if (BN == 16 && a.rstd_ss) {
            asm volatile("griddepcontrol.wait;" ::: "memory");
            float t = 0.f;
            for (int p0 = 0; p0 < a.rstd_parts; p0 += 4) {
                const int p = p0 + (lane >> 3);
                if (p < a.rstd_parts) t += a.rstd_ss[p * 8 + (lane & 7)];
            }
            t += __shfl_xor_sync(0xffffffffu, t, 8);
            t += __shfl_xor_sync(0xffffffffu, t, 16);
            const float rs = rsqrtf(t * a.rstd_inv_h + a.rstd_eps);
#pragma unroll
            for (int j = 0; j < 8; ++j) rstd[j] = __shfl_sync(0xffffffffu, rs, j);
            have_rstd = true;
        }
        while (u < u1) {
            const int mt = (int)(u / a.k_blocks);
            const long long seg_begin = u;
            const long long seg_end = min(u1, (long long)(mt + 1) * a.k_blocks);
            u = seg_end;
            const bool whole = (seg_begin == (long long)mt * a.k_blocks) && (seg_end == (long long)(mt + 1) * a.k_blocks);
            const int epi = whole ? a.epi_full : a.epi_partial;
            for (long long uu = seg_begin; uu < seg_end; ++uu) {
                mbar_wait(&full[stage], phase);
                const uint32_t sa = smem_u32(smem + (size_t)stage * S::STAGE);
                wg_fence();
#pragma unroll
                for (int k = 0; k < BK / UMMA_K; ++k) {
#pragma unroll
                    for (int rb = 0; rb < C::RB; ++rb) {
                        const uint64_t ad = make_smem_desc(sa + (uint32_t)((row_blk + rb) * 64 * 128)) + (uint64_t)(2 * k);
                        const uint64_t bd = make_smem_desc(sa + S::A_BYTES + (uint32_t)(col_blk * C::WN * 128)) + (uint64_t)(2 * k);
                        wgmma_bf16<C::WN>(acc[rb], ad, bd, (uu == seg_begin && k == 0) ? 0u : 1u);
                    }
                }
                wg_commit();
                wg_wait0();
                __syncwarp();
                if (lane == 0) mbar_arrive(&empty[stage]);
                if (++stage == a.stages) { stage = 0; phase ^= 1; }
            }
#pragma unroll
            for (int rb = 0; rb < C::RB; ++rb) wg_fence_operand(acc[rb]);
            named_sync(1, 32 * C::EPI_WARPS);
#pragma unroll
            for (int rb = 0; rb < C::RB; ++rb) store_frag<C::WN>(sacc, C::LD, acc[rb], (row_blk + rb) * 64, col_blk * C::WN);
            named_sync(1, 32 * C::EPI_WARPS);
            const int m = mt * TR + q * 32 + lane;
            const float* arow = sacc + (size_t)(q * 32 + lane) * C::LD;
            const long long units = (long long)a.m_tiles * a.k_blocks;
            const int first_owner = stream_k_owner((long long)mt * a.k_blocks, units, gridDim.x);
            const size_t tile_id = (size_t)blockIdx.y * a.m_tiles + mt;
            float* ws_tile = whole ? nullptr : a.part_ws + (tile_id * a.part_slots + (blockIdx.x - first_owner)) * BN * BM;
            constexpr int HALF = BN / 2;
            constexpr int CH = (BN == 16) ? 8 : 16;
            const int n_cols = a.hilo ? HALF : BN;
            const int ntok0 = a.hilo ? (int)blockIdx.y * HALF : n0;
            const bool m_ok = m < a.M && q * 32 + lane < TR;
            const int cstep = (BN == 16 && !a.hilo) ? 16 : CH;
            for (int c0 = cg * cstep; c0 < n_cols; c0 += cstep * NCG) {
                float v[16];
                if (BN == 16) {
                    ld_acc16(arow, v);
                    if (a.hilo) {
#pragma unroll
                        for (int j = 0; j < 8; ++j) v[j] += v[j + 8];
                    }
                    if (have_rstd) {
#pragma unroll
                        for (int j = 0; j < 8; ++j) v[j] *= rstd[j];
                    }
                } else {
                    ld_acc16(arow + c0, v);
                    if (a.hilo) {
                        float w[16];
                        ld_acc16(arow + c0 + HALF, w);
#pragma unroll
                        for (int j = 0; j < 16; ++j) v[j] += w[j];
                    }
                }
                const int jn = (BN == 16 && !a.hilo) ? 16 : CH;
                if (a.bias || a.act) {
                    const float bv = (a.bias && m_ok && (whole || seg_begin == (long long)mt * a.k_blocks)) ? a.bias[m] : 0.f;
#pragma unroll
                    for (int j = 0; j < 16; ++j) {
                        float t = v[j] + bv;
                        if (a.act == ACT_GELU) t = 0.5f * t * (1.0f + erff(t * 0.70710678118654752f));
                        v[j] = t;
                    }
                }
                const int nt = ntok0 + c0;
                const int nvalid = min(jn, a.N - nt);
                if (epi == EPI_SWIGLU) {
                    const long long hrow = a.lo_rows ? (long long)(nt / HALF) * BN + (nt % HALF) : nt;
                    __nv_bfloat16* ph = a.out_bf16 + hrow * a.ldo + (m >> 1);
                    const long long lo_off = (long long)HALF * a.ldo;
#pragma unroll
                    for (int j = 0; j < 16; ++j) {
                        if (j >= jn) break;
                        const float other = __shfl_xor_sync(0xffffffffu, v[j], 1);
                        if (j < nvalid && m_ok && (lane & 1) == 0) {
                            const float r = v[j] / (1.0f + __expf(-v[j])) * other;
                            const __nv_bfloat16 hi = __float2bfloat16_rn(r);
                            ph[0] = hi;
                            if (a.lo_rows) ph[lo_off] = __float2bfloat16_rn(r - __bfloat162float(hi));
                        }
                        ph += a.ldo;
                    }
                } else if (epi == EPI_STORE_BF16) {
                    const long long hrow = a.lo_rows ? (long long)(nt / HALF) * BN + (nt % HALF) : nt;
                    __nv_bfloat16* ph = a.out_bf16 + hrow * a.ldo + m;
                    const long long lo_off = (long long)HALF * a.ldo;
#pragma unroll
                    for (int j = 0; j < 16; ++j) {
                        if (j >= jn) break;
                        if (j < nvalid && m_ok) {
                            const __nv_bfloat16 hi = __float2bfloat16_rn(v[j]);
                            ph[0] = hi;
                            if (a.lo_rows) ph[lo_off] = __float2bfloat16_rn(v[j] - __bfloat162float(hi));
                        }
                        ph += a.ldo;
                    }
                } else if (epi == EPI_PARTIAL) {
                    float* pw = ws_tile + (size_t)(nt - ntok0) * BM + q * 32 + lane;
#pragma unroll
                    for (int j = 0; j < 16; ++j)
                        if (j < jn) pw[(size_t)j * BM] = v[j];
                } else {
                    float* pf = a.out_f32 + (long long)nt * a.ldo + m;
                    if (epi == EPI_ADD) {
#pragma unroll
                        for (int j = 0; j < 16; ++j)
                            if (j < jn && j < nvalid && m_ok) v[j] += pf[(long long)j * a.ldo];
                    }
#pragma unroll
                    for (int j = 0; j < 16; ++j) {
                        if (j >= jn) break;
                        if (j < nvalid && m_ok) {
                            pf[0] = v[j];
                        }
                        pf += a.ldo;
                    }
                }
            }
            if (!whole) {
                const int n_parts = stream_k_owner((long long)(mt + 1) * a.k_blocks - 1, units, gridDim.x) - first_owner + 1;
                const unsigned my_kb = (unsigned)(seg_end - seg_begin);
                __threadfence();
                named_sync(1, 32 * C::EPI_WARPS);
                if (threadIdx.x == 0) *s_reduce = atomicAdd(&a.part_cnt[tile_id], my_kb) + my_kb == (unsigned)a.k_blocks;
                named_sync(1, 32 * C::EPI_WARPS);
                if (*s_reduce) {
                    __threadfence();
                    const float* base = a.part_ws + tile_id * a.part_slots * BN * BM;
                    constexpr int NT = 32 * C::EPI_WARPS, PER = 16;
                    const int n_el = n_cols * BM;
                    for (int i0 = 0; i0 < n_el; i0 += NT * PER) {
                        float sum[PER];
#pragma unroll
                        for (int e = 0; e < PER; ++e) sum[e] = 0.f;
                        for (int p = 0; p < n_parts; ++p) {
                            const long long c = first_owner + p;
                            if (units * (c + 1) / gridDim.x == units * c / gridDim.x) continue;
                            const float* slot = base + (size_t)p * BN * BM;
#pragma unroll
                            for (int e = 0; e < PER; ++e) {
                                const int i = i0 + threadIdx.x + e * NT;
                                if (i < n_el) sum[e] += __ldcg(slot + i);
                            }
                        }
#pragma unroll
                        for (int e = 0; e < PER; ++e) {
                            const int i = i0 + threadIdx.x + e * NT;
                            const int tcol = i / BM, r = i - tcol * BM, mm = mt * BM + r, tok = ntok0 + tcol;
                            if (i < n_el && tok < a.N && mm < a.M) a.out_f32[(long long)tok * a.ldo + mm] += sum[e];
                        }
                    }
                    if (threadIdx.x == 0) a.part_cnt[tile_id] = 0;
                }
            }
        }
    }
}

struct SplitArgs {
    int M, N, K;
    int k_blocks, stages;
    float* h;
    const float* gain;
    __nv_bfloat16* xn;
    float* ss;
    const float* rstd_ss;
    int rstd_parts;
    float rstd_inv_h, rstd_eps;
};

__device__ __forceinline__ uint32_t cluster_ctarank() { uint32_t r; asm volatile("mov.u32 %0, %%cluster_ctarank;" : "=r"(r)); return r; }
__device__ __forceinline__ uint32_t cluster_nctarank() { uint32_t r; asm volatile("mov.u32 %0, %%cluster_nctarank;" : "=r"(r)); return r; }
__device__ __forceinline__ void cluster_sync_all() {
    asm volatile("barrier.cluster.arrive.release.aligned;" ::: "memory");
    asm volatile("barrier.cluster.wait.acquire.aligned;" ::: "memory");
}
__device__ __forceinline__ uint32_t map_to_rank(uint32_t saddr, uint32_t rank) {
    uint32_t r;
    asm volatile("mapa.shared::cluster.u32 %0, %1, %2;" : "=r"(r) : "r"(saddr), "r"(rank));
    return r;
}
__device__ __forceinline__ void st_cluster_f4(uint32_t addr, float a, float b, float c, float d) {
    asm volatile("st.shared::cluster.v4.f32 [%0], {%1, %2, %3, %4};" ::"r"(addr), "f"(a), "f"(b), "f"(c), "f"(d) : "memory");
}

constexpr int SPLIT_MAX_CLUSTER = 8;
struct SmemSplit {
    static constexpr int STAGE = Smem<16>::STAGE;
    static constexpr int PART_BYTES = BM * 8 * 4;
    static_assert(Smem<16>::ACC_BYTES <= STAGE, "the staged accumulator lives in ring stage 0");
    static size_t bytes(int stages, int cluster) { return (size_t)stages * STAGE + (size_t)(cluster - 1) * PART_BYTES + 512; }
};

#ifdef B2A_TC_GEMM_IMPL
__global__ void __launch_bounds__(THREADS, 2)
tc_gemm_splitk_kernel(const __grid_constant__ CUtensorMap tmA, const __grid_constant__ CUtensorMap tmB, SplitArgs a) {
    using S = Smem<16>;
    constexpr int BN = 16;
    extern __shared__ __align__(1024) uint8_t smem[];
    const uint32_t C = cluster_nctarank(), rank = cluster_ctarank();
    float* part = reinterpret_cast<float*>(smem + (size_t)a.stages * S::STAGE);
    float* sacc = reinterpret_cast<float*>(smem);
    uint64_t* full = reinterpret_cast<uint64_t*>(part + (size_t)(C - 1) * BM * 8);
    uint64_t* empty = full + a.stages;
    float* s_red = reinterpret_cast<float*>(empty + a.stages);

    const int warp = threadIdx.x >> 5, lane = threadIdx.x & 31;
    const int mt = blockIdx.x / C;
    const int kb0 = (int)((long long)a.k_blocks * rank / C), kb1 = (int)((long long)a.k_blocks * (rank + 1) / C);
    asm volatile("griddepcontrol.launch_dependents;" ::: "memory");

    check_smem_base(smem);
    if (threadIdx.x == 0) {
        tma_prefetch_desc(&tmA);
        tma_prefetch_desc(&tmB);
        for (int i = 0; i < a.stages; ++i) { mbar_init(&full[i], 1); mbar_init(&empty[i], 4); }
        fence_barrier_init();
    }
    __syncthreads();

    if (warp == 4) {
        if (lane == 0) {
            const int n = kb1 - kb0, npre = min(a.stages, n);
            for (int i = 0; i < npre; ++i) {
                mbar_arrive_expect_tx(&full[i], S::STAGE);
                tma_load_2d(smem + (size_t)i * S::STAGE, &tmA, &full[i], (kb0 + i) * BK, mt * BM);
            }
            asm volatile("griddepcontrol.wait;" ::: "memory");
            for (int i = 0; i < npre; ++i) tma_load_2d(smem + (size_t)i * S::STAGE + S::A_BYTES, &tmB, &full[i], (kb0 + i) * BK, 0);
            int stage = npre == a.stages ? 0 : npre;
            uint32_t phase = npre == a.stages ? 1 : 0;
            for (int i = npre; i < n; ++i) {
                mbar_wait(&empty[stage], phase ^ 1);
                uint8_t* sa = smem + (size_t)stage * S::STAGE;
                mbar_arrive_expect_tx(&full[stage], S::STAGE);
                tma_load_2d(sa, &tmA, &full[stage], (kb0 + i) * BK, mt * BM);
                tma_load_2d(sa + S::A_BYTES, &tmB, &full[stage], (kb0 + i) * BK, 0);
                if (++stage == a.stages) { stage = 0; phase ^= 1; }
            }
        }
    }
    float acc[8], hold[8];
    float g = 0.f;
    const int q = warp & 3, row = q * 32 + lane;
    const int m = mt * BM + row;
    const bool m_ok = m < a.M;
    if (warp < 4) {
        if (rank == 0) {
            asm volatile("griddepcontrol.wait;" ::: "memory");
            g = m_ok ? a.gain[m] : 0.f;
#pragma unroll
            for (int j = 0; j < 8; ++j) hold[j] = (j < a.N && m_ok) ? a.h[(long long)j * a.M + m] : 0.f;
        }
        float d[2][8];
#pragma unroll
        for (int rb = 0; rb < 2; ++rb)
#pragma unroll
            for (int i = 0; i < 8; ++i) d[rb][i] = 0.f;
        int stage = 0; uint32_t phase = 0;
        for (int kb = kb0; kb < kb1; ++kb) {
            mbar_wait(&full[stage], phase);
            const uint32_t sa = smem_u32(smem + (size_t)stage * S::STAGE);
            wg_fence();
#pragma unroll
            for (int k = 0; k < BK / UMMA_K; ++k) {
#pragma unroll
                for (int rb = 0; rb < 2; ++rb)
                    wgmma_bf16<BN>(d[rb], make_smem_desc(sa + (uint32_t)(rb * 64 * 128)) + (uint64_t)(2 * k),
                                   make_smem_desc(sa + S::A_BYTES) + (uint64_t)(2 * k), (kb == kb0 && k == 0) ? 0u : 1u);
            }
            wg_commit();
            wg_wait0();
            __syncwarp();
            if (lane == 0) mbar_arrive(&empty[stage]);
            if (++stage == a.stages) { stage = 0; phase ^= 1; }
        }
        named_sync(3, 128);
#pragma unroll
        for (int rb = 0; rb < 2; ++rb) {
            wg_fence_operand(d[rb]);
            store_frag<BN>(sacc, Cfg<BN>::LD, d[rb], rb * 64, 0);
        }
        named_sync(3, 128);
        float v[16];
        ld_acc16(sacc + (size_t)row * Cfg<BN>::LD, v);
#pragma unroll
        for (int j = 0; j < 8; ++j) acc[j] = v[j] + v[j + 8];
        if (rank != 0) {
            const uint32_t dst = map_to_rank(smem_u32(part + ((size_t)(rank - 1) * BM + row) * 8), 0);
            st_cluster_f4(dst, acc[0], acc[1], acc[2], acc[3]);
            st_cluster_f4(dst + 16, acc[4], acc[5], acc[6], acc[7]);
        }
    }
    __syncwarp();
    cluster_sync_all();
    if (rank == 0 && warp < 4) {
        for (uint32_t r = 1; r < C; ++r) {
            const float4 p0 = *reinterpret_cast<const float4*>(part + ((size_t)(r - 1) * BM + row) * 8);
            const float4 p1 = *reinterpret_cast<const float4*>(part + ((size_t)(r - 1) * BM + row) * 8 + 4);
            acc[0] += p0.x; acc[1] += p0.y; acc[2] += p0.z; acc[3] += p0.w;
            acc[4] += p1.x; acc[5] += p1.y; acc[6] += p1.z; acc[7] += p1.w;
        }
        const int w4 = warp;
        if (a.rstd_ss) {
            if (w4 == 0 && lane < 8) {
                float t = 0.f;
                for (int p = 0; p < a.rstd_parts; ++p) t += a.rstd_ss[p * 8 + lane];
                s_red[32 + lane] = rsqrtf(t * a.rstd_inv_h + a.rstd_eps);
            }
            asm volatile("bar.sync 1, 128;" ::: "memory");
#pragma unroll
            for (int j = 0; j < 8; ++j) acc[j] *= s_red[32 + j];
        }
        float sq[8];
#pragma unroll
        for (int j = 0; j < 8; ++j) {
            float hv = 0.f;
            if (j < a.N && m_ok) {
                hv = hold[j] + acc[j];
                a.h[(long long)j * a.M + m] = hv;
                const float t = hv * g;
                const __nv_bfloat16 hi = __float2bfloat16_rn(t);
                a.xn[(long long)j * a.M + m] = hi;
                a.xn[(long long)(8 + j) * a.M + m] = __float2bfloat16_rn(t - __bfloat162float(hi));
            }
            sq[j] = hv * hv;
        }
#pragma unroll
        for (int j = 0; j < 8; ++j) {
#pragma unroll
            for (int o = 16; o; o >>= 1) sq[j] += __shfl_xor_sync(0xffffffffu, sq[j], o);
        }
        if (lane == 0) {
#pragma unroll
            for (int j = 0; j < 8; ++j) s_red[w4 * 8 + j] = sq[j];
        }
        asm volatile("bar.sync 2, 128;" ::: "memory");
        if (w4 == 0 && lane < 8) a.ss[mt * 8 + lane] = s_red[lane] + s_red[8 + lane] + s_red[16 + lane] + s_red[24 + lane];
    }
}
#endif

CUtensorMap make_tmap_bf16(const void* base, long long rows, long long cols, int box_rows, int f16 = 0);
CUtensorMap make_tmap_f16_3d(const void* base, long long d0, long long d1, long long d2, int b0, int b1);
CUtensorMap make_tmap_planes(const void* base, int C, long long Ttot, int B, int box_frames, int f16);

template <int BN>
void launch(const CUtensorMap& tmA, const CUtensorMap& tmB, const Args& a, int ctas, int n_tiles, cudaStream_t s);

void launch_splitk(const CUtensorMap& tmA, const CUtensorMap& tmB, const SplitArgs& a, int m_tiles, int cluster, cudaStream_t s);

void set_attributes();

}
}
```

Measured before the change: 29.79.

## Run QKV projection as clustered split-K GEMM with stream-K partitioning

```diff
diff --git a/include/b200audio_internal.h b/include/b200audio_internal.h
--- a/include/b200audio_internal.h
+++ b/include/b200audio_internal.h
@@ -35,6 +35,9 @@
                          int32_t split, int32_t hilo, int32_t ctas, void* stream);
 int32_t b2a_tc_gemm_splitk_test(const void* W, const void* X, float* h, const float* gain, void* xn, float* ss, int32_t M, int32_t N,
                                 int32_t K, int32_t cluster, int32_t stages, void* stream);
+int32_t b2a_tc_gemm_splitk_store_test(const void* W, const void* X, float* out, const float* rstd_ss, int32_t rstd_parts, float rstd_eps,
+                                      int32_t M, int32_t N, int32_t K, int32_t cluster, int32_t sk_ctas, int32_t stages, void* stream);
+int32_t b2a_debug_qkv_split(int32_t m_tiles, int32_t k_blocks, int32_t* out);
 int32_t b2a_mha_tc_test(const float* qkv, void* out, int32_t B, int32_t T, int32_t nh, void* stream);
 int32_t b2a_wh_decode_attn_test(int32_t self_attn, const float* q, const float* kv, const int32_t* pos, void* kcache, void* vcache,
                                 void* out, float* part_o, float* part_ml, int32_t* counters, int32_t B, int32_t nh, int32_t max_t,
diff --git a/mlx-audio-swift_b200/_ffi.py b/mlx-audio-swift_b200/_ffi.py
--- a/mlx-audio-swift_b200/_ffi.py
+++ b/mlx-audio-swift_b200/_ffi.py
@@ -208,6 +208,8 @@
     "b2a_tc_gemm_epilogue_test": (C.c_int32, [_P, _P, _P] + [C.c_int32] * 8 + [_P, C.c_int32, C.c_int32, C.c_int32, _P, C.c_int32,
                                                                              C.c_float, C.c_int32, _P]),
     "b2a_tc_gemm_splitk_test": (C.c_int32, [_P, _P, _P, _P, _P, _P] + [C.c_int32] * 5 + [_P]),
+    "b2a_tc_gemm_splitk_store_test": (C.c_int32, [_P, _P, _P, _P, C.c_int32, C.c_float] + [C.c_int32] * 6 + [_P]),
+    "b2a_debug_qkv_split": (C.c_int32, [C.c_int32, C.c_int32, C.POINTER(C.c_int32)]),
     "b2a_mha_tc_test": (C.c_int32, [_P, _P, C.c_int32, C.c_int32, C.c_int32, _P]),
     "b2a_wh_decode_attn_test": (C.c_int32, [C.c_int32, _P, _P, _P, _P, _P, _P, _P, _P, _P, C.c_int32, C.c_int32, C.c_int32, _P]),
     "b2a_conv_gemm_test": (C.c_int32, [_P, C.c_int32, C.c_int32, _P, C.c_int32, C.c_int32, _P, _P, _P, C.c_int32, _P, C.c_int32, _P,
diff --git a/mlx-audio-swift_b200/csrc/llama.cu b/mlx-audio-swift_b200/csrc/llama.cu
--- a/mlx-audio-swift_b200/csrc/llama.cu
+++ b/mlx-audio-swift_b200/csrc/llama.cu
@@ -68,9 +68,8 @@
 constexpr int RN_THREADS = 1024, RN_MAXV = 8;
 __global__ void __launch_bounds__(RN_THREADS)
 add_rmsnorm_kernel(float* __restrict__ x, float* __restrict__ delta, const float* __restrict__ w,
-                   bf16* __restrict__ xn, int H, float eps, float* __restrict__ trace, float* __restrict__ zero_ptr,
-                   int zero_n, int half, float* __restrict__ normed = nullptr, float* __restrict__ ss_out = nullptr,
-                   int ss_parts = 0) {
+                   bf16* __restrict__ xn, int H, float eps, float* __restrict__ trace, int half,
+                   float* __restrict__ normed = nullptr, float* __restrict__ ss_out = nullptr, int ss_parts = 0) {
     __shared__ float red[RN_THREADS / 32];
     const int b = blockIdx.x, tid = threadIdx.x;
     pdl_trigger();
@@ -107,8 +106,6 @@
             if (normed) normed[(long long)b * H + i] = o;
         }
     }
-    if (zero_ptr)
-        for (int i = tid; i < zero_n; i += RN_THREADS) zero_ptr[(long long)b * zero_n + i] = 0.f;
 }
 
 constexpr int GV_MAX_THREADS = 256;
@@ -208,7 +205,6 @@
     const float* qnorm;
     const float* knorm;
     float qk_eps;
-    int zero_qkv;
 };
 
 template <int G>
@@ -408,11 +404,6 @@
         }
     }
     cluster.sync();
-    if (a.zero_qkv && rank == 0) {
-        float* wrow = const_cast<float*>(row);
-        for (int i = tid; i < G * HD; i += AT_THREADS) wrow[(long long)h * G * HD + i] = 0.f;
-        if (tid < HD) { wrow[(a.nq + h) * HD + tid] = 0.f; wrow[(a.nq + a.nkv + h) * HD + tid] = 0.f; }
-    }
     if (rank == 0 && tid < HD) {
         _Pragma("unroll") for (int g = 0; g < G; ++g) {
             const float M1 = xml[g], L1 = xml[MAXG + g], O1 = xo[g * HD + tid];
@@ -847,6 +838,8 @@
     cudaEvent_t ev_poll[2] = {nullptr, nullptr};
     bool fused = false;
     static constexpr int fused_cluster = 5;
+    int qkv_cluster = 0;
+    int qkv_sk_ctas = 0;
     static constexpr int gemm_stages = 6, splitk_stages = 5;
     int fused_parts = 0;
     DBuf<float> ss_a, ss_b;
@@ -977,6 +970,9 @@
         use_batched_prefill = !(envp && std::string(envp) == "step");
         if (use_tc) {
             tc::set_attributes();
+            if (fused) {
+                qkv_cluster = pick_qkv_cluster(cdiv(NQ + 2 * NKV, tc::BM), H / tc::BK, num_sms, &qkv_sk_ctas);
+            }
             for (auto& L : layers) {
                 tm_qkv.push_back(tc::make_tmap_bf16(L.wqkv.p, NQ + 2 * NKV, H, tc::BM));
                 tm_o.push_back(tc::make_tmap_bf16(L.wo.p, H, NQ, tc::BM));
@@ -1192,19 +1188,34 @@
         a.rstd_ss = nullptr; a.rstd_parts = 0; a.rstd_inv_h = 0.f; a.rstd_eps = 0.f;
         tc::launch_splitk(tmW, tmX, a, cdiv(M, tc::BM), std::max(1, std::min(fused_cluster, a.k_blocks)), s);
     }
+    void qkv_gemm(int layer, int B, cudaStream_t s) {
+        const int H = cfg.hidden_size, M = (cfg.num_attention_heads + 2 * cfg.num_key_value_heads) * HD;
+        if (qkv_cluster < 1) { tc_gemm(tm_qkv[layer], tmx_xn, OP_QKV, qkv.p, nullptr, B, M, H, s, ss_b.p); return; }
+        tc::SplitArgs a{};
+        a.M = M; a.N = B; a.K = H; a.k_blocks = H / tc::BK; a.stages = splitk_stages; a.sk_ctas = qkv_sk_ctas;
+        a.out = qkv.p;
+        a.rstd_ss = ss_b.p; a.rstd_parts = fused_parts; a.rstd_inv_h = 1.0f / (float)H; a.rstd_eps = cfg.rms_norm_eps;
+        tc::launch_splitk(tm_qkv[layer], tmx_xn, a, cdiv(M, tc::BM), qkv_cluster, s);
+    }
+    static int pick_qkv_cluster(int m_tiles, int k_blocks, int sms, int* sk_ctas) {
+        *sk_ctas = (int)std::min<long long>(sms, (long long)m_tiles * k_blocks);
+        const int c = tc::stream_k_slots(m_tiles, k_blocks, *sk_ctas);
+        if (c > tc::SPLIT_MAX_CLUSTER) return 0;
+        return m_tiles <= tc::splitk_active_clusters(c, tc::SmemSplit::bytes(splitk_stages, c)) ? c : 0;
+    }
     void run_layers_fused(int B, cudaStream_t s) {
         const int H = cfg.hidden_size, I = cfg.intermediate_size, nq = cfg.num_attention_heads, nkv = cfg.num_key_value_heads;
-        const int NQ = nq * HD, NKV = nkv * HD, L = cfg.num_hidden_layers;
+        const int NQ = nq * HD, L = cfg.num_hidden_layers;
         if (x_ext) launch_pdl(ext_embed_kernel, dim3(B), dim3(256), 0, s, x_ext, x.p, y.p, H);
         else launch_pdl(embed_kernel, dim3(B), dim3(256), 0, s, tokens.p, embed.p, x.p, y.p, H, cfg.vocab_size);
         launch_pdl(add_rmsnorm_kernel, dim3(B), dim3(RN_THREADS), 0, s, x.p, (float*)nullptr, layers[0].ln1.p, xn.p, H, cfg.rms_norm_eps,
-                   (float*)nullptr, (float*)nullptr, 0, LO_ROW, (float*)nullptr, ss_b.p, fused_parts);
+                   (float*)nullptr, LO_ROW, (float*)nullptr, ss_b.p, fused_parts);
         const size_t kv_layer = (size_t)cfg.max_batch * nkv * cfg.max_context * HD;
         for (int l = 0; l < L; ++l) {
             LayerW& Lw = layers[l];
-            tc_gemm(tm_qkv[l], tmx_xn, OP_QKV, qkv.p, nullptr, B, NQ + 2 * NKV, H, s, ss_b.p);
+            qkv_gemm(l, B, s);
             AttnArgs aa{qkv.p, pos.p, freqs.p, kcache.p + l * kv_layer, vcache.p + l * kv_layer, attn.p, nq, nkv, cfg.max_context,
-                        1.0f / sqrtf((float)HD), spec.qk_norm ? Lw.qnorm.p : nullptr, spec.qk_norm ? Lw.knorm.p : nullptr, cfg.rms_norm_eps, 1};
+                        1.0f / sqrtf((float)HD), spec.qk_norm ? Lw.qnorm.p : nullptr, spec.qk_norm ? Lw.knorm.p : nullptr, cfg.rms_norm_eps};
             attn_launch(aa, B, s);
             splitk_gemm(tm_o[l], tmx_attn, H, NQ, Lw.ln2.p, ss_a.p, B, s);
             tc_gemm(tm_gu_dec[l], tmx_xn, OP_GU, nullptr, act.p, B, 2 * I, H, s, ss_a.p);
@@ -1216,22 +1227,22 @@
     void run_layers(int B, cudaStream_t s) {
         if (fused && !trace_on) { run_layers_fused(B, s); return; }
         const int H = cfg.hidden_size, nq = cfg.num_attention_heads, nkv = cfg.num_key_value_heads;
-        const int QKV_N = (nq + 2 * nkv) * HD, G = nq / nkv;
+        const int G = nq / nkv;
         if (x_ext) launch_pdl(ext_embed_kernel, dim3(B), dim3(256), 0, s, x_ext, x.p, y.p, H);
         else launch_pdl(embed_kernel, dim3(B), dim3(256), 0, s, tokens.p, embed.p, x.p, y.p, H, cfg.vocab_size);
         const size_t kv_layer = (size_t)cfg.max_batch * nkv * cfg.max_context * HD;
         for (int l = 0; l < cfg.num_hidden_layers; ++l) {
             LayerW& L = layers[l];
             launch_pdl(add_rmsnorm_kernel, dim3(B), dim3(RN_THREADS), 0, s, x.p, l == 0 ? (float*)nullptr : y.p, L.ln1.p, xn.p, H,
-                       cfg.rms_norm_eps, trace_on ? trace.p + (size_t)(2 * l) * 8 * H : (float*)nullptr, (float*)nullptr, 0, LO_ROW,
+                       cfg.rms_norm_eps, trace_on ? trace.p + (size_t)(2 * l) * 8 * H : (float*)nullptr, LO_ROW,
                        (float*)nullptr, (float*)nullptr, 0);
             gemm(OP_QKV, l, B, s);
             AttnArgs aa{qkv.p, pos.p, freqs.p, kcache.p + l * kv_layer, vcache.p + l * kv_layer, attn.p, nq, nkv, cfg.max_context,
-                        1.0f / sqrtf((float)HD), spec.qk_norm ? L.qnorm.p : nullptr, spec.qk_norm ? L.knorm.p : nullptr, cfg.rms_norm_eps, 0};
+                        1.0f / sqrtf((float)HD), spec.qk_norm ? L.qnorm.p : nullptr, spec.qk_norm ? L.knorm.p : nullptr, cfg.rms_norm_eps};
             attn_launch(aa, B, s);
             gemm(OP_O, l, B, s);
             launch_pdl(add_rmsnorm_kernel, dim3(B), dim3(RN_THREADS), 0, s, x.p, y.p, L.ln2.p, xn.p, H, cfg.rms_norm_eps,
-                       trace_on ? trace.p + (size_t)(2 * l + 1) * 8 * H : (float*)nullptr, qkv.p, QKV_N, LO_ROW, (float*)nullptr, (float*)nullptr, 0);
+                       trace_on ? trace.p + (size_t)(2 * l + 1) * 8 * H : (float*)nullptr, LO_ROW, (float*)nullptr, (float*)nullptr, 0);
             gemm(OP_GU, l, B, s);
             gemm(OP_DOWN, l, B, s);
         }
@@ -1246,7 +1257,7 @@
             return;
         }
         launch_pdl(add_rmsnorm_kernel, dim3(B), dim3(RN_THREADS), 0, s, x.p, y.p, final_ln.p, xn.p, cfg.hidden_size, cfg.rms_norm_eps,
-                   trace_on ? trace.p + (size_t)(2 * cfg.num_hidden_layers) * 8 * cfg.hidden_size : (float*)nullptr, (float*)nullptr, 0, LO_ROW,
+                   trace_on ? trace.p + (size_t)(2 * cfg.num_hidden_layers) * 8 * cfg.hidden_size : (float*)nullptr, LO_ROW,
                    normed_out, (float*)nullptr, 0);
     }
     void run_lm_head(int B, cudaStream_t s) {
@@ -1256,7 +1267,7 @@
     }
     void run_lm_head_after_prefill(int B, cudaStream_t s) {
         launch_pdl(add_rmsnorm_kernel, dim3(B), dim3(RN_THREADS), 0, s, x.p, y.p, final_ln.p, xn.p, cfg.hidden_size, cfg.rms_norm_eps,
-                   (float*)nullptr, (float*)nullptr, 0, LO_ROW, (float*)nullptr, (float*)nullptr, 0);
+                   (float*)nullptr, LO_ROW, (float*)nullptr, (float*)nullptr, 0);
         gemm(OP_LM, -1, B, s);
     }
     void run_head(const CUtensorMap& tmW, const bf16* W, int M, float* logits_out, int B, cudaStream_t s, int tile_rows = 0) {
@@ -1315,7 +1326,7 @@
         for (int l = 0; l < cfg.num_hidden_layers; ++l) {
             LayerW& Lw = layers[l];
             launch_pdl(add_rmsnorm_kernel, dim3(T), dim3(RN_THREADS), 0, s, xp.p, l == 0 ? (float*)nullptr : yp.p, Lw.ln1.p, xnp.p, H,
-                       cfg.rms_norm_eps, (float*)nullptr, (float*)nullptr, 0, PF_HALF, (float*)nullptr, (float*)nullptr, 0);
+                       cfg.rms_norm_eps, (float*)nullptr, PF_HALF, (float*)nullptr, (float*)nullptr, 0);
             pf_gemm(tm_qkv[l], tmp_xn, tc::EPI_STORE, qkvp.p, nullptr, T, QKV_N, H, s);
             PrefillAttnArgs pa{qkvp.p, rope_tab.p, kcache.p + l * kv_layer, vcache.p + l * kv_layer, attnp.p, nq, nkv,
                                cfg.max_context, L, 1.0f / sqrtf((float)HD)};
@@ -1332,7 +1343,7 @@
             count_launch();
             pf_gemm(tm_o[l], tmp_attn, tc::EPI_STORE, yp.p, nullptr, T, H, NQ, s);
             launch_pdl(add_rmsnorm_kernel, dim3(T), dim3(RN_THREADS), 0, s, xp.p, yp.p, Lw.ln2.p, xnp.p, H, cfg.rms_norm_eps,
-                       (float*)nullptr, (float*)nullptr, 0, PF_HALF, (float*)nullptr, (float*)nullptr, 0);
+                       (float*)nullptr, PF_HALF, (float*)nullptr, (float*)nullptr, 0);
             pf_gemm(tm_gu[l], tmp_xn, tc::EPI_SWIGLU, nullptr, actp.p, T, 2 * I, H, s);
             pf_gemm(tm_down[l], tmp_act, tc::EPI_STORE, yp.p, nullptr, T, H, I, s);
         }
@@ -1783,6 +1794,21 @@
     });
 }
 
+int32_t b2a_debug_qkv_split(int32_t m_tiles, int32_t k_blocks, int32_t* out) {
+    return guarded([&] {
+        B2A_CHECK(out && m_tiles >= 1 && k_blocks >= 1, B2A_ERR_INVALID_INPUT, "b2a_debug_qkv_split: bad argument");
+        require_device(0);
+        tc::set_attributes();
+        int sms = 0, sk_ctas = 0;
+        B2A_CUDA(cudaDeviceGetAttribute(&sms, cudaDevAttrMultiProcessorCount, 0));
+        out[0] = b2a_tts::pick_qkv_cluster(m_tiles, k_blocks, sms, &sk_ctas);
+        out[1] = out[0] ? (int32_t)tc::SmemSplit::bytes(b2a_tts::splitk_stages, out[0]) : 0;
+        out[2] = out[0] ? tc::splitk_active_clusters(out[0], (size_t)out[1]) : 0;
+        out[3] = sk_ctas;
+        out[4] = tc::stream_k_slots(m_tiles, k_blocks, sk_ctas);
+    });
+}
+
 int32_t b2a_tts_debug_trace(b2a_tts* h, int32_t enable, int32_t batch, float* out) {
     return guarded([&] {
         B2A_CHECK(h, B2A_ERR_INVALID_INPUT, "b2a_tts_debug_trace: null handle");
diff --git a/mlx-audio-swift_b200/csrc/tc_gemm.cu b/mlx-audio-swift_b200/csrc/tc_gemm.cu
--- a/mlx-audio-swift_b200/csrc/tc_gemm.cu
+++ b/mlx-audio-swift_b200/csrc/tc_gemm.cu
@@ -79,6 +79,8 @@
 
 void launch_splitk(const CUtensorMap& tmA, const CUtensorMap& tmB, const SplitArgs& a, int m_tiles, int cluster, cudaStream_t s) {
     B2A_CHECK(SmemSplit::bytes(a.stages, cluster) <= 227 * 1024, B2A_ERR_INVALID_INPUT, "tc_gemm: split-K ring does not fit in shared memory");
+    B2A_CHECK(a.sk_ctas <= 0 || (!a.h && cluster >= stream_k_slots(m_tiles, a.k_blocks, a.sk_ctas)), B2A_ERR_INVALID_INPUT,
+              "tc_gemm: the stream-K cut is a store-mode option and needs a CTA per piece of a tile");
     cudaLaunchConfig_t cfg{};
     cfg.gridDim = dim3((unsigned)(m_tiles * cluster)); cfg.blockDim = dim3(THREADS);
     cfg.dynamicSmemBytes = SmemSplit::bytes(a.stages, cluster); cfg.stream = s;
@@ -90,6 +92,20 @@
     cfg.attrs = at; cfg.numAttrs = 2;
     B2A_CUDA(cudaLaunchKernelEx(&cfg, tc_gemm_splitk_kernel, tmA, tmB, a));
     count_launch();
+}
+
+int splitk_active_clusters(int cluster, size_t smem_bytes) {
+    B2A_CHECK(cluster >= 1 && cluster <= SPLIT_MAX_CLUSTER, B2A_ERR_INVALID_INPUT, "tc_gemm: split-K cluster size must be in [1, 8]");
+    cudaLaunchConfig_t cfg{};
+    cfg.gridDim = dim3((unsigned)cluster); cfg.blockDim = dim3(THREADS);
+    cfg.dynamicSmemBytes = smem_bytes;
+    cudaLaunchAttribute at[1];
+    at[0].id = cudaLaunchAttributeClusterDimension;
+    at[0].val.clusterDim.x = (unsigned)cluster; at[0].val.clusterDim.y = 1; at[0].val.clusterDim.z = 1;
+    cfg.attrs = at; cfg.numAttrs = 1;
+    int n = 0;
+    B2A_CUDA(cudaOccupancyMaxActiveClusters(&n, tc_gemm_splitk_kernel, &cfg));
+    return n;
 }
 
 void set_attributes() {
@@ -189,3 +205,27 @@
         B2A_CUDA(cudaStreamSynchronize((cudaStream_t)stream));
     });
 }
+
+extern "C" int32_t b2a_tc_gemm_splitk_store_test(const void* W, const void* X, float* out, const float* rstd_ss, int32_t rstd_parts,
+                                                 float rstd_eps, int32_t M, int32_t N, int32_t K, int32_t cluster, int32_t sk_ctas,
+                                                 int32_t stages, void* stream) {
+    using namespace b2a;
+    using namespace b2a::tc;
+    return guarded([&] {
+        B2A_CHECK(W && X && out && M > 0 && M % 8 == 0 && K > 0 && K % BK == 0 && N >= 1 && N <= 8 && stages >= 1 &&
+                      (!rstd_ss || rstd_parts >= 1),
+                  B2A_ERR_INVALID_INPUT, "b2a_tc_gemm_splitk_store_test: bad argument");
+        B2A_CHECK(cluster >= 1 && cluster <= SPLIT_MAX_CLUSTER && cluster <= K / BK, B2A_ERR_INVALID_INPUT,
+                  "b2a_tc_gemm_splitk_store_test: cluster must be in [1, min(8, K / 64)]");
+        require_device(0);
+        set_attributes();
+        CUtensorMap ta = make_tmap_bf16(W, M, K, BM), tb = make_tmap_bf16(X, 16, K, 16);
+        SplitArgs a{};
+        a.M = M; a.N = N; a.K = K; a.k_blocks = K / BK; a.stages = stages; a.sk_ctas = sk_ctas;
+        a.out = out;
+        a.rstd_ss = rstd_ss; a.rstd_parts = rstd_parts; a.rstd_inv_h = 1.0f / (float)K; a.rstd_eps = rstd_eps;
+        launch_splitk(ta, tb, a, cdiv(M, BM), cluster, (cudaStream_t)stream);
+        B2A_CUDA(cudaGetLastError());
+        B2A_CUDA(cudaStreamSynchronize((cudaStream_t)stream));
+    });
+}
diff --git a/mlx-audio-swift_b200/csrc/tc_gemm.cuh b/mlx-audio-swift_b200/csrc/tc_gemm.cuh
--- a/mlx-audio-swift_b200/csrc/tc_gemm.cuh
+++ b/mlx-audio-swift_b200/csrc/tc_gemm.cuh
@@ -451,7 +451,10 @@
                         for (int e = 0; e < PER; ++e) {
                             const int i = i0 + threadIdx.x + e * NT;
                             const int tcol = i / BM, r = i - tcol * BM, mm = mt * BM + r, tok = ntok0 + tcol;
-                            if (i < n_el && tok < a.N && mm < a.M) a.out_f32[(long long)tok * a.ldo + mm] += sum[e];
+                            if (i < n_el && tok < a.N && mm < a.M) {
+                                float* o = a.out_f32 + (long long)tok * a.ldo + mm;
+                                *o = a.epi_full == EPI_ADD ? *o + sum[e] : sum[e];
+                            }
                         }
                     }
                     if (threadIdx.x == 0) a.part_cnt[tile_id] = 0;
@@ -464,10 +467,12 @@
 struct SplitArgs {
     int M, N, K;
     int k_blocks, stages;
+    int sk_ctas;
     float* h;
     const float* gain;
     __nv_bfloat16* xn;
     float* ss;
+    float* out;
     const float* rstd_ss;
     int rstd_parts;
     float rstd_inv_h, rstd_eps;
@@ -486,6 +491,20 @@
 }
 __device__ __forceinline__ void st_cluster_f4(uint32_t addr, float a, float b, float c, float d) {
     asm volatile("st.shared::cluster.v4.f32 [%0], {%1, %2, %3, %4};" ::"r"(addr), "f"(a), "f"(b), "f"(c), "f"(d) : "memory");
+}
+
+__host__ __device__ __forceinline__ void split_range(const SplitArgs& a, int mt, int m_tiles, int r, int C, int& kb0, int& kb1) {
+    if (a.sk_ctas > 0) {
+        const long long units = (long long)m_tiles * a.k_blocks, t0 = (long long)mt * a.k_blocks, t1 = t0 + a.k_blocks;
+        const long long c = stream_k_owner(t0, units, a.sk_ctas) + r;
+        const long long u0 = units * c / a.sk_ctas, u1 = units * (c + 1) / a.sk_ctas;
+        kb0 = (int)(u0 > t0 ? u0 - t0 : 0);
+        kb1 = (int)(u1 < t1 ? u1 - t0 : a.k_blocks);
+        if (kb1 < kb0) kb1 = kb0;
+    } else {
+        kb0 = (int)((long long)a.k_blocks * r / C);
+        kb1 = (int)((long long)a.k_blocks * (r + 1) / C);
+    }
 }
 
 constexpr int SPLIT_MAX_CLUSTER = 8;
@@ -510,8 +529,9 @@
     float* s_red = reinterpret_cast<float*>(empty + a.stages);
 
     const int warp = threadIdx.x >> 5, lane = threadIdx.x & 31;
-    const int mt = blockIdx.x / C;
-    const int kb0 = (int)((long long)a.k_blocks * rank / C), kb1 = (int)((long long)a.k_blocks * (rank + 1) / C);
+    const int mt = blockIdx.x / C, m_tiles = gridDim.x / C;
+    int kb0, kb1;
+    split_range(a, mt, m_tiles, rank, C, kb0, kb1);
     asm volatile("griddepcontrol.launch_dependents;" ::: "memory");
 
     check_smem_base(smem);
@@ -544,7 +564,7 @@
             }
         }
     }
-    float acc[8], hold[8];
+    float acc[8], hold[8], rstd[8];
     float g = 0.f;
     const int q = warp & 3, row = q * 32 + lane;
     const int m = mt * BM + row;
@@ -552,9 +572,23 @@
     if (warp < 4) {
         if (rank == 0) {
             asm volatile("griddepcontrol.wait;" ::: "memory");
-            g = m_ok ? a.gain[m] : 0.f;
-#pragma unroll
-            for (int j = 0; j < 8; ++j) hold[j] = (j < a.N && m_ok) ? a.h[(long long)j * a.M + m] : 0.f;
+            if (a.h) {
+                g = m_ok ? a.gain[m] : 0.f;
+#pragma unroll
+                for (int j = 0; j < 8; ++j) hold[j] = (j < a.N && m_ok) ? a.h[(long long)j * a.M + m] : 0.f;
+            }
+            if (a.rstd_ss) {
+                float t = 0.f;
+                for (int p0 = 0; p0 < a.rstd_parts; p0 += 4) {
+                    const int p = p0 + (lane >> 3);
+                    if (p < a.rstd_parts) t += a.rstd_ss[p * 8 + (lane & 7)];
+                }
+                t += __shfl_xor_sync(0xffffffffu, t, 8);
+                t += __shfl_xor_sync(0xffffffffu, t, 16);
+                const float rs = rsqrtf(t * a.rstd_inv_h + a.rstd_eps);
+#pragma unroll
+                for (int j = 0; j < 8; ++j) rstd[j] = __shfl_sync(0xffffffffu, rs, j);
+            }
         }
         float d[2][8];
 #pragma unroll
@@ -599,23 +633,34 @@
     __syncwarp();
     cluster_sync_all();
     if (rank == 0 && warp < 4) {
+        if (!a.h) {
+            float sum[8];
+#pragma unroll
+            for (int j = 0; j < 8; ++j) sum[j] = __fadd_rn(0.f, a.rstd_ss ? __fmul_rn(acc[j], rstd[j]) : acc[j]);
+            for (uint32_t r = 1; r < C; ++r) {
+                int r0, r1;
+                split_range(a, mt, m_tiles, (int)r, (int)C, r0, r1);
+                if (r0 == r1) continue;
+                const float* p = part + ((size_t)(r - 1) * BM + row) * 8;
+#pragma unroll
+                for (int j = 0; j < 8; ++j) sum[j] = __fadd_rn(sum[j], a.rstd_ss ? __fmul_rn(p[j], rstd[j]) : p[j]);
+            }
+#pragma unroll
+            for (int j = 0; j < 8; ++j)
+                if (j < a.N && m_ok) a.out[(long long)j * a.M + m] = sum[j];
+            return;
+        }
         for (uint32_t r = 1; r < C; ++r) {
             const float4 p0 = *reinterpret_cast<const float4*>(part + ((size_t)(r - 1) * BM + row) * 8);
             const float4 p1 = *reinterpret_cast<const float4*>(part + ((size_t)(r - 1) * BM + row) * 8 + 4);
             acc[0] += p0.x; acc[1] += p0.y; acc[2] += p0.z; acc[3] += p0.w;
             acc[4] += p1.x; acc[5] += p1.y; acc[6] += p1.z; acc[7] += p1.w;
         }
+        if (a.rstd_ss) {
+#pragma unroll
+            for (int j = 0; j < 8; ++j) acc[j] *= rstd[j];
+        }
         const int w4 = warp;
-        if (a.rstd_ss) {
-            if (w4 == 0 && lane < 8) {
-                float t = 0.f;
-                for (int p = 0; p < a.rstd_parts; ++p) t += a.rstd_ss[p * 8 + lane];
-                s_red[32 + lane] = rsqrtf(t * a.rstd_inv_h + a.rstd_eps);
-            }
-            asm volatile("bar.sync 1, 128;" ::: "memory");
-#pragma unroll
-            for (int j = 0; j < 8; ++j) acc[j] *= s_red[32 + j];
-        }
         float sq[8];
 #pragma unroll
         for (int j = 0; j < 8; ++j) {
@@ -653,6 +698,7 @@
 void launch(const CUtensorMap& tmA, const CUtensorMap& tmB, const Args& a, int ctas, int n_tiles, cudaStream_t s);
 
 void launch_splitk(const CUtensorMap& tmA, const CUtensorMap& tmB, const SplitArgs& a, int m_tiles, int cluster, cudaStream_t s);
+int splitk_active_clusters(int cluster, size_t smem_bytes);
 
 void set_attributes();
 
```

Result: faster. 32.63 (median of 6 runs) (+9.6%).
